# diegoroyo/mitransient

Measured on AMD Instinct MI355X. Metric: Mray/s (closest-hit + shadow rays), Cornell-box 512^2 x 1024 bins x 1024 spp per GPU, higher is better.
Workload: dtype f32; 1 GPU; cornell_box() diffuse, 512x512 px, 1024 time bins (start_opl 3.5, width 6/1024), 1024 spp per GPU (1024 spp total), max_depth 8, rr_depth 5, seed 0; parallelism=1 GPU, mode=auto (fused: scene + per-pixel time histograms in LDS)

## Files before the change

__graft_entry__.py:

```python
from __future__ import annotations

import os
import subprocess
import sys

ROOT = os.path.dirname(os.path.abspath(__file__))
if ROOT not in sys.path:
    sys.path.insert(0, ROOT)


def _run(cmd, cwd=None):
    r = subprocess.run(cmd, cwd=cwd, stdout=subprocess.PIPE, stderr=subprocess.STDOUT, text=True)
    if r.returncode != 0:
        raise RuntimeError(f"{' '.join(cmd)} failed:\n{r.stdout}")
    return r.stdout


def build_host_harness():
    out_dir = os.path.join(ROOT, "tests", "_build")
    os.makedirs(out_dir, exist_ok=True)
    out = os.path.join(out_dir, "libhost_harness.so")
    srcs = [os.path.join(ROOT, "tests", "host_harness.cpp"),
            os.path.join(ROOT, "mitransient_amd", "csrc", "mtr_scene_host.cpp"),
            os.path.join(ROOT, "mitransient_amd", "csrc", "mtr_bvh.cpp")]
    deps = srcs + [os.path.join(ROOT, "mitransient_amd", "csrc", h) for h in
                   ("mtr_core.h", "mtr_scene_host.h", "mtr_bvh.h", "mtr_knobs.h")]
    if os.path.exists(out) and all(os.path.getmtime(out) >= os.path.getmtime(d) for d in deps):
        return out
    _run(["g++", "-O2", "-std=c++17", "-fPIC", "-shared", "-ffp-contract=off", "-fno-fast-math", "-mfma", "-DMTR_EXPERIMENTS",
          "-o", out] + srcs)
    return out


def build() -> None:
    _run(["make", "-C", os.path.join(ROOT, "mitransient_amd", "csrc")])
    _run(["make", "-C", os.path.join(ROOT, "oracle")])
    build_host_harness()
    import mitransient_amd
    from mitransient_amd import _cabi
    lib = _cabi.load_library()
    for name in _cabi.EXPORTS:
        getattr(lib, name)


def smoke() -> None:
    import numpy as np
    import torch
    import mitransient_amd as mitr
    import mitransient_amd.mi as mi
    from oracle import oracle

    assert torch.cuda.is_available(), "smoke() needs a GPU"
    torch.cuda.set_device(0)
    mi.set_variant("llvm_ad_rgb")
    d = mitr.cornell_box()
    d["sensor"]["film"].update(width=64, height=64, temporal_bins=64, bin_width_opl=6.0 / 64)
    scene = mi.load_dict(d)
    integ = scene.integrator()
    integ.collect_stats = True
    steady, transient = mi.render(scene, spp=16, seed=0)
    torch.cuda.synchronize()
    t_gpu = np.array(transient)
    s_gpu = np.array(steady)
    sd = scene.data()
    params = integ.render_params(scene.sensors()[0].film(), 0, 16)
    t4, s4, cnt = oracle.render(sd, params, use_bvh=True)
    t_ref, s_ref = oracle.develop(sd.film, t4, s4)
    rel = float(np.linalg.norm(t_gpu - t_ref) / np.linalg.norm(t_ref))
    rel_s = float(np.linalg.norm(s_gpu - s_ref) / np.linalg.norm(s_ref))
    print(f"smoke: transient rel-L2 {rel:.3e}, steady rel-L2 {rel_s:.3e}, counters {integ.last_counters} vs oracle {cnt}")
    assert t_gpu.shape == (64, 64, 64, 3) and s_gpu.shape == (64, 64, 3)
    assert rel <= 1e-5, rel
    assert rel_s <= 1e-5, rel_s
    for k in ("paths", "rays_closest", "rays_shadow", "splats_issued", "bounces"):
        assert integ.last_counters[k] == cnt[k], (k, integ.last_counters[k], cnt[k])


if __name__ == "__main__":
    build()
# ... 3 lines not shown
```

include/mitransient_amd.h:

```cpp
#ifndef MITRANSIENT_AMD_H
#define MITRANSIENT_AMD_H

#include <stdint.h>
#include <stddef.h>

#ifdef __cplusplus
extern "C" {
#endif

#define MTR_ABI_VERSION 24

typedef enum mtr_status {
    MTR_OK = 0,
    MTR_ERR_INVALID = -1,
    MTR_ERR_NO_DEVICE = -2,
    MTR_ERR_HIP = -3,
    MTR_ERR_OOM = -4,
    MTR_ERR_UNSUPPORTED = -5
} mtr_status;

enum { MTR_BSDF_DIFFUSE = 0, MTR_BSDF_CONDUCTOR = 1, MTR_BSDF_DIELECTRIC = 2,
       MTR_BSDF_NULL = 3 ,
       MTR_BSDF_ROUGHCONDUCTOR = 4,
       MTR_BSDF_ROUGHPLASTIC = 5,
// ... 88 lines not shown
    uint32_t has_to_world;
    float    to_world[12];
    uint32_t kind;
    float    radius;
} mtr_shape;

#define MTR_NLOS_NO_RELAY 0xffffffffu
typedef struct mtr_nlos_desc {
    float    sensor_origin[3];
    uint32_t relay_shape;
    float    laser_to_world[16];
    float    laser_fov;
    float    laser_irradiance[3];
    float    laser_scale;
    uint32_t capture_type;
    uint32_t flags;
    int32_t  filter_depth;
    float    illumination_scan_fov;
    uint32_t n_shapes;
    const mtr_shape *shapes;
    uint32_t sensor_is_confocal;
    float    sensor_target[3];
} mtr_nlos_desc;

typedef struct mtr_scene_desc {
    uint32_t        n_tris;
    const float    *tri_verts;
    const uint32_t *tri_material;
    const int32_t  *tri_emitter;
    uint32_t        n_materials;
    const mtr_material *materials;
    uint32_t        n_emitters;
    const mtr_emitter  *emitters;
    mtr_camera      camera;
    mtr_film_desc   film;
    const mtr_nlos_desc *nlos;
    uint32_t        n_shapes;
    const mtr_shape *shapes;
    const float    *tri_uv;
    const float    *tri_normals;
    uint32_t        n_textures;
    const mtr_texture *textures;
} mtr_scene_desc;

enum { MTR_FLAG_CAMERA_UNWARP = 1u,
       MTR_FLAG_DISCARD_DIRECT_LIGHT = 2u,
       MTR_FLAG_FILM_ZERO = 4u,
       MTR_FLAG_KEEP_COUNTERS = 16u,
       MTR_FLAG_DETERMINISTIC = 32u,
       MTR_FLAG_DEVELOPED_ROWS = 64u,
       MTR_FLAG_PCG_INITSEQ_PLUS_LANE = 8u ,
       MTR_FLAG_POLARIZED = 256u,
       MTR_FLAG_PCG_TEA64 = 128u            };

enum { MTR_MODE_AUTO = 0,
       MTR_MODE_FUSED = 1,
       MTR_MODE_WAVEFRONT = 2,
       MTR_MODE_SAMPLES = 3      };

typedef struct mtr_render_params {
    uint32_t spp_total;
    uint32_t spp_begin;
    uint32_t spp_end;
    uint32_t pixel_begin;
    uint32_t pixel_end;
    uint32_t seed;
    int32_t  max_depth;
    int32_t  rr_depth;
    uint32_t flags;
    uint32_t mode;
    uint32_t spp_scale;
    uint32_t reserve_cus;
    uint32_t n_bands;
    uint32_t band_epoch;
    uint64_t band_done;
} mtr_render_params;

typedef struct mtr_counters {
    uint64_t paths;
    uint64_t rays_closest;
    uint64_t rays_shadow;
    uint64_t splats_issued;
    uint64_t bounces;
    uint64_t splats_overflow;
    uint64_t reserved[2];
} mtr_counters;

typedef struct mtr_splat_soa {
    const uint32_t *pixel;
    const float    *opl;
    const float    *r, *g, *b;
    uint64_t        n;
    const uint32_t *laser;
} mtr_splat_soa;

typedef struct mtr_kernel_times {
    float    total_ms;
    float    trace_ms;
    float    scatter_ms;
    uint32_t trace_launches;
    uint32_t scatter_launches;
    float    wf_trace_ms;
    uint32_t wf_trace_kernel_launches;
    float    wf_shade_ms;
} mtr_kernel_times;

typedef struct mtr_ctx   mtr_ctx;
typedef struct mtr_scene mtr_scene;

int  mtr_abi_version(void);

int  mtr_ctx_create(int device_ordinal, mtr_ctx **out);
void mtr_ctx_destroy(mtr_ctx *);
int  mtr_ctx_set_stream(mtr_ctx *, void *hip_stream);
const char *mtr_last_error(const mtr_ctx *);

int  mtr_scene_create(mtr_ctx *, const mtr_scene_desc *, mtr_scene **out);
void mtr_scene_destroy(mtr_scene *);
int  mtr_scene_set_film(mtr_scene *, const mtr_film_desc *);
int  mtr_scene_set_camera(mtr_scene *, const mtr_camera *);
int  mtr_scene_set_nlos(mtr_scene *, const mtr_nlos_desc *);
int  mtr_scene_bvh_info(const mtr_scene *, uint32_t *n_nodes, uint32_t *max_depth, uint32_t *n_leaves);
#define MTR_TRAIT_DIFFUSE          1u
#define MTR_TRAIT_ONE_RECT_EMITTER 2u
#define MTR_TRAIT_LEAF_PAIR        4u
#define MTR_TRAIT_FLAT_TOP         8u
#define MTR_TRAIT_FLAT_LEAVES     16u
#define MTR_TRAIT_NO_LOBES        32u
#define MTR_TRAIT_GREY            64u
int  mtr_scene_traits(const mtr_scene *, uint32_t *traits);
int  mtr_scene_set_colors(mtr_scene *, const float *material_a, const float *emitter_radiance);
int  mtr_scene_set_texture(mtr_scene *, uint32_t index, const float *rgb);
int  mtr_scene_texture_layout(const mtr_scene *, uint32_t index, uint32_t *first_texel, uint32_t *width, uint32_t *height);

int  mtr_scene_tint_layout(const mtr_scene *, uint32_t *n_slots, uint32_t *slot_material, uint32_t *slot_which);
int  mtr_scene_set_tints(mtr_scene *, const float *material_c, const float *material_c2);

int  mtr_film_clear(mtr_ctx *, const mtr_film_desc *, float *transient_hwt4 ,
                    float *steady_hw4 );

int  mtr_render(mtr_scene *, const mtr_render_params *,
                float *transient_hwt4, float *steady_hw4,
                mtr_counters *counters_out , mtr_kernel_times *times_out );

int  mtr_render_plan(mtr_scene *, const mtr_render_params *, uint32_t *mode_out,
                     uint32_t *developed_rows_ok );
int  mtr_render_samples_plan(mtr_scene *, const mtr_render_params *, uint32_t *slab_len, uint32_t *n_slabs,
                             uint32_t *scene_in_lds, uint32_t *extended);

int  mtr_render_grad(mtr_scene *, const mtr_render_params *params,
                     const float *grad_steady_hw3, const float *grad_transient_hwt3,
                     float *grad_materials, float *grad_emitters);

int  mtr_render_grad_tex(mtr_scene *, const mtr_render_params *params,
                         const float *grad_steady_hw3, const float *grad_transient_hwt3,
                         float *grad_materials, float *grad_emitters, float *grad_texels);
#define MTR_GRAD_TEX_NONE   0u
#define MTR_GRAD_TEX_SLAB   1u
#define MTR_GRAD_TEX_GLOBAL 2u
int  mtr_render_grad_tex_tier(const mtr_scene *, uint32_t *tier);

int  mtr_render_fwd(mtr_scene *, const mtr_render_params *params,
                    const float *tan_materials, const float *tan_emitters, const float *tan_texels ,
                    float *steady_hw3, float *transient_hwt3);
#define MTR_FWD_ROWS   1u
#define MTR_FWD_GLOBAL 2u
int  mtr_render_fwd_tier(const mtr_scene *, const mtr_render_params *params, uint32_t *tier);

int  mtr_render_grad_tint(mtr_scene *, const mtr_render_params *params,
                          const float *grad_steady_hw3, const float *grad_transient_hwt3,
                          float *grad_materials, float *grad_emitters, float *grad_texels , float *grad_tints );
int  mtr_render_fwd_tint(mtr_scene *, const mtr_render_params *params,
                         const float *tan_materials, const float *tan_emitters, const float *tan_texels ,
                         const float *tan_tints , float *steady_hw3, float *transient_hwt3);

int  mtr_counters_reset(mtr_ctx *);

int  mtr_counters_read(mtr_ctx *, mtr_counters *out );

int  mtr_film_develop(mtr_ctx *, const mtr_film_desc *,
                      const float *transient_hwt4, float *transient_hwt3 ,
                      const float *steady_hw4, float *steady_hw3 );

// ... 29 lines not shown
```

mitransient_amd/_cabi.py:

```python
from __future__ import annotations

import ctypes as C
import os

_HERE = os.path.dirname(os.path.abspath(__file__))
LIB_PATH = os.environ.get("MITRANSIENT_AMD_LIB") or os.path.join(_HERE, "csrc", "libmitransient_amd.so")

MTR_ABI_VERSION = 24
MTR_TRAIT_DIFFUSE, MTR_TRAIT_ONE_RECT_EMITTER, MTR_TRAIT_LEAF_PAIR, MTR_TRAIT_FLAT_TOP, MTR_TRAIT_FLAT_LEAVES, MTR_TRAIT_NO_LOBES, MTR_TRAIT_GREY = 1, 2, 4, 8, 16, 32, 64
MTR_SPLAT_FILM_ZERO = 0x100

MTR_BSDF_DIFFUSE, MTR_BSDF_CONDUCTOR, MTR_BSDF_DIELECTRIC, MTR_BSDF_NULL = 0, 1, 2, 3
MTR_BSDF_ROUGHCONDUCTOR, MTR_BSDF_ROUGHPLASTIC, MTR_BSDF_ROUGHDIELECTRIC, MTR_BSDF_THINDIELECTRIC, MTR_BSDF_PLASTIC = 4, 5, 6, 7, 8
MTR_MAT_TWOSIDED, MTR_MAT_NONLINEAR, MTR_MAT_BECKMANN, MTR_MAT_ANISOTROPIC = 1, 2, 4, 8
MTR_ROUGH_TRANSMITTANCE_RES = 64
MTR_FLAG_CAMERA_UNWARP = 1
MTR_FLAG_DISCARD_DIRECT_LIGHT = 2
MTR_FLAG_FILM_ZERO = 4
MTR_FLAG_PCG_INITSEQ_PLUS_LANE = 8
MTR_FLAG_PCG_TEA64 = 128
MTR_FLAG_KEEP_COUNTERS = 16
MTR_FLAG_DETERMINISTIC = 32
MTR_FLAG_DEVELOPED_ROWS = 64
MTR_FLAG_POLARIZED = 256
MTR_MODE_AUTO, MTR_MODE_FUSED, MTR_MODE_WAVEFRONT, MTR_MODE_SAMPLES = 0, 1, 2, 3
MTR_RECT_ANALYTIC, MTR_RECT_FLIP_NORMALS = 1, 2
MTR_EMITTER_AREA, MTR_EMITTER_POINT, MTR_EMITTER_SPOT, MTR_EMITTER_SPHERE = 0, 1, 2, 3
MTR_SHAPE_DEFAULT, MTR_SHAPE_SPHERE, MTR_SHAPE_FLIP_NORMALS = 0, 1, 0x100
MTR_GRAD_TEX_NONE, MTR_GRAD_TEX_SLAB, MTR_GRAD_TEX_GLOBAL = 0, 1, 2
MTR_FWD_ROWS, MTR_FWD_GLOBAL = 1, 2

_f3 = C.c_float * 3
_f16 = C.c_float * 16


class mtr_material(C.Structure):
    _fields_ = [("type", C.c_uint32), ("flags", C.c_uint32),
                ("a", _f3), ("b", _f3), ("c", _f3),
                ("int_ior", C.c_float), ("ext_ior", C.c_float), ("c2", _f3),
                ("alpha", C.c_float), ("internal_reflectance", C.c_float), ("specular_sampling_weight", C.c_float),
                ("albedo_texture", C.c_uint32), ("external_transmittance", C.c_float * MTR_ROUGH_TRANSMITTANCE_RES)]


class mtr_texture(C.Structure):
    _fields_ = [("width", C.c_uint32), ("height", C.c_uint32), ("rgb", C.POINTER(C.c_float))]


class mtr_emitter(C.Structure):
    _fields_ = [("center", _f3), ("du", _f3), ("dv", _f3), ("radiance", _f3),
                ("is_mesh", C.c_uint32), ("first_tri", C.c_uint32), ("n_tris", C.c_uint32),
                ("flip_normals", C.c_uint32),
                ("angular", C.c_uint32), ("cutoff", C.c_float), ("cos_cutoff", C.c_float), ("cos_beam", C.c_float),
                ("inv_transition", C.c_float),
                ("kind", C.c_uint32), ("axis", _f3),
                ("radius", C.c_float)]


class mtr_camera(C.Structure):
    _fields_ = [("sample_to_camera", _f16), ("to_world", _f16),
                ("near_clip", C.c_float), ("far_clip", C.c_float)]


class mtr_film_desc(C.Structure):
    _fields_ = [("width", C.c_uint32), ("height", C.c_uint32),
                ("crop_width", C.c_uint32), ("crop_height", C.c_uint32),
                ("crop_offset_x", C.c_uint32), ("crop_offset_y", C.c_uint32),
                ("temporal_bins", C.c_uint32),
                ("start_opl", C.c_float), ("bin_width_opl", C.c_float),
                ("laser_scan_width", C.c_uint32), ("laser_scan_height", C.c_uint32),
                ("n_frequencies", C.c_uint32), ("frequencies", C.POINTER(C.c_float))]


MTR_CAPTURE_SINGLE, MTR_CAPTURE_CONFOCAL, MTR_CAPTURE_EXHAUSTIVE = 1, 2, 3
# ... 41 lines not shown
                ("emitters", C.POINTER(mtr_emitter)),
                ("camera", mtr_camera),
                ("film", mtr_film_desc),
                ("nlos", C.POINTER(mtr_nlos_desc)),
                ("n_shapes", C.c_uint32),
                ("shapes", C.POINTER(mtr_shape)),
                ("tri_uv", C.POINTER(C.c_float)),
                ("tri_normals", C.POINTER(C.c_float)),
                ("n_textures", C.c_uint32),
                ("textures", C.POINTER(mtr_texture))]


class mtr_render_params(C.Structure):
    _fields_ = [("spp_total", C.c_uint32), ("spp_begin", C.c_uint32), ("spp_end", C.c_uint32),
                ("pixel_begin", C.c_uint32), ("pixel_end", C.c_uint32),
                ("seed", C.c_uint32), ("max_depth", C.c_int32), ("rr_depth", C.c_int32),
                ("flags", C.c_uint32), ("mode", C.c_uint32), ("spp_scale", C.c_uint32), ("reserve_cus", C.c_uint32),
                ("n_bands", C.c_uint32), ("band_epoch", C.c_uint32), ("band_done", C.c_uint64)]


class mtr_counters(C.Structure):
    _fields_ = [("paths", C.c_uint64), ("rays_closest", C.c_uint64), ("rays_shadow", C.c_uint64),
                ("splats_issued", C.c_uint64), ("bounces", C.c_uint64), ("splats_overflow", C.c_uint64),
                ("reserved", C.c_uint64 * 2)]

    def as_dict(self):
        d = {k: int(getattr(self, k)) for k in
             ("paths", "rays_closest", "rays_shadow", "splats_issued", "bounces", "splats_overflow")}
        d["reserved"] = [int(self.reserved[0]), int(self.reserved[1])]
        return d


class mtr_splat_soa(C.Structure):
    _fields_ = [("pixel", C.c_void_p), ("opl", C.c_void_p),
                ("r", C.c_void_p), ("g", C.c_void_p), ("b", C.c_void_p), ("n", C.c_uint64),
                ("laser", C.c_void_p)]


class mtr_kernel_times(C.Structure):
    _fields_ = [("total_ms", C.c_float), ("trace_ms", C.c_float), ("scatter_ms", C.c_float),
                ("trace_launches", C.c_uint32), ("scatter_launches", C.c_uint32),
                ("wf_trace_ms", C.c_float), ("wf_trace_kernel_launches", C.c_uint32),
                ("wf_shade_ms", C.c_float)]

    def as_dict(self):
        return {"total_ms": float(self.total_ms), "trace_ms": float(self.trace_ms),
                "scatter_ms": float(self.scatter_ms), "trace_launches": int(self.trace_launches),
                "scatter_launches": int(self.scatter_launches), "wf_trace_ms": float(self.wf_trace_ms),
                "wf_trace_kernel_launches": int(self.wf_trace_kernel_launches), "wf_shade_ms": float(self.wf_shade_ms)}


EXPORTS = [
    "mtr_abi_version", "mtr_ctx_create", "mtr_ctx_destroy", "mtr_ctx_set_stream", "mtr_last_error",
    "mtr_scene_create", "mtr_scene_destroy", "mtr_scene_set_film", "mtr_scene_set_nlos", "mtr_scene_bvh_info", "mtr_scene_traits",
    "mtr_ctx_trim", "mtr_film_clear", "mtr_render", "mtr_render_plan", "mtr_counters_reset", "mtr_counters_read", "mtr_film_develop", "mtr_splat_add", "mtr_debug_set_splat_log",
    "mtr_render_grad", "mtr_scene_set_colors",
    "mtr_render_grad_tex", "mtr_render_grad_tex_tier", "mtr_scene_set_texture", "mtr_scene_texture_layout",
    "mtr_render_fwd", "mtr_render_fwd_tier",
    "mtr_scene_tint_layout", "mtr_scene_set_tints", "mtr_render_grad_tint", "mtr_render_fwd_tint",
    "mtr_scene_set_camera", "mtr_render_samples_plan",
    "mtr_backproject",
]

_lib = None


class MitransientAMDError(RuntimeError):
    pass


def load_library() -> C.CDLL:
    global _lib
    if _lib is not None:
        return _lib
    if not os.path.exists(LIB_PATH):
        raise MitransientAMDError(
            f"{LIB_PATH} not found: build the gfx950 HIP library first "
            "(python -c 'import __graft_entry__ as g; g.build()'). There is no CPU fallback.")
    import torch
    lib = C.CDLL(LIB_PATH)
    vp = C.c_void_p
    lib.mtr_abi_version.restype = C.c_int
    lib.mtr_ctx_create.argtypes = [C.c_int, C.POINTER(vp)]
    lib.mtr_ctx_destroy.argtypes = [vp]
    lib.mtr_ctx_destroy.restype = None
    lib.mtr_ctx_set_stream.argtypes = [vp, vp]
    lib.mtr_last_error.argtypes = [vp]
    lib.mtr_last_error.restype = C.c_char_p
    lib.mtr_scene_create.argtypes = [vp, C.POINTER(mtr_scene_desc), C.POINTER(vp)]
    lib.mtr_scene_destroy.argtypes = [vp]
    lib.mtr_scene_destroy.restype = None
    lib.mtr_scene_set_film.argtypes = [vp, C.POINTER(mtr_film_desc)]
    lib.mtr_scene_set_nlos.argtypes = [vp, C.POINTER(mtr_nlos_desc)]
    lib.mtr_scene_bvh_info.argtypes = [vp, C.POINTER(C.c_uint32), C.POINTER(C.c_uint32), C.POINTER(C.c_uint32)]
    lib.mtr_scene_traits.argtypes = [vp, C.POINTER(C.c_uint32)]
    lib.mtr_counters_read.argtypes = [vp, C.POINTER(mtr_counters)]
    lib.mtr_counters_reset.argtypes = [vp]
    lib.mtr_ctx_trim.argtypes = [vp]
    lib.mtr_render_plan.argtypes = [vp, C.POINTER(mtr_render_params), C.POINTER(C.c_uint32), C.POINTER(C.c_uint32)]
    lib.mtr_film_clear.argtypes = [vp, C.POINTER(mtr_film_desc), vp, vp]
    lib.mtr_render.argtypes = [vp, C.POINTER(mtr_render_params), vp, vp,
                               C.POINTER(mtr_counters), C.POINTER(mtr_kernel_times)]
    lib.mtr_film_develop.argtypes = [vp, C.POINTER(mtr_film_desc), vp, vp, vp, vp]
    lib.mtr_splat_add.argtypes = [vp, C.POINTER(mtr_splat_soa), C.POINTER(mtr_film_desc), C.c_int, vp,
                                  C.POINTER(C.c_float)]
    lib.mtr_debug_set_splat_log.argtypes = [vp, vp, C.c_uint64, vp]
    lib.mtr_render_grad.argtypes = [vp, C.POINTER(mtr_render_params), vp, vp, vp, vp]
    lib.mtr_scene_set_colors.argtypes = [vp, vp, vp]
    lib.mtr_render_grad_tex.argtypes = [vp, C.POINTER(mtr_render_params), vp, vp, vp, vp, vp]
    lib.mtr_render_grad_tex_tier.argtypes = [vp, C.POINTER(C.c_uint32)]
    lib.mtr_scene_set_texture.argtypes = [vp, C.c_uint32, vp]
    lib.mtr_scene_texture_layout.argtypes = [vp, C.c_uint32, C.POINTER(C.c_uint32), C.POINTER(C.c_uint32), C.POINTER(C.c_uint32)]
    lib.mtr_render_fwd.argtypes = [vp, C.POINTER(mtr_render_params), vp, vp, vp, vp, vp]
    lib.mtr_render_fwd_tier.argtypes = [vp, C.POINTER(mtr_render_params), C.POINTER(C.c_uint32)]
    lib.mtr_scene_tint_layout.argtypes = [vp, C.POINTER(C.c_uint32), vp, vp]
    lib.mtr_scene_set_tints.argtypes = [vp, vp, vp]
    lib.mtr_render_grad_tint.argtypes = [vp, C.POINTER(mtr_render_params), vp, vp, vp, vp, vp, vp]
    lib.mtr_render_fwd_tint.argtypes = [vp, C.POINTER(mtr_render_params), vp, vp, vp, vp, vp, vp]
    lib.mtr_scene_set_camera.argtypes = [vp, C.POINTER(mtr_camera)]
    lib.mtr_render_samples_plan.argtypes = [vp, C.POINTER(mtr_render_params)] + [C.POINTER(C.c_uint32)] * 4
    lib.mtr_backproject.argtypes = [vp, C.POINTER(mtr_backproject_desc), vp, vp]
    if lib.mtr_abi_version() != MTR_ABI_VERSION:
        raise MitransientAMDError("libmitransient_amd.so ABI version mismatch; rebuild")
    _lib = lib
    return lib


def check(status: int, ctx=None, what: str = ""):
    if status == 0:
        return
    msg = ""
    try:
        msg = (load_library().mtr_last_error(ctx) or b"").decode()
    except Exception:
        pass
    raise MitransientAMDError(f"{what} failed (status {status}): {msg}")
```

mitransient_amd/csrc/mtr_api.hip:

```cpp
#include "../../include/mitransient_amd.h"
#include "mtr_knobs.h"
#include "mtr_scene_host.h"
#include "mtr_core.h"
#include "mtr_kernels.h"
#include "mtr_polar.h"
#include "mtr_grad.h"
#include "mtr_fwd_args.h"
#include "mtr_tint_args.h"
#include "mtr_samples_args.h"
#include "mtr_backproject.h"

#include <hip/hip_runtime.h>
#include <cassert>
#include <cmath>
#include <cstdio>
#include <cstring>
#include <cstdlib>
#include <initializer_list>
#include <string>
#include <vector>
#include <algorithm>
#include <utility>

using namespace mtr;
// ... 10 lines not shown
    hipEvent_t ev2 = nullptr, ev3 = nullptr;
    float *d_freq = nullptr; size_t freq_cap = 0;
    void *d_runs = nullptr; size_t runs_cap = 0;
    uint32_t *d_band_count = nullptr; size_t band_cap = 0;
    void *d_part = nullptr; size_t part_cap = 0;
    void *d_samples = nullptr; size_t samples_cap = 0;
    void *d_start = nullptr; size_t start_cap = 0;
    void *d_bp = nullptr; size_t bp_cap = 0;
};

struct WfWorkspace {
    void *planes = nullptr, *q_live = nullptr, *q_ray = nullptr, *q_mat = nullptr, *r_shadow = nullptr, *occ = nullptr, *counts = nullptr, *rec = nullptr, *rec_count = nullptr, *q_zombie = nullptr;
    uint32_t n_slots = 0, P = 0, rec_cap = 0, rows = 0;
    size_t bytes = 0;
    bool polar = false;
    uint32_t *host_count = nullptr;
    hipEvent_t poll_ev[2] = { nullptr, nullptr };
    void release()
    {
        n_slots = 0; P = 0; rec_cap = 0; rows = 0; bytes = 0; polar = false;
        for (void **p : { &planes, &q_live, &q_ray, &q_mat, &r_shadow, &occ, &counts, &rec, &rec_count, &q_zombie })
            if (*p) { (void)hipFree(*p); *p = nullptr; }
    }
};

struct NlosDev {
    bool on = false;
    NlosConst k{};
    void *shapes = nullptr, *tables = nullptr, *hg_tris = nullptr, *hg_vn = nullptr, *targets = nullptr;
    std::vector<mtr_shape> host_shapes;
};

struct mtr_scene {
    mtr_ctx *ctx = nullptr;
    WfWorkspace wf;
    NlosDev nlos;
    std::vector<float> tri_verts;
    std::vector<float> tri_normals;
    uint32_t n_emitters_area = 0;
    bool polar_ok = false;
    bool grey_scene = false;
    bool has_sphere = false;
    SceneDev dev{};
    Camera cam{};
    Film film{};
    mtr_film_desc film_desc{};
    float *d_freq = nullptr;
    std::vector<float> h_freq;
    uint32_t n_leaves = 0;
    std::vector<q4> tex_info;
    uint32_t n_texels = 0;
    std::vector<void *> allocs;
    SplatLog log{ nullptr, 0, nullptr };
};

static thread_local std::string g_err;

static int fail(mtr_ctx *c, int code, const std::string &msg)
{
    if (c) c->err = msg; else g_err = msg;
    return code;
}
static int usable_cus(const mtr_ctx *c, const mtr_render_params *p)
{
    const int keep = (int)std::min<uint32_t>(p->reserve_cus, (uint32_t)(c->n_cu > 1 ? c->n_cu - 1 : 0));
    return c->n_cu - keep;
}

#define HIP_TRY(c, expr)                                                                       \
    do {                                                                                        \
        hipError_t e_ = (expr);                                                                 \
        if (e_ != hipSuccess)                                                                   \
            return fail((c), e_ == hipErrorOutOfMemory ? MTR_ERR_OOM : MTR_ERR_HIP,             \
                        std::string(#expr) + ": " + hipGetErrorString(e_));                     \
    } while (0)

extern "C" {

int mtr_abi_version(void) { return MTR_ABI_VERSION; }

const char *mtr_last_error(const mtr_ctx *c) { return c ? c->err.c_str() : g_err.c_str(); }

int mtr_ctx_create(int device_ordinal, mtr_ctx **out)
{
    if (!out) return fail(nullptr, MTR_ERR_INVALID, "mtr_ctx_create: out is NULL");
    *out = nullptr;
    int n = 0;
    if (hipGetDeviceCount(&n) != hipSuccess || n == 0)
        return fail(nullptr, MTR_ERR_NO_DEVICE, "no HIP device visible; this library has no CPU path");
    if (device_ordinal < 0 || device_ordinal >= n)
        return fail(nullptr, MTR_ERR_INVALID, "mtr_ctx_create: device ordinal out of range");
    mtr_ctx *c = new mtr_ctx();
    c->device = device_ordinal;
    HIP_TRY(nullptr, hipSetDevice(device_ordinal));
    hipDeviceProp_t prop;
    HIP_TRY(nullptr, hipGetDeviceProperties(&prop, device_ordinal));
    c->n_cu = prop.multiProcessorCount > 0 ? prop.multiProcessorCount : 256;
    HIP_TRY(nullptr, hipMalloc((void **)&c->d_counters, sizeof(DevCounters)));
    HIP_TRY(nullptr, hipMalloc((void **)&c->d_ticket, 32 * sizeof(uint32_t)));
    for (hipEvent_t *e : { &c->ev0, &c->ev1, &c->ev2, &c->ev3 }) HIP_TRY(nullptr, hipEventCreate(e));
    *out = c;
    return MTR_OK;
}

void mtr_ctx_destroy(mtr_ctx *c)
{
// ... 32 lines not shown
    return MTR_OK;
}

template <class T>
static int upload(mtr_scene *s, const std::vector<T> &v, const T **out)
{
    size_t bytes = ((v.size() * sizeof(T) + 15) / 16) * 16;
    if (bytes == 0) bytes = 16;
    void *p = nullptr;
    HIP_TRY(s->ctx, hipMalloc(&p, bytes));
    s->allocs.push_back(p);
    HIP_TRY(s->ctx, hipMemset(p, 0, bytes));
    if (!v.empty()) HIP_TRY(s->ctx, hipMemcpy(p, v.data(), v.size() * sizeof(T), hipMemcpyHostToDevice));
    *out = (const T *)p;
    return MTR_OK;
}

extern "C" {

static int scene_take_film(mtr_scene *s, const mtr_film_desc &f);

int mtr_scene_create(mtr_ctx *c, const mtr_scene_desc *d, mtr_scene **out)
{
    if (!c || !d || !out) return fail(c, MTR_ERR_INVALID, "mtr_scene_create: NULL argument");
    *out = nullptr;
    int rc = check_film(c, d->film);
    if (rc) return rc;
    HostScene hs;
    if (const char *msg = derive_scene(*d, hs)) return fail(c, MTR_ERR_INVALID, std::string("mtr_scene_create: ") + msg);
    HIP_TRY(c, hipSetDevice(c->device));

    mtr_scene *s = new mtr_scene();
    s->ctx = c;
    s->cam = hs.cam;
    rc = scene_take_film(s, d->film);
    if (rc) { delete s; return rc; }

#define UP(vec, field)                                                       \
    do { rc = upload(s, vec, &s->dev.field); if (rc) { mtr_scene_destroy(s); return rc; } } while (0)
    UP(hs.nodes, nodes); UP(hs.tpairs, tpairs); UP(hs.tshade, tshade); UP(hs.mats, mats); UP(hs.ems, ems);
    s->dev.n_wnodes = (uint32_t)hs.wnodes.size(); s->dev.n_wnodes4 = (uint32_t)hs.wnodes4.size(); s->dev.n_wnodes8q = (uint32_t)hs.wnodes8q.size();
    if (hs.has_wide) UP(hs.wnodes, wnodes);
    UP(hs.wnodes4, wnodes4);
    if (!hs.wnodes8q.empty()) UP(hs.wnodes8q, wnodes8q);
    if (!hs.samp_tris.empty()) { UP(hs.samp_tris, samp_tris); UP(hs.face_pmf, face_pmf); UP(hs.face_cdf, face_cdf); }
    if (!hs.samp_vn.empty()) UP(hs.samp_vn, samp_vn);
    if (!hs.vnormals.empty()) UP(hs.vnormals, vnormals);
    if (!hs.texels.empty()) { UP(hs.texels, texels); UP(hs.tex_info, tex_info); UP(hs.uvs, uvs); }
#undef UP
    s->tex_info = hs.tex_info; s->n_texels = (uint32_t)hs.texels.size();
    s->dev.n_nodes = (uint32_t)hs.nodes.size(); s->dev.n_slots = (uint32_t)hs.tshade.size();
    s->dev.n_mats = d->n_materials; s->dev.n_ems = d->n_emitters;
    s->polar_ok = hs.polar_ok; s->grey_scene = hs.grey_scene; s->has_sphere = hs.has_sphere;
    s->dev.has_rough = hs.needs_ext ? 1u : 0u; s->dev.traits = hs.traits; s->dev.flat = hs.flat;
    s->dev.bvh_depth = hs.bvh_depth; s->n_leaves = hs.n_leaves;
    s->dev.wide_levels = hs.wide_levels; s->dev.wide4_levels = hs.wide4_levels; s->dev.wide8q_levels = hs.wide8q_levels;
    s->tri_verts.assign(d->tri_verts, d->tri_verts + 9 * (size_t)d->n_tris);
    if (d->tri_normals) s->tri_normals.assign(d->tri_normals, d->tri_normals + 9 * (size_t)d->n_tris);
    s->n_emitters_area = d->n_emitters;
    if (d->nlos) {
        rc = mtr_scene_set_nlos(s, d->nlos);
        if (rc) { mtr_scene_destroy(s); return rc; }
    }
    *out = s;
    return MTR_OK;
}

int mtr_scene_set_nlos(mtr_scene *s, const mtr_nlos_desc *n)
{
    if (!s || !n) return fail(s ? s->ctx : nullptr, MTR_ERR_INVALID, "mtr_scene_set_nlos: NULL argument");
    mtr_ctx *c = s->ctx;
    HIP_TRY(c, hipSetDevice(c->device));
    mtr_scene_desc d{};
    d.n_tris = (uint32_t)(s->tri_verts.size() / 9); d.tri_verts = s->tri_verts.data(); d.n_emitters = s->n_emitters_area;
    d.tri_normals = s->tri_normals.empty() ? nullptr : s->tri_normals.data();
    d.film = s->film_desc;
    memcpy(d.camera.sample_to_camera, s->cam.s2c, sizeof s->cam.s2c);
    memcpy(d.camera.to_world, s->cam.tw, sizeof s->cam.tw);
    d.camera.near_clip = s->cam.near_clip; d.camera.far_clip = s->cam.far_clip;
    d.nlos = n;
    if (d.film.n_frequencies && n->capture_type == MTR_CAPTURE_EXHAUSTIVE)
        return fail(c, MTR_ERR_UNSUPPORTED, "mtr_scene_set_nlos: an Exhaustive capture (MTR_CAPTURE_EXHAUSTIVE) is not available with a phasor_hdr_film");
    HostNlos hn;
    if (const char *msg = derive_nlos(d, hn)) return fail(c, MTR_ERR_INVALID, std::string("mtr_scene_set_nlos: ") + msg);
    NlosDev &D = s->nlos;
    void **old[] = { &D.shapes, &D.tables, &D.hg_tris, &D.hg_vn, &D.targets };
    for (void **p : old) if (*p) { (void)hipFree(*p); *p = nullptr; }
    const size_t ns = hn.shapes.size(), nt = hn.face_pmf.size();
    HIP_TRY(c, hipMalloc(&D.shapes, ns * sizeof(NlosShape)));
    HIP_TRY(c, hipMemcpy(D.shapes, hn.shapes.data(), ns * sizeof(NlosShape), hipMemcpyHostToDevice));
    std::vector<float> tab;
    tab.insert(tab.end(), hn.shape_pmf.begin(), hn.shape_pmf.end());
    tab.insert(tab.end(), hn.shape_cdf.begin(), hn.shape_cdf.end());
    tab.insert(tab.end(), hn.face_pmf.begin(), hn.face_pmf.end());
    tab.insert(tab.end(), hn.face_cdf.begin(), hn.face_cdf.end());
    HIP_TRY(c, hipMalloc(&D.tables, tab.size() * 4));
    HIP_TRY(c, hipMemcpy(D.tables, tab.data(), tab.size() * 4, hipMemcpyHostToDevice));
    HIP_TRY(c, hipMalloc(&D.hg_tris, hn.hg_tris.size() * sizeof(q4)));
    HIP_TRY(c, hipMemcpy(D.hg_tris, hn.hg_tris.data(), hn.hg_tris.size() * sizeof(q4), hipMemcpyHostToDevice));
    if (!hn.hg_vn.empty()) {
        HIP_TRY(c, hipMalloc(&D.hg_vn, hn.hg_vn.size() * sizeof(q4)));
        HIP_TRY(c, hipMemcpy(D.hg_vn, hn.hg_vn.data(), hn.hg_vn.size() * sizeof(q4), hipMemcpyHostToDevice));
    }
    const size_t n_targets = nlos_target_count(hn.k);
    HIP_TRY(c, hipMalloc(&D.targets, n_targets * sizeof(q4)));
    D.k = hn.k;
    D.k.shapes = (const NlosShape *)D.shapes;
// ... 119 lines not shown
                if (slot_material) slot_material[slots[i]] = (uint32_t)(i / 2u);
                if (slot_which) slot_which[slots[i]] = (uint32_t)(i & 1u);
            }
    return MTR_OK;
}

int mtr_scene_set_texture(mtr_scene *s, uint32_t index, const float *rgb)
{
    if (!s || !rgb) return fail(s ? s->ctx : nullptr, MTR_ERR_INVALID, "mtr_scene_set_texture: NULL argument");
    mtr_ctx *c = s->ctx;
    if (index >= s->tex_info.size()) return fail(c, MTR_ERR_INVALID, "mtr_scene_set_texture: unknown texture");
    if (s->nlos.on) return fail(c, MTR_ERR_UNSUPPORTED, "mtr_scene_set_texture: not for the NLOS tier");
    HIP_TRY(c, hipSetDevice(c->device));
    HIP_TRY(c, hipStreamSynchronize(c->stream));
    const q4 info = s->tex_info[index];
    const size_t first = fbits(info.x), n = (size_t)fbits(info.y) * fbits(info.z);
    std::vector<q4> tx(n);
    for (size_t k = 0; k < n; ++k) tx[k] = q4{ rgb[3 * k], rgb[3 * k + 1], rgb[3 * k + 2], 0.0f };
    HIP_TRY(c, hipMemcpy((void *)(s->dev.texels + first), tx.data(), n * sizeof(q4), hipMemcpyHostToDevice));
    double mean[3] = { 0.0, 0.0, 0.0 };
    for (size_t k = 0; k < n; ++k) for (int j = 0; j < 3; ++j) mean[j] += (double)rgb[3 * k + j];
    std::vector<mtr_material> mats(s->dev.n_mats);
    if (!mats.empty()) HIP_TRY(c, hipMemcpy(mats.data(), s->dev.mats, mats.size() * sizeof(mtr_material), hipMemcpyDeviceToHost));
    for (mtr_material &m : mats)
        if (m.albedo_texture == index + 1u) for (int j = 0; j < 3; ++j) m.a[j] = (float)(mean[j] / (double)n);
    if (!mats.empty()) HIP_TRY(c, hipMemcpy((void *)s->dev.mats, mats.data(), mats.size() * sizeof(mtr_material), hipMemcpyHostToDevice));
    return MTR_OK;
}

int mtr_scene_texture_layout(const mtr_scene *s, uint32_t index, uint32_t *first_texel, uint32_t *width, uint32_t *height)
{
    if (!s || index > s->tex_info.size()) return MTR_ERR_INVALID;
    const bool end = index == s->tex_info.size();
    if (first_texel) *first_texel = end ? s->n_texels : fbits(s->tex_info[index].x);
    if (width) *width = end ? 0u : fbits(s->tex_info[index].y);
    if (height) *height = end ? 0u : fbits(s->tex_info[index].z);
    return MTR_OK;
}

int mtr_render_grad_tex_tier(const mtr_scene *s, uint32_t *tier)
{
    if (!s || !tier) return MTR_ERR_INVALID;
    *tier = grad_tex_tier(s->dev, s->n_texels, s->nlos.on);
    return MTR_OK;
}

int mtr_scene_traits(const mtr_scene *s, uint32_t *traits)
{
    if (!s || !traits) return MTR_ERR_INVALID;
    static_assert(MTR_TRAIT_DIFFUSE == kTrDiffuse && MTR_TRAIT_ONE_RECT_EMITTER == kTrOneRectEmitter && MTR_TRAIT_LEAF_PAIR == kTrLeafPair &&
                  MTR_TRAIT_FLAT_TOP == kTrFlatTop && MTR_TRAIT_FLAT_LEAVES == kTrFlatLeaves && MTR_TRAIT_NO_LOBES == kTrNoLobes &&
                  MTR_TRAIT_GREY == kTrGrey, "public trait bits");
    *traits = s->dev.traits;
    return MTR_OK;
}

}

struct WfBytes {
    size_t planes, q_live, q_ray, q_mat, q_zombie, r_shadow, occ, counts, rec, rec_count;
    size_t total() const { return planes + q_live + q_ray + q_mat + q_zombie + r_shadow + occ + counts + rec + rec_count; }
};
static WfBytes wf_bytes(uint32_t n_slots, uint32_t P, uint32_t n_seg, uint32_t rec_cap, bool polar)
{
    WfBytes b;
    b.planes = wf_planes_bytes(n_slots) + (polar ? wf_polar_planes_bytes(n_slots) : 0);
    b.q_live = (size_t)2 * n_slots * 4;
    b.q_ray = (size_t)2 * n_slots * 32;
    b.q_mat = (size_t)kWfKeys * n_slots * 4;
    b.q_zombie = (size_t)2 * n_slots * 4;
    b.r_shadow = (size_t)n_slots * 32;
    b.occ = (size_t)n_slots + (size_t)n_seg * 16u + 16u;
    b.counts = ((size_t)n_seg * (7 + kWfKeys) + 16) * 4;
    b.rec = std::max<size_t>(16, (size_t)P * rec_cap * 16);
    b.rec_count = (size_t)P * 4;
    return b;
}
static int wf_alloc(mtr_scene *s, uint32_t n_slots, uint32_t P, uint32_t n_seg, uint32_t rec_cap, bool polar = false)
{
    mtr_ctx *c = s->ctx;
    WfWorkspace &w = s->wf;
    if (w.n_slots >= n_slots && w.P >= P && w.rec_cap == rec_cap && w.rows >= n_seg && w.planes && (w.polar || !polar)) return MTR_OK;
    w.release();
    const WfBytes b = wf_bytes(n_slots, P, n_seg, rec_cap, polar);
    HIP_TRY(c, hipMalloc(&w.planes, b.planes));
    HIP_TRY(c, hipMalloc(&w.q_live, b.q_live));
    HIP_TRY(c, hipMalloc(&w.q_ray, b.q_ray));
    HIP_TRY(c, hipMalloc(&w.q_mat, b.q_mat));
    HIP_TRY(c, hipMalloc(&w.q_zombie, b.q_zombie));
    HIP_TRY(c, hipMalloc(&w.r_shadow, b.r_shadow));
    HIP_TRY(c, hipMalloc(&w.occ, b.occ));
    HIP_TRY(c, hipMalloc(&w.counts, b.counts));
    HIP_TRY(c, hipMalloc(&w.rec, b.rec));
    HIP_TRY(c, hipMalloc(&w.rec_count, b.rec_count));
    if (!w.host_count) HIP_TRY(c, hipHostMalloc((void **)&w.host_count, 64));
    for (hipEvent_t &e : w.poll_ev) if (!e) HIP_TRY(c, hipEventCreateWithFlags(&e, hipEventDisableTiming));
    w.n_slots = n_slots; w.P = P; w.rec_cap = rec_cap; w.rows = n_seg; w.bytes = b.total(); w.polar = polar;
    return MTR_OK;
}

struct RenderStats {
    uint32_t launches = 0, scatter_launches = 0, trace_kernel_launches = 0;
    float trace_ms = 0.0f, shade_ms = 0.0f, scatter_ms = 0.0f;
};
struct EventPairs {
    std::vector<std::pair<hipEvent_t, hipEvent_t>> ev;
// ... 260 lines not shown
    HIP_TRY(c, hipMemcpy(&h, c->d_counters, sizeof h, hipMemcpyDeviceToHost));
    memset(out, 0, sizeof *out);
    out->paths = h.paths; out->rays_closest = h.rays_closest; out->rays_shadow = h.rays_shadow;
    out->splats_issued = h.splats_issued; out->bounces = h.bounces; out->splats_overflow = h.splats_overflow;
    out->reserved[0] = h.r0; out->reserved[1] = h.r1;
    return MTR_OK;
}
static int grow_device_buffer(mtr_ctx *c, void **ptr, size_t *cap, size_t need)
{
    if (*cap >= need) return MTR_OK;
    HIP_TRY(c, hipStreamSynchronize(c->stream));
    if (*ptr) (void)hipFree(*ptr);
    *ptr = nullptr; *cap = 0;
    HIP_TRY(c, hipMalloc(ptr, need));
    *cap = need;
    return MTR_OK;
}

extern "C" {

int mtr_film_clear(mtr_ctx *c, const mtr_film_desc *f, float *t4, float *s4)
{
    if (!c || !f) return fail(c, MTR_ERR_INVALID, "mtr_film_clear: NULL argument");
    HIP_TRY(c, hipSetDevice(c->device));
    size_t npix = (size_t)f->width * f->height;
    const Film fm = film_from_desc(*f);
    const size_t per_pixel = fm.n_freq ? (size_t)2 * fm.n_freq + 1 : (size_t)fm.bins * 4;
    if (t4) HIP_TRY(c, hipMemsetAsync(t4, 0, npix * per_pixel * sizeof(float), c->stream));
    if (s4) HIP_TRY(c, hipMemsetAsync(s4, 0, npix * 4 * sizeof(float), c->stream));
    return MTR_OK;
}

int mtr_render(mtr_scene *s, const mtr_render_params *p, float *t4, float *s4,
               mtr_counters *counters_out, mtr_kernel_times *times_out)
{
    if (!s || !p || !t4 || !s4) return fail(s ? s->ctx : nullptr, MTR_ERR_INVALID, "mtr_render: NULL argument");
    mtr_ctx *c = s->ctx;
    const Film &f = s->film;
    if (int r = check_render_ranges(c, f, p, "mtr_render", "shard the render")) return r;
    if (p->mode > MTR_MODE_SAMPLES) return fail(c, MTR_ERR_INVALID, "mtr_render: unknown mode");
    SamplesPlan spl{};
    if (p->mode == MTR_MODE_SAMPLES)
        if (int r = samples_check(s, p, p->pixel_end - p->pixel_begin, p->spp_end - p->spp_begin, &spl)) return r;
    HIP_TRY(c, hipSetDevice(c->device));

    FusedArgs a{};
    a.sc = s->dev; a.cam = s->cam; a.film = f;
    a.rc = make_render_const(*p, f, s->dev.n_ems);
    a.pixel_begin = p->pixel_begin; a.pixel_end = p->pixel_end;
    a.spp_begin = p->spp_begin; a.spp_chunk = p->spp_end - p->spp_begin;
    a.film_out = t4; a.steady_out = s4;
    a.counters = c->d_counters;
    a.log = s->log;
    a.nlos_on = s->nlos.on ? 1u : 0u;
    if (s->nlos.on) {
        a.nlos = s->nlos.k;
        if (s->nlos.k.film_w != f.width || s->nlos.k.film_h != f.height)
            return fail(c, MTR_ERR_INVALID, "mtr_render: film size changed after mtr_scene_set_nlos; call it again");
    }

    const uint32_t n_pixels = p->pixel_end - p->pixel_begin;
    const bool want_stats = counters_out || times_out;
    if (!(p->flags & MTR_FLAG_KEEP_COUNTERS)) HIP_TRY(c, hipMemsetAsync(c->d_counters, 0, sizeof(DevCounters), c->stream));
    if (s->log.count) HIP_TRY(c, hipMemsetAsync(s->log.count, 0, sizeof(unsigned long long), c->stream));
    if (times_out) HIP_TRY(c, hipEventRecord(c->ev0, c->stream));
    RenderStats st;
    if (n_pixels && a.spp_chunk && p->mode == MTR_MODE_SAMPLES) {
        constexpr size_t kSamplesRetain = (size_t)256 << 20;
        if (int r = grow_device_buffer(c, &c->d_samples, &c->samples_cap, spl.partial_bytes)) return r;
        SamplesArgs sa{};
        sa.sc = s->dev; sa.cam = s->cam; sa.film = f; sa.rc = a.rc;
        sa.pixel_begin = p->pixel_begin; sa.n_pixels = n_pixels; sa.spp_begin = p->spp_begin; sa.spp_chunk = a.spp_chunk;
        sa.film_zero = (p->flags & MTR_FLAG_FILM_ZERO) ? 1u : 0u;
        sa.partial = (float *)c->d_samples; sa.film_out = t4; sa.steady_out = s4; sa.counters = c->d_counters;
        HIP_TRY(c, launch_samples(sa, spl, c->stream));
        st.launches = 2;
        if (c->samples_cap > kSamplesRetain) {
            HIP_TRY(c, hipStreamSynchronize(c->stream));
            (void)hipFree(c->d_samples);
            c->d_samples = nullptr; c->samples_cap = 0;
        }
    } else if (n_pixels && a.spp_chunk) {
        uint32_t mode = p->mode, dev_ok = 0u;
        if (int r = resolve_mode(s, p, n_pixels, a.spp_chunk, &mode, &dev_ok)) return r;
        if ((p->flags & MTR_FLAG_DEVELOPED_ROWS) && !dev_ok)
            return fail(c, MTR_ERR_UNSUPPORTED, "mtr_render: MTR_FLAG_DEVELOPED_ROWS needs the fused organisation with time-bin rows in LDS (see mtr_render_plan)");
        if (p->n_bands && (mode == MTR_MODE_WAVEFRONT || !p->band_done || p->n_bands > n_pixels))
            return fail(c, MTR_ERR_UNSUPPORTED, "mtr_render: band completion words need the fused organisation, a band_done array and at most one band per pixel");
        if (mode == MTR_MODE_WAVEFRONT) {
            if (int r = wf_render(s, p, t4, s4, a.rc, times_out != nullptr, want_stats, &st)) return r;
        } else {
            FusedConfig cfg{};
            if (!fused_plan(s->dev, f, n_pixels, a.spp_chunk, usable_cus(c, p), a, cfg))
                return fail(c, MTR_ERR_UNSUPPORTED, "mtr_render: no kernel configuration fits (BVH depth / LDS)");
            const uint32_t launch_slot = c->fused_launches++ & 15u;
            a.ticket = c->d_ticket + launch_slot;
            static_assert(kStartSlots == 16u, "one path-start table per ticket counter of the rotation");
            if (const size_t tab_bytes = fused_start_table_bytes(a, cfg)) {
                if (start_slot_stride(c->start_cap) < tab_bytes)
                    if (int r = grow_device_buffer(c, &c->d_start, &c->start_cap, start_alloc_bytes(tab_bytes))) return r;
                a.start_tab = (unsigned char *)c->d_start + start_slot_off(start_slot_stride(c->start_cap), launch_slot);
            }
            a.n_bands = 0u;
            if (p->n_bands) {
                if (int r = grow_device_buffer(c, (void **)&c->d_band_count, &c->band_cap, (size_t)p->n_bands * sizeof(uint32_t))) return r;
                HIP_TRY(c, hipMemsetAsync(c->d_band_count, 0, (size_t)p->n_bands * sizeof(uint32_t), c->stream));
// ... 441 lines not shown
```

mitransient_amd/csrc/mtr_core.h:

```cpp
#pragma once
#ifndef MTR_WIDE
#define MTR_WIDE 8
#endif
#ifndef MTR_BATCH
#define MTR_BATCH 15
#endif
#ifndef MTR_PATH_STATE
#define MTR_PATH_STATE 3
#endif

#include <stdint.h>
#include <math.h>
#include "../../include/mitransient_amd.h"
#include "mtr_flat_prims.h"

#if defined(__HIPCC__)
#include <hip/hip_runtime.h>
#define MTR_HD __host__ __device__ __forceinline__
#else
#define MTR_HD inline __attribute__((always_inline))
#endif

namespace mtr {

struct f3 { float x, y, z; };

MTR_HD f3 mk(float x, float y, float z) { f3 r; r.x = x; r.y = y; r.z = z; return r; }
MTR_HD f3 operator-(f3 a, f3 b) { return mk(a.x - b.x, a.y - b.y, a.z - b.z); }
MTR_HD f3 operator-(f3 a) { return mk(-a.x, -a.y, -a.z); }
MTR_HD f3 operator*(f3 a, float s) { return mk(a.x * s, a.y * s, a.z * s); }
MTR_HD f3 operator/(f3 a, float s) { float r = 1.0f / s; return mk(a.x * r, a.y * r, a.z * r); }
MTR_HD float dot(f3 a, f3 b) { return fmaf(a.x, b.x, fmaf(a.y, b.y, a.z * b.z)); }
MTR_HD f3 cross(f3 a, f3 b)
{
    return mk(fmaf(a.y, b.z, -(a.z * b.y)), fmaf(a.z, b.x, -(a.x * b.z)), fmaf(a.x, b.y, -(a.y * b.x)));
}
MTR_HD f3 normalize(f3 a) { return a / sqrtf(dot(a, a)); }
MTR_HD f3 fma3(f3 a, float s, f3 b) { return mk(fmaf(a.x, s, b.x), fmaf(a.y, s, b.y), fmaf(a.z, s, b.z)); }
MTR_HD float max3(float a, float b, float c) { return fmaxf(a, fmaxf(b, c)); }
MTR_HD bool sign_neg(float s) { return s < 0.0f || (s == 0.0f && signbit(s)); }

constexpr float kPi = 3.14159265358979323846f;
constexpr float kInvPi = 0.31830988618379067154f;
constexpr float kRayEps = 1500.0f * 5.9604644775390625e-8f;
constexpr float kShadowEps = kRayEps * 10.0f;
constexpr float kInf = __builtin_huge_valf();
constexpr float kEdgeEps = 1.9073486328125e-06f;

struct Rng { uint64_t state, inc; };

MTR_HD uint32_t rng_u32(Rng &r)
{
    uint64_t old = r.state;
    r.state = old * 0x5851f42d4c957f2dULL + r.inc;
    uint32_t xs = (uint32_t)(((old >> 18u) ^ old) >> 27u);
    uint32_t rot = (uint32_t)(old >> 59u);
    return (xs >> rot) | (xs << ((0u - rot) & 31u));
}
MTR_HD float rng_f32(Rng &r)
{
    uint32_t u = (rng_u32(r) >> 9) | 0x3f800000u;
    float f;
    __builtin_memcpy(&f, &u, 4);
    return f - 1.0f;
}
MTR_HD void tea4(uint32_t &v0, uint32_t &v1)
{
// ... 221 lines not shown
    const uint32_t q = (uint32_t)(int32_t)k & 3u;
    s = (q == 0u) ? sq : (q == 1u) ? cq : (q == 2u) ? -sq : -cq;
    c = (q == 0u) ? cq : (q == 1u) ? -sq : (q == 2u) ? -cq : sq;
}
MTR_HD void sphere_dir_encode(f3 n, float &u, float &v)
{
    const float inv = 1.0f / ((fabsf(n.x) + fabsf(n.y)) + fabsf(n.z));
    const float px = n.x * inv, py = n.y * inv;
    const bool low = n.z < 0.0f;
    u = low ? copysignf(1.0f - fabsf(py), px) : px;
    v = low ? copysignf(1.0f - fabsf(px), py) : py;
}
MTR_HD f3 sphere_dir_decode(float u, float v)
{
    const float z = (1.0f - fabsf(u)) - fabsf(v);
    const bool low = z < 0.0f;
    return normalize(mk(low ? copysignf(1.0f - fabsf(v), u) : u, low ? copysignf(1.0f - fabsf(u), v) : v, z));
}

struct Camera {
    float s2c[16];
    float tw[16];
    float near_clip, far_clip;
};

struct Film {
    uint32_t width, height, crop_w, crop_h, crop_x, crop_y;
    uint32_t bins;
    float start_opl, bin_width;
    uint32_t tbins;
    uint32_t lasers;
    uint32_t n_freq;
    const float *freq;
};

struct SceneView {
    bool node_pairs;
    const Node *nodes;
    const WNode *wnodes;
    const QNode4 *wnodes4;
    const QNode8 *wnodes8q;
    const TriPair *tpairs;
    const TriShade *tshade;
    const mtr_material *mats;
    const Emitter *ems;
    uint32_t n_emitters;
    uint32_t n_slots;
    const q4 *samp_tris;
    const q4 *samp_vn;
    const float *face_pmf, *face_cdf;
    const q4 *vnormals;
    const q4 *texels; const q4 *tex_info; const q4 *uvs;
    uint32_t flat_off;
};

MTR_HD uint32_t distr_sample_reuse(const float *cdf, const float *pmf, uint32_t n, float value, float &reused, float &pmf_out)
{
    uint32_t i = 0;
    while (i + 1 < n && !(value < cdf[i])) ++i;
    while (i + 1 < n && pmf[i] == 0.0f) ++i;
    const float prev = i ? cdf[i - 1] : 0.0f;
    reused = (value - prev) / pmf[i];
    pmf_out = pmf[i];
    return i;
}

MTR_HD void mesh_sample_position(const q4 *samp_tris, const float *face_cdf, const float *face_pmf, uint32_t first_tri,
                                 uint32_t n_tris, float u1, float u2, f3 &p, f3 &n, const q4 *samp_vn = nullptr)
{
    float sy = u2;
    uint32_t fi = 0;
    if (n_tris > 1) { float r2, fp; fi = distr_sample_reuse(face_cdf + first_tri, face_pmf + first_tri, n_tris, u2, r2, fp); sy = r2; }
    const q4 *t = samp_tris + 3 * (size_t)(first_tri + fi);
    const q4 a = t[0], b = t[1], cc = t[2];
    const float tt = sqrtf(fmaxf(1.0f - u1, 0.0f));
    const float b0 = 1.0f - tt, b1 = tt * sy;
    p = mk(fmaf(a.w, b0, fmaf(b.z, b1, a.x)), fmaf(b.x, b0, fmaf(b.w, b1, a.y)), fmaf(b.y, b0, fmaf(cc.x, b1, a.z)));
    n = mk(cc.y, cc.z, cc.w);
    if (samp_vn) {
        const q4 *v = samp_vn + 3 * (size_t)(first_tri + fi);
        const q4 n0 = v[0];
        if (n0.w != 0.0f) {
            const q4 n1 = v[1], n2 = v[2];
            const float w0 = 1.0f - b0 - b1;
            n = normalize(mk(fmaf(n0.x, w0, fmaf(n1.x, b0, n2.x * b1)), fmaf(n0.y, w0, fmaf(n1.y, b0, n2.y * b1)),
                             fmaf(n0.z, w0, fmaf(n1.z, b0, n2.z * b1))));
        }
    }
}

struct FastDiv { uint32_t m, s1, s2, d; };
inline FastDiv fastdiv_make(uint32_t d)
{
    FastDiv f; f.d = d ? d : 1u;
    if (f.d == 1u) { f.m = 0u; f.s1 = 0u; f.s2 = 0u; return f; }
    uint32_t l = 0; while ((1ull << l) < f.d) ++l;
    f.m = (uint32_t)((((1ull << l) - f.d) << 32) / f.d + 1ull);
    f.s1 = 1u; f.s2 = l - 1u;
    return f;
}
MTR_HD uint32_t fastdiv(uint32_t n, const FastDiv &f)
{
#if defined(__HIP_DEVICE_COMPILE__)
    const uint32_t t = __umulhi(f.m, n);
#else
    const uint32_t t = (uint32_t)(((uint64_t)f.m * n) >> 32);
// ... 518 lines not shown
    while (tr.cur != kTravDone) {
        const bool at_prim = tr.cur < 0;
        if (__ballot(at_prim) != 0ull) {
            if (is_quad_leaf(tr.cur)) {
                const bool found = trav_quad_test(tr, sc, st, ANY_HIT);
                if (ANY_HIT & found) tr.cur = kTravDone;
                else wide_advance<kWide>(tr, sc.wnodes, st, tr.grp);
            } else if (at_prim) wide_leaf_step<kWide, ONE_PAIR, SPH>(tr, sc, sc.wnodes, st, ANY_HIT);
        } else {
            wide_node_step<kWide, true>(tr, sc.wnodes, st);
        }
    }
#endif
}
#endif

#if defined(__HIPCC__)
template <class T, bool ONE_BASE = false>
__device__ __forceinline__ T kernarg_copy(size_t offset)
{
    static_assert(sizeof(T) % 4 == 0, "dword-sized fields");
    typedef const uint32_t __attribute__((address_space(4))) *WordPtr;
    typedef const char __attribute__((address_space(4))) *BytePtr;
    BytePtr base = (BytePtr)__builtin_amdgcn_kernarg_segment_ptr();
    if (ONE_BASE) asm volatile("" : "+s"(base));
    WordPtr w = (WordPtr)(base + offset);
    if (!ONE_BASE) asm volatile("" : "+s"(w));
    T out;
    uint32_t *o = (uint32_t *)&out;
#pragma unroll
    for (size_t k = 0; k < sizeof(T) / 4; ++k) o[k] = w[k];
    return out;
}
constexpr bool flat_prim_table_on(bool lean, bool top_leaves) { return lean && !top_leaves && (MTR_BATCH & 4) != 0 && kWide <= kFlatPrimQuads; }
template <size_t N>
__device__ __forceinline__ void kernarg_pin_words(const uint32_t *o)
{
#define MTR_PIN_W(k) "s"(o[(k) < N ? (k) : N - 1])
    asm volatile("" :: MTR_PIN_W(0), MTR_PIN_W(1), MTR_PIN_W(2), MTR_PIN_W(3), MTR_PIN_W(4), MTR_PIN_W(5), MTR_PIN_W(6), MTR_PIN_W(7),
                       MTR_PIN_W(8), MTR_PIN_W(9), MTR_PIN_W(10), MTR_PIN_W(11), MTR_PIN_W(12), MTR_PIN_W(13), MTR_PIN_W(14), MTR_PIN_W(15));
#undef MTR_PIN_W
    if constexpr (N > 16) kernarg_pin_words<N - 16>(o + 16);
}
template <class T>
__device__ __forceinline__ void kernarg_pin(const T &v)
{
    static_assert(sizeof(T) % 4 == 0, "dword-sized fields");
    kernarg_pin_words<sizeof(T) / 4>((const uint32_t *)&v);
}
#endif

template <class S, class = void> struct stack_one_kernarg_base { static constexpr bool value = false; };
template <class S> struct stack_one_kernarg_base<S, decltype((void)S::kOneKernargBase)> { static constexpr bool value = S::kOneKernargBase; };

#if defined(__HIP_DEVICE_COMPILE__)
template <bool ANY_HIT, uint32_t J, bool BATCH = false>
__device__ __forceinline__ void flat_slab_pair(const f3 id, const f3 noid, const float tb, const uint32_t sel0, const uint32_t sel1, const uint32_t sel2,
                                               const char *root, const bool p0, const bool p1, uint32_t &qm, uint32_t &key1, uint32_t &key2)
{
    const char *pb = root + 48u * J;
    f2 nx, fx, ny, fy, nz, fz;
    if constexpr (BATCH) {
        const f2 pnx = *(const f2 *)(pb + sel0), pfx = *(const f2 *)(pb + (sel0 ^ 8u));
        const f2 pny = *(const f2 *)(pb + sel1), pfy = *(const f2 *)(pb + (sel1 ^ 8u));
        const f2 pnz = *(const f2 *)(pb + sel2), pfz = *(const f2 *)(pb + (sel2 ^ 8u));
        nx = fma2<kPkSlabs>(pnx, id.x, noid.x); fx = fma2<kPkSlabs>(pfx, id.x, noid.x);
        ny = fma2<kPkSlabs>(pny, id.y, noid.y); fy = fma2<kPkSlabs>(pfy, id.y, noid.y);
        nz = fma2<kPkSlabs>(pnz, id.z, noid.z); fz = fma2<kPkSlabs>(pfz, id.z, noid.z);
    } else {
        nx = fma2<kPkSlabs>(*(const f2 *)(pb + sel0), id.x, noid.x); fx = fma2<kPkSlabs>(*(const f2 *)(pb + (sel0 ^ 8u)), id.x, noid.x);
        ny = fma2<kPkSlabs>(*(const f2 *)(pb + sel1), id.y, noid.y); fy = fma2<kPkSlabs>(*(const f2 *)(pb + (sel1 ^ 8u)), id.y, noid.y);
        nz = fma2<kPkSlabs>(*(const f2 *)(pb + sel2), id.z, noid.z); fz = fma2<kPkSlabs>(*(const f2 *)(pb + (sel2 ^ 8u)), id.z, noid.z);
    }
    const float tn0 = fmaxf(fmaxf(nx.x, ny.x), fmaxf(nz.x, 0.0f));
    const float tf0 = fminf(fminf(fx.x, fy.x), fminf(fz.x, tb));
    const float tn1 = fmaxf(fmaxf(nx.y, ny.y), fmaxf(nz.y, 0.0f));
    const float tf1 = fminf(fminf(fx.y, fy.y), fminf(fz.y, tb));
    const bool h0 = (tn0 <= tf0) && p0;
    const bool h1 = (tn1 <= tf1) && p1;
    qm |= (h0 ? 1u : 0u) << (2u * J);
    qm |= (h1 ? 2u : 0u) << (2u * J);
    if (!ANY_HIT) {
        const uint32_t ka = h0 ? ((fbits(tn0) & ~7u) | (2u * J)) : 0xffffffffu, kb = h1 ? ((fbits(tn1) & ~7u) | (2u * J + 1u)) : 0xffffffffu;
        key2 = min(key2, max(key1, ka)); key1 = min(key1, ka);
        key2 = min(key2, max(key1, kb)); key1 = min(key1, kb);
    }
}
__device__ __forceinline__ RecByValue flat_prim_fetch(const char *root, const uint32_t n_boxes, const uint32_t entry)
{
    const char *tab = root - flat_prim_bytes(n_boxes);
    const TriPair *p = (const TriPair *)(tab + flat_prim_rec_off(entry));
    RecByValue r;
    r.tp.g[0] = p->g[0]; r.tp.g[1] = p->g[1]; r.tp.g[2] = p->g[2]; r.tp.g[3] = p->g[3]; r.tp.g[4] = p->g[4];
    r.first = *(const uint32_t *)(tab + flat_prim_first_off(n_boxes, entry));
    return r;
}
template <bool ANY_HIT, bool ONE_PAIR, bool TOP_LEAVES, class Stack>
__device__ __forceinline__ Hit flat_walk_device(const SceneView &sc, const f3 o, const f3 d, const float tmax, Stack &st)
{
    typedef WNode N;
    Trav tr;
    const RayByValue ray{ o, d, tmax };
    tr.h.t = kInf; tr.h.u = 0.0f; tr.h.v = 0.0f; tr.h.prim = -1;
    tr.best_orig = 0xffffffffu;
    st.reset();
    if (!sc.n_slots) return tr.h;
    const char *root = (const char *)sc.wnodes;
    constexpr bool kOneBase = stack_one_kernarg_base<Stack>::value;
    constexpr bool kTable = flat_prim_table_on(kOneBase, TOP_LEAVES);
    const FlatHdr fh =kernarg_copy<FlatHdr, kOneBase>(sc.flat_off);
    bool live = true;
    uint32_t fm = 0u;
    const float omax = fmaxf(fmaxf(fabsf(o.x), fabsf(o.y)), fabsf(o.z));
    for (uint32_t b = 0; b < fh.n_boxes; ++b) {
        const FlatXf X = kernarg_copy<FlatXf, kOneBase>(sc.flat_off + sizeof(FlatHdr) + sizeof(FlatXf) * b);
        const q4 A = X.A, B = X.B, C = X.C, S = X.S;
        const f3 ol = mk(fmaf(A.z, o.z, fmaf(A.y, o.y, fmaf(A.x, o.x, A.w))), fmaf(B.z, o.z, fmaf(B.y, o.y, fmaf(B.x, o.x, B.w))),
                         fmaf(C.z, o.z, fmaf(C.y, o.y, fmaf(C.x, o.x, C.w))));
        const f3 dl = mk(fmaf(A.z, d.z, fmaf(A.y, d.y, A.x * d.x)), fmaf(B.z, d.z, fmaf(B.y, d.y, B.x * d.x)),
                         fmaf(C.z, d.z, fmaf(C.y, d.y, C.x * d.x)));
        const f3 id = mk(safe_rcp(dl.x), safe_rcp(dl.y), safe_rcp(dl.z));
        fm |= box_select(box_mag_bound(A, B, C, S, omax), ol, dl, id, tmax) << (6u * b);
    }
    st.prof_flat(0);
    while (__ballot(live && fm != 0u) != 0ull) {
        if (live && fm != 0u) {
            const uint32_t k = (uint32_t)__builtin_ctz(fm);
            fm &= fm - 1u;
            if constexpr (kTable) {
                const RecByValue rec = flat_prim_fetch(root, fh.n_boxes, kFlatPrimQuads + k);
                const bool found = trav_leaf_test<true, false>(tr, sc, st, ANY_HIT, ray, rec);
                if (ANY_HIT && found) live = false;
            } else {
                const uint32_t box = (k * 43u) >> 8, face = k - 6u * box;
                tr.cur = *(const int32_t *)(root + (size_t)(fh.node0 + box) * N::kBytes + N::kRefOff + 4u * face);
                const bool found = trav_leaf_test<true>(tr, sc, st, ANY_HIT, ray);
                if (ANY_HIT && found) live = false;
            }
        }
    }
    st.prof_flat(5);
    if (__ballot(live) != 0ull) {
        const f3 id = mk(safe_rcp(d.x), safe_rcp(d.y), safe_rcp(d.z));
        const f3 noid = mk(-(o.x * id.x), -(o.y * id.y), -(o.z * id.z));
        const uint32_t sel0 = id.x < 0.0f ? 8u : 0u, sel1 = 16u + (id.y < 0.0f ? 8u : 0u), sel2 = 32u + (id.z < 0.0f ? 8u : 0u);
        const float tb = fminf(tmax, tr.h.t);
        uint32_t qm = 0u;
        uint32_t key1 = 0xffffffffu, key2 = 0xffffffffu;
#define MTR_FLAT_SLAB_PAIR(J) flat_slab_pair<ANY_HIT, J, kOneBase && (MTR_BATCH & 1) != 0>(id, noid, tb, sel0, sel1, sel2, root, \
            TOP_LEAVES ? ((fh.prim_mask >> (2u * J)) & 1u) != 0u : 2u * J < fh.n_quads, \
            TOP_LEAVES ? ((fh.prim_mask >> (2u * J + 1u)) & 1u) != 0u : 2u * J + 1u < fh.n_quads, qm, key1, key2)
        if (TOP_LEAVES) {
            MTR_FLAT_SLAB_PAIR(0u);
            if (fh.prim_mask > 3u) MTR_FLAT_SLAB_PAIR(1u);
            if (fh.prim_mask > 15u) MTR_FLAT_SLAB_PAIR(2u);
            if (kWide > 6u && fh.prim_mask > 63u) MTR_FLAT_SLAB_PAIR(3u);
        } else {
            MTR_FLAT_SLAB_PAIR(0u); MTR_FLAT_SLAB_PAIR(1u); MTR_FLAT_SLAB_PAIR(2u);
            if (kWide > 6u && fh.n_quads > 6u) MTR_FLAT_SLAB_PAIR(3u);
        }
#undef MTR_FLAT_SLAB_PAIR
        if (!live) qm = 0u;
        st.prof_flat(2);
        for (uint32_t it = 0; __ballot(qm != 0u) != 0ull; ++it) {
            if (qm != 0u) {
                const uint32_t k = (!ANY_HIT && it == 0u) ? (key1 & 7u) : (uint32_t)__builtin_ctz(qm);
                qm &= ~(1u << k);
                if constexpr (kTable) {
                    const RecByValue rec = flat_prim_fetch(root, fh.n_boxes, flat_prim_quad_entry(k));
                    const bool found = trav_quad_test(tr, sc, st, ANY_HIT, ray, rec);
                    if (ANY_HIT ? found : (it == 0u && tr.h.t < bitsf(key2 & ~7u))) qm = 0u;
                } else {
                    tr.cur = *(const int32_t *)(root + N::kRefOff + 4u * k);
                    const bool found = (!TOP_LEAVES || is_quad_leaf(tr.cur)) ? trav_quad_test(tr, sc, st, ANY_HIT, ray)
                                                                             : trav_leaf_test<ONE_PAIR, false>(tr, sc, st, ANY_HIT, ray);
                    if (ANY_HIT ? found : (it == 0u && tr.h.t < bitsf(key2 & ~7u))) qm = 0u;
                }
            }
        }
    }
    st.prof_flat(4);
    return tr.h;
}
#endif

template <bool ANY_HIT, bool ONE_PAIR = false, int FLAT = 0, bool SPH = !ONE_PAIR && FLAT == 0, class Stack>
MTR_HD Hit traverse(const SceneView &sc, f3 o, f3 d, float tmax, Stack &st)
{
#if defined(__HIP_DEVICE_COMPILE__)
    if (FLAT) return flat_walk_device<ANY_HIT, ONE_PAIR, FLAT == 2>(sc, o, d, tmax, st);
#endif
    Trav tr;
    trav_init(tr, sc, o, d, tmax, st);
#ifdef MTR_PROFILE_SIMT
    uint32_t my_nodes = 0;
#endif
    if (sc.wnodes) {
#if defined(__HIP_DEVICE_COMPILE__) && !defined(MTR_NODES_FIRST)
        wide_walk_device<ANY_HIT, ONE_PAIR, SPH>(tr, sc, st);
#else
        while (tr.cur != kTravDone) {
            while (tr.cur >= 0) {
                wide_node_step<kWide, true>(tr, sc.wnodes, st);
#ifdef MTR_PROFILE_SIMT
                ++my_nodes;
#endif
            }
            if (is_quad_leaf(tr.cur)) {
                const bool found = trav_quad_test(tr, sc, st, ANY_HIT);
                if (ANY_HIT & found) tr.cur = kTravDone;
                else wide_advance<kWide>(tr, sc.wnodes, st, tr.grp);
            } else if (tr.cur != kTravDone) wide_leaf_step<kWide, ONE_PAIR, SPH>(tr, sc, sc.wnodes, st, ANY_HIT);
        }
#endif
    } else if (sc.wnodes8q) {
        while (tr.cur != kTravDone) {
            while (tr.cur >= 0) q8_node_step(tr, sc.wnodes8q, st);
            if (tr.cur != kTravDone) q8_leaf_step<SPH>(tr, sc, st, ANY_HIT);
        }
    } else if (sc.wnodes4) {
        while (tr.cur != kTravDone) {
            while (tr.cur >= 0) qwide_node_step(tr, sc.wnodes4, st);
            if (tr.cur != kTravDone) qwide_leaf_step<SPH>(tr, sc, st, ANY_HIT);
        }
    } else
    while (tr.cur != kTravDone) {
        while (tr.cur >= 0) {
            trav_node_step(tr, sc, st);
#ifdef MTR_PROFILE_SIMT
            ++my_nodes;
#endif
        }
        if (tr.cur != kTravDone) trav_leaf_step<SPH>(tr, sc, st, ANY_HIT);
    }
#ifdef MTR_PROFILE_SIMT
    st.tail(my_nodes);
#endif
    return tr.h;
}

MTR_HD Ray camera_ray(const Camera &c, const RenderConst &rc, uint32_t px, uint32_t py, float j1, float j2)
{
    float sx = fmaf((float)px + j1, rc.inv_crop_w, rc.off_x);
// ... 650 lines not shown
    if (!EXT || m.albedo_texture == 0u || !sc.texels) return mk(m.a[0], m.a[1], m.a[2]);
    float u, v;
    if (fbits(sc.tshade[h.prim].h[4].w) & kShadeQuadBit) { u = fmaf(h.u, 0.5f, 0.5f); v = fmaf(h.v, 0.5f, 0.5f); }
    else {
        const q4 a = sc.uvs[2u * (uint32_t)h.prim], b = sc.uvs[2u * (uint32_t)h.prim + 1u];
        const float b1 = h.u, b2 = h.v, b0 = 1.0f - b1 - b2;
        u = fmaf(b.x, b2, fmaf(a.z, b1, a.x * b0)); v = fmaf(b.y, b2, fmaf(a.w, b1, a.y * b0));
    }
    return texture_eval(sc.texels, sc.tex_info[m.albedo_texture - 1u], u, v);
}

struct TexTaps { size_t i00, i10, i01, i11; uint32_t first; float w0x, w1x, w0y, w1y; };
MTR_HD TexTaps texture_taps(q4 info, float u, float v)
{
    TexTaps t;
    const int32_t W = (int32_t)fbits(info.y), H = (int32_t)fbits(info.z);
    const float fu = fmaf(u, (float)W, -0.5f), fv = fmaf(v, (float)H, -0.5f);
    const float flu = floorf(fu), flv = floorf(fv);
    t.w1x = fu - flu; t.w1y = fv - flv; t.w0x = 1.0f - t.w1x; t.w0y = 1.0f - t.w1y;
    const int32_t ix = (int32_t)flu, iy = (int32_t)flv;
    int32_t x0 = ix % W, x1 = (ix + 1) % W, y0 = iy % H, y1 = (iy + 1) % H;
    x0 += x0 < 0 ? W : 0; x1 += x1 < 0 ? W : 0; y0 += y0 < 0 ? H : 0; y1 += y1 < 0 ? H : 0;
    t.first = fbits(info.x);
    t.i00 = (size_t)y0 * W + x0; t.i10 = (size_t)y0 * W + x1; t.i01 = (size_t)y1 * W + x0; t.i11 = (size_t)y1 * W + x1;
    return t;
}
MTR_HD f3 texture_eval(const q4 *texels, const TexTaps &k)
{
    const float w0x = k.w0x, w1x = k.w1x, w0y = k.w0y, w1y = k.w1y;
    const q4 *t = texels + k.first;
    const q4 v00 = t[k.i00], v10 = t[k.i10], v01 = t[k.i01], v11 = t[k.i11];
    const float r0 = fmaf(w0x, v00.x, w1x * v10.x), r1 = fmaf(w0x, v01.x, w1x * v11.x);
    const float g0 = fmaf(w0x, v00.y, w1x * v10.y), g1 = fmaf(w0x, v01.y, w1x * v11.y);
    const float b0 = fmaf(w0x, v00.z, w1x * v10.z), b1 = fmaf(w0x, v01.z, w1x * v11.z);
    return mk(fmaf(w0y, r0, w1y * r1), fmaf(w0y, g0, w1y * g1), fmaf(w0y, b0, w1y * b1));
}
MTR_HD void hit_uv(const SceneView &sc, const Hit &h, float &u, float &v)
{
    if (fbits(sc.tshade[h.prim].h[4].w) & kShadeQuadBit) { u = fmaf(h.u, 0.5f, 0.5f); v = fmaf(h.v, 0.5f, 0.5f); }
    else {
        const q4 a = sc.uvs[2u * (uint32_t)h.prim], b = sc.uvs[2u * (uint32_t)h.prim + 1u];
        const float b1 = h.u, b2 = h.v, b0 = 1.0f - b1 - b2;
        u = fmaf(b.x, b2, fmaf(a.z, b1, a.x * b0)); v = fmaf(b.y, b2, fmaf(a.w, b1, a.y * b0));
    }
}

MTR_HD f3 offset_point(f3 sp, f3 sn, f3 dir)
{
    float m = max3(fabsf(sp.x), fabsf(sp.y), fabsf(sp.z));
    float mag = (1.0f + m) * kRayEps;
    if (sign_neg(dot(sn, dir))) mag = -mag;
    return fma3(sn, mag, sp);
}

MTR_HD bool sphere_ref_outside(const Emitter &E, float dc2)
{
    const float radj = E.du[0] * (E.n[0] < 0.0f ? 1.0f + kRayEps : 1.0f - kRayEps);
    return dc2 > radj * radj;
}
MTR_HD float sphere_cone_one_minus_cos(const Emitter &E, float dc2, float &sin2_max, float &cos_max)
{
    sin2_max = (E.du[0] * E.du[0]) / dc2;
    const float c2 = 1.0f - sin2_max;
    cos_max = sqrtf(c2 > 0.0f ? c2 : 0.0f);
    return sin2_max / (1.0f + cos_max);
}
MTR_HD float sphere_pdf_direction(const Emitter &E, f3 ref, float dist2, float adp)
{
    const f3 dc = ld3(E.center) - ref;
    const float dc2 = dot(dc, dc);
    if (sphere_ref_outside(E, dc2)) {
        float s2, cm;
        const float omc = sphere_cone_one_minus_cos(E, dc2, s2, cm);
        const float pdf = 1.0f / ((2.0f * kPi) * omc);
        return (fabsf(pdf) <= 3.402823466e+38f) ? pdf : 0.0f;
    }
    const float x = dist2 / adp;
    return E.inv_area * ((fabsf(x) <= 3.402823466e+38f) ? x : 0.0f);
}
MTR_HD void sphere_sample_direction(const Emitter &E, f3 ref, float u1, float u2, f3 &ep, f3 &en)
{
    const f3 c = ld3(E.center);
    const f3 dc = c - ref;
    const float dc2 = dot(dc, dc), r = E.du[0];
    f3 d;
    if (sphere_ref_outside(E, dc2)) {
        float sin2_max, cos_max;
        const float omc = sphere_cone_one_minus_cos(E, dc2, sin2_max, cos_max);
        const float sin_max = sqrtf(sin2_max);
        const float ct = fmaf(-omc, u1, 1.0f);
        const float sin2 = sin2_max > 0.00068523f ? fmaf(-ct, ct, 1.0f) : sin2_max * u1;
        const float c2 = 1.0f - sin2, cos_t = sqrtf(c2 > 0.0f ? c2 : 0.0f);
        const float w = 1.0f - sin2 / sin2_max;
        const float cos_a = fmaf(cos_t, sqrtf(w > 0.0f ? w : 0.0f), sin2 / sin_max);
        const float sa2 = fmaf(-cos_a, cos_a, 1.0f), sin_a = sqrtf(sa2 > 0.0f ? sa2 : 0.0f);
        float sp, cp;
        sincos_2pi(u2, sp, cp);
        const f3 axis = -(dc / sqrtf(dc2));
        f3 fs, ft;
        coordinate_system(axis, fs, ft);
        const float lx = cp * sin_a, ly = sp * sin_a;
        d = mk(fmaf(axis.x, cos_a, fmaf(ft.x, ly, fs.x * lx)), fmaf(axis.y, cos_a, fmaf(ft.y, ly, fs.y * lx)), fmaf(axis.z, cos_a, fmaf(ft.z, ly, fs.z * lx)));
    } else {
        const float z = fmaf(-2.0f, u2, 1.0f), rho2 = fmaf(-z, z, 1.0f), rho = sqrtf(rho2 > 0.0f ? rho2 : 0.0f);
        float sp, cp;
        sincos_2pi(u1, sp, cp);
// ... 36 lines not shown
    const mtr_material &mat = sc.mats[c.mat];

    if (c.em_plus1 != 0u && !(rc.flags & MTR_FLAG_DISCARD_DIRECT_LIGHT)) {
        const Emitter &E = sc.ems[kOneRect ? 0u : c.em_plus1 - 1u];
        f3 rel = c.sp - p.prev_p;
        float dist = sqrtf(dot(rel, rel));
        f3 dd = rel / dist;
        float em_pdf = 0.0f;
        const bool ang = !kOneRect && E.angular != 0u;
        if (!prev_delta) {
            float dp = dot(dd, c.sn);
            if (dp < 0.0f && (!ang || angular_falloff(E, unit_z(to_local_about(c.sn, -dd))) > 0.0f)) {
                float adp = fabsf(dp);
                em_pdf = E.inv_area * (adp != 0.0f ? (dist * dist) / adp : 0.0f);
                if constexpr (kSph) { if (E.kind == kEmSphere) em_pdf = sphere_pdf_direction(E, p.prev_p, dist * dist, adp); }
                if (n_emitters > 1) em_pdf *= rc.inv_n_emitters;
            }
        }
        float mis = mis_weight(p.prev_pdf, em_pdf);
        if (ang) {
            const float fall = angular_falloff(E, unit_z(c.wi));
            if (c.wi.z > 0.0f && fall > 0.0f)
                pd.Le = mk((p.beta.x * mis) * (E.radiance[0] * fall), (p.beta.y * mis) * (E.radiance[1] * fall),
                           (p.beta.z * mis) * (E.radiance[2] * fall));
        } else
        if (c.wi.z > 0.0f)
            pd.Le = mk((p.beta.x * mis) * E.radiance[0], (p.beta.y * mis) * E.radiance[1],
                       (p.beta.z * mis) * E.radiance[2]);
        float vr = pd.Le.x * rc.sample_scale, vg = pd.Le.y * rc.sample_scale, vb = pd.Le.z * rc.sample_scale;
        if (in_film && (vr != 0.0f || vg != 0.0f || vb != 0.0f)) {
            int32_t bin = film_bin(film, p.dist);
            if (bin >= 0) sink.splat(fx, fy, (uint32_t)bin, vr, vg, vb, p.dist, p.depth, 0u);
        }
    }

    if (pd.active_next && (kDiff || mat.type == MTR_BSDF_DIFFUSE || (lobes_on<ROUGH, TR>() && bsdf_is_rough(mat.type))) && n_emitters > 0 ) {
        uint32_t ei = 0;
        if (n_emitters > 1) {
            float su = u1 * rc.n_emitters_f;
            uint32_t i = (uint32_t)su;
            if (i > n_emitters - 1) i = n_emitters - 1;
            ei = i; u1 = su - (float)i;
        }
        pick(ei);
        const Emitter &E = sc.ems[ei];
        const bool delta = !kOneRect && (kSph ? (E.kind == kEmPoint || E.kind == kEmSpot) : E.kind >= kEmPoint);
        const bool sphere = kSph && E.kind == kEmSphere;
        f3 ep, en;
        if (delta) { ep = ld3(E.center); en = ld3(E.n); }
        else if (sphere) sphere_sample_direction(E, c.sp, u1, u2, ep, en);
        else if (!kOneRect && E.kind == kEmMesh) {
            mesh_sample_position(sc.samp_tris, sc.face_cdf, sc.face_pmf, E.first_tri, E.n_tris, u1, u2, ep, en, ROUGH ? sc.samp_vn : nullptr);
        } else {
            float a = fmaf(u1, 2.0f, -1.0f), b = fmaf(u2, 2.0f, -1.0f);
            ep = mk(fmaf(E.du[0], a, fmaf(E.dv[0], b, E.center[0])),
                    fmaf(E.du[1], a, fmaf(E.dv[1], b, E.center[1])),
                    fmaf(E.du[2], a, fmaf(E.dv[2], b, E.center[2])));
            en = ld3(E.n);
        }
        f3 dd = ep - c.sp;
        float dist2 = dot(dd, dd), dist = sqrtf(dist2);
        dd = dd / dist;
        float dp = dot(dd, en), adp = fabsf(dp);
        float x = dist2 / adp;
        float pdf_dir = E.inv_area * ((fabsf(x) <= 3.402823466e+38f) ? x : 0.0f);
        if (delta) pdf_dir = dist2 > 0.0f ? 1.0f : 0.0f;
        if (sphere) pdf_dir = dist2 > 0.0f ? sphere_pdf_direction(E, c.sp, dist2, adp) : 0.0f;
        const bool ang = !kOneRect && (E.angular != 0u || E.kind == kEmSpot);
        const float fall = ang ? angular_falloff(E, unit_z(to_local_about(en, -dd))) : 1.0f;
        if (((dp < 0.0f) | delta) & (pdf_dir != 0.0f) & (fall > 0.0f)) {
            f3 emw;
            if (ang || delta) { const float inv_dist = 1.0f / dist; emw = (ld3(E.radiance) * (fall * (inv_dist * inv_dist))) / pdf_dir; }
            else emw = ld3(E.radiance) / pdf_dir;
            float pdf = pdf_dir;
            if (n_emitters > 1) { pdf = pdf_dir * rc.inv_n_emitters; emw = emw * rc.n_emitters_f; }
            if (pdf != 0.0f) {
                f3 wo = mk(dot(dd, c.ss), dot(dd, c.stt), dot(dd, c.sn));
                f3 wi_e = c.wi;
                if (!kDiff && (mat.flags & MTR_MAT_TWOSIDED) && wi_e.z < 0.0f) { wi_e.z = -wi_e.z; wo.z = -wo.z; }
                f3 so = offset_point(c.sp, c.gn, ep - c.sp);
                f3 sd = ep - so;
                float sdist = sqrtf(dot(sd, sd));
                shadow.o = so; shadow.d = sd / sdist; shadow.tmax = sdist * (1.0f - kShadowEps);
                pd.has_shadow = 1u;
                if constexpr (LEAN && (MTR_PATH_STATE & 2) != 0) { pd.Lr = mk(0, 0, 0); pd.opl = 0.0f; }
                if (lobes_on<ROUGH, TR>() && bsdf_is_rough(mat.type)) {
                    f3 bval; float bpdf;
                    pd.alb = material_albedo<ROUGH>(sc, mat, h); pd.has_alb = 1u;
                    rough_eval_pdf(mat, pd.alb, wi_e, wo, bval, bpdf);
                    float mis_em = delta ? 1.0f : mis_weight(pdf, bpdf);
                    pd.Lr = mk(((p.beta.x * mis_em) * bval.x) * emw.x, ((p.beta.y * mis_em) * bval.y) * emw.y,
                               ((p.beta.z * mis_em) * bval.z) * emw.z);
                    pd.opl = p.dist + dist * eta;
                } else
                if (wi_e.z > 0.0f && wo.z > 0.0f) {
                    float bpdf = kInvPi * wo.z;
                    float mis_em = delta ? 1.0f : mis_weight(pdf, bpdf);
                    const f3 alb = material_albedo<ROUGH>(sc, mat, h);
                    if (ROUGH) { pd.alb = alb; pd.has_alb = 1u; }
                    pd.Lr = mk(((p.beta.x * mis_em) * ((alb.x * kInvPi) * wo.z)) * emw.x,
                               ((p.beta.y * mis_em) * ((alb.y * kInvPi) * wo.z)) * emw.y,
                               ((p.beta.z * mis_em) * ((alb.z * kInvPi) * wo.z)) * emw.z);
                    pd.opl = p.dist + (kDiff ? dist : dist * eta);
                }
            }
        }
    }
}

template <bool ROUGH = true, uint32_t TR = 0u, bool LEAN = false, class Sink>
MTR_HD bool shade_finish(Path &p, const Hit &h, bool occluded, const Pending &pd, const SceneView &sc,
                         const Film &film, const RenderConst &rc, Sink &sink, const HitCtx *kept = nullptr)
{
    constexpr bool kDiff = (TR & kTrDiffuse) != 0u;
    const bool valid = h.prim >= 0;
    bool active_next = pd.active_next != 0u;
    f3 Lr = mk(0, 0, 0);
    if (pd.has_shadow && !occluded) {
        Lr = pd.Lr;
        const uint32_t fx = p.px - film.crop_x, fy = p.py - film.crop_y;
        float vr = Lr.x * rc.sample_scale, vg = Lr.y * rc.sample_scale, vb = Lr.z * rc.sample_scale;
        if ((fx < film.width) & (fy < film.height) && (vr != 0.0f || vg != 0.0f || vb != 0.0f)) {
            int32_t bin = film_bin(film, pd.opl);
            if (bin >= 0) sink.splat(fx, fy, (uint32_t)bin, vr, vg, vb, pd.opl, p.depth, 1u);
        }
    }
    float s1 = rng_f32(p.rng), s2a = rng_f32(p.rng), s2b = rng_f32(p.rng);
    float rr_u = rng_f32(p.rng);

    BsdfSample bs;
    bs.wo = mk(0, 0, 0); bs.pdf = 0.0f; bs.eta = 1.0f; bs.delta = false; bs.w = mk(0, 0, 0);
    f3 sp = mk(0, 0, 0);
    if constexpr (LEAN && (MTR_PATH_STATE & 2) != 0) {
        MTR_FORGET(bs.w.x); MTR_FORGET(bs.w.y); MTR_FORGET(bs.w.z); MTR_FORGET(bs.pdf); MTR_FORGET(sp.x); MTR_FORGET(sp.y); MTR_FORGET(sp.z);
    }
    p.L = mk((p.L.x + pd.Le.x) + Lr.x, (p.L.y + pd.Le.y) + Lr.y, (p.L.z + pd.Le.z) + Lr.z);
// ... 5 lines not shown
        if (active_next) {
            const f3 albedo = (ROUGH && pd.has_alb) ? pd.alb : material_albedo<ROUGH>(sc, sc.mats[c.mat], h);
            bs = bsdf_sample<ROUGH, TR>(sc.mats[c.mat], c.wi, s1, s2a, s2b, albedo);
            f3 wo_w = mk(fmaf(c.sn.x, bs.wo.z, fmaf(c.stt.x, bs.wo.y, c.ss.x * bs.wo.x)),
                         fmaf(c.sn.y, bs.wo.z, fmaf(c.stt.y, bs.wo.y, c.ss.y * bs.wo.x)),
                         fmaf(c.sn.z, bs.wo.z, fmaf(c.stt.z, bs.wo.y, c.ss.z * bs.wo.x)));
            p.ray.o = offset_point(c.sp, c.gn, wo_w);
            p.ray.d = wo_w;
            p.ray.tmax = kInf;
        }
    }
    if (!kDiff) p.eta *= bs.eta;
    p.beta = mk(p.beta.x * bs.w.x, p.beta.y * bs.w.y, p.beta.z * bs.w.z);
    p.prev_p = sp; p.prev_pdf = bs.pdf;
    if (!kDiff) p.prev_delta = bs.delta ? 1u : 0u;

    float bmax = max3(p.beta.x, p.beta.y, p.beta.z);
    active_next &= (bmax != 0.0f);
    float rr_prob = fminf(kDiff ? bmax : bmax * (p.eta * p.eta), 0.95f);
    active_next &= rr_prob > 0.0f;
    bool rr_active = p.depth >= rc.rr_depth;
    if (rr_active) {
        float inv = rr_prob > 0.0f ? 1.0f / rr_prob : 0.0f;
        p.beta = p.beta * inv;
    }
    active_next &= (!rr_active) | (rr_u < rr_prob);
    if (valid) p.depth += 1;
    return active_next;
}

struct NoRefresh { template <class Sink> MTR_HD void operator()(Path &, Sink &) const {} };
template <bool ROUGH = true, uint32_t TR = 0u, class Stack, class Sink, class Refresh = NoRefresh>
MTR_HD bool path_bounce(Path &p, const SceneView &sc, const Film &film, const RenderConst &rc,
                        Stack &st, Sink &sink, BounceStats &stats, const Refresh &refresh = Refresh(), bool unwarp_here = false)
{
    st.prof_mark(2);
    Hit h = traverse<false, (TR & kTrLeafPair) != 0u, flat_kind(TR), tr_spheres(TR)>(sc, p.ray.o, p.ray.d, p.ray.tmax, st);
    st.prof_mark(0);
    stats.closest++;
    Pending pd; Ray shadow;
    shadow.o = mk(0, 0, 0); shadow.d = mk(0, 0, 1); shadow.tmax = 0.0f;
    constexpr bool kLeanState = stack_one_kernarg_base<Stack>::value && flat_kind(TR) == 1;
    if constexpr (kLeanState && (MTR_PATH_STATE & 2) != 0) forget_ray(shadow);
    if (Stack::kPark) { p.prev_p = st.unpark_prev_p(); p.prev_pdf = st.unpark_prev_pdf(); p.rng.inc = st.unpark_inc(); }
    refresh(p, sink);
    if (unwarp_here && p.depth == 0u && h.prim >= 0) p.dist = -h.t;
    constexpr bool kHandOver = stack_one_kernarg_base<Stack>::value && flat_kind(TR) == 1 && (TR & kTrCornell) == kTrCornell && (MTR_BATCH & 8) != 0;
    HitCtx kept;
    shade_hit<ROUGH, TR, kLeanState>(p, h, sc, film, rc, sink, pd, shadow, kHandOver ? &kept : nullptr);
    st.prof_mark(1);
    bool occluded = false;
    if (pd.has_shadow) {
        stats.shadow++;
        Hit sh = traverse<true, (TR & kTrLeafPair) != 0u, flat_kind(TR), tr_spheres(TR)>(sc, shadow.o, shadow.d, shadow.tmax, st);
        occluded = sh.prim >= 0;
    }
    st.prof_mark(0);
    if (Stack::kPark) p.rng.inc = st.unpark_inc();
    refresh(p, sink);
    const bool an = shade_finish<ROUGH, TR, kLeanState>(p, h, occluded, pd, sc, film, rc, sink, kHandOver ? &kept : nullptr);
    if (Stack::kPark) { st.park_prev_p(p.prev_p); st.park_prev_pdf(p.prev_pdf); }
    st.prof_mark(1);
    return an;
}

template <class Sink>
MTR_HD void commit_pending(f3 &L, f3 Lr, float opl, uint32_t depth_log, uint32_t px, uint32_t py,
                           const Film &film, const RenderConst &rc, Sink &sink)
{
    const uint32_t fx = px - film.crop_x, fy = py - film.crop_y;
    const float vr = Lr.x * rc.sample_scale, vg = Lr.y * rc.sample_scale, vb = Lr.z * rc.sample_scale;
    if ((fx < film.width) & (fy < film.height) && (vr != 0.0f || vg != 0.0f || vb != 0.0f)) {
        const int32_t bin = film_bin(film, opl);
        if (bin >= 0) sink.splat(fx, fy, (uint32_t)bin, vr, vg, vb, opl, depth_log, 1u);
    }
    L = mk(L.x + Lr.x, L.y + Lr.y, L.z + Lr.z);
}

}
```

mitransient_amd/csrc/mtr_kernels.h:

```cpp
#pragma once
#include <hip/hip_runtime.h>
#include "mtr_core.h"
#include "mtr_nlos.h"
#include "mtr_start_blocks.h"

namespace mtr {

#ifndef MTR_BLOCK
#define MTR_BLOCK 256
#endif
constexpr int kBlock = MTR_BLOCK;

struct DevCounters {
    unsigned long long paths, rays_closest, rays_shadow, splats_issued, bounces, splats_overflow, r0, r1;
};

struct SceneDev {
    const Node *nodes; uint32_t n_nodes;
    const WNode *wnodes; uint32_t n_wnodes;
    const QNode4 *wnodes4; uint32_t n_wnodes4;
    const QNode8 *wnodes8q; uint32_t n_wnodes8q;
    const TriPair *tpairs; const TriShade *tshade; uint32_t n_slots;
    const mtr_material *mats; uint32_t n_mats;
    const Emitter *ems; uint32_t n_ems;
// ... 72 lines not shown
        WNode *n = (WNode *)(smem + off); off += al16(sc.n_wnodes * sizeof(WNode));
        TriPair *tg = (TriPair *)(smem + off); off += al16(sc.n_slots / 2 * sizeof(TriPair));
        TriShade *ts = (TriShade *)(smem + off); off += al16(sc.n_slots * sizeof(TriShade));
        mtr_material *mm = (mtr_material *)(smem + off); off += al16(sc.n_mats * sizeof(mtr_material));
        Emitter *ee = (Emitter *)(smem + off);
        cp16(n, sc.wnodes, al16(sc.n_wnodes * sizeof(WNode)), tid);
        cp16(tg, sc.tpairs, al16(sc.n_slots / 2 * sizeof(TriPair)), tid);
        cp16(ts, sc.tshade, al16(sc.n_slots * sizeof(TriShade)), tid);
        cp16(mm, sc.mats, al16(sc.n_mats * sizeof(mtr_material)), tid);
        cp16(ee, ems, al16(sc.n_ems * sizeof(Emitter)), tid);
        sv.nodes = nullptr; sv.wnodes = n; sv.wnodes4 = nullptr; sv.wnodes8q = nullptr; sv.tpairs = tg; sv.tshade = ts; sv.mats = mm; sv.ems = ee;
        sv.node_pairs = true;
    } else {
        sv.nodes = sc.nodes; sv.tpairs = sc.tpairs; sv.tshade = sc.tshade; sv.mats = sc.mats; sv.ems = ems;
        sv.wnodes = nullptr; sv.wnodes4 = sc.wnodes4; sv.wnodes8q = sc.wnodes8q;
        sv.node_pairs = false;
    }
    return sv;
}

template <class K, class A>
hipError_t launch_with_lds(K kernel, const A &args, int grid, size_t lds, hipStream_t stream)
{
    hipError_t e = hipFuncSetAttribute((const void *)kernel, hipFuncAttributeMaxDynamicSharedMemorySize, (int)lds);
    if (e != hipSuccess) return e;
    hipLaunchKernelGGL(kernel, dim3(grid), dim3(kBlock), lds, stream, args);
    return hipGetLastError();
}

struct SplatLog { uint32_t *rec; unsigned long long cap; unsigned long long *count; };

struct FusedArgs {
    SceneDev sc;
    Camera cam;
    Film film;
    RenderConst rc;
    uint32_t pixel_begin, pixel_end;
    uint32_t spp_begin, spp_chunk;
    uint32_t G;
    FastDiv div_spp, div_G;
    uint32_t stack_rows;
    uint32_t chunk, n_chunks;
    uint32_t *ticket;
    float *film_out;
    float *steady_out;
    DevCounters *counters;
    SplatLog log;
    uint32_t nlos_on;
    float fixed_lim; uint32_t fixed_dcap;
    uint32_t n_bands, band_px, band_epoch;
    uint32_t *band_count, *band_done;
    NlosConst nlos;
    unsigned char *start_tab;
};

struct FusedConfig { int stack; bool scene_lds; bool hist_lds; bool fixed; bool rough; size_t lds_bytes; int grid; int per_cu; uint32_t traits; };

constexpr uint64_t kChunkContribs = 16u;
inline uint32_t fused_chunk_cap(uint32_t chunk, uint32_t spp_chunk)
{
    const uint64_t per_px = (uint64_t)(spp_chunk ? spp_chunk : 1u) * kChunkContribs;
    const uint64_t cap = ((1ull << 32) - 1ull) / per_px;
    if ((uint64_t)chunk > cap) chunk = (uint32_t)cap;
    return chunk < 1u ? 1u : chunk;
}

uint32_t fused_chunk(uint32_t n_pixels, uint32_t spp_chunk, uint32_t grid);
bool fused_plan(const SceneDev &sc, const Film &film, uint32_t n_pixels, uint32_t spp_chunk, int n_cu,
                FusedArgs &args, FusedConfig &cfg);
size_t fused_start_table_bytes(const FusedArgs &args, const FusedConfig &cfg);
hipError_t launch_fused(const FusedArgs &args, const FusedConfig &cfg, hipStream_t stream);
hipError_t launch_nlos_prepare(const SceneDev &sc, const NlosConst &nc, q4 *targets, hipStream_t stream);

constexpr uint32_t kWfKeys = 5;

struct WfArgs {
    SceneDev sc;
    Camera cam;
    Film film;
    RenderConst rc;
    uint32_t pix0, P;
    uint32_t spp_begin, S;
    uint32_t n_slots;
    uint32_t G, seg, n_seg;
    uint32_t parity;
    uint32_t *ticket; uint32_t ticket_cur;
    float *planes;
    uint32_t *q_live;
    float4 *q_ray;
    uint32_t *seg_live;
    uint32_t *seg_list;
    uint32_t *seg_list_n;
    uint32_t *q_mat;
    float4 *r_shadow;
    uint32_t *seg_shadow;
    uint32_t *q_zombie;
    uint32_t *seg_zombie;
    uint8_t *occ;
    uint32_t occ_stride;
    uint32_t trace_any;
    uint32_t first_bounce;
    uint32_t *seg_mat;
    uint32_t *live_total;
    uint4 *rec;
    uint32_t *rec_count;
    uint32_t rec_cap;
// ... 43 lines not shown
```

mitransient_amd/csrc/mtr_kernels.hip:

```cpp
#include "mtr_kernels.h"
#include "mtr_knobs.h"

#include <hip/hip_runtime.h>
#include <algorithm>
#include <type_traits>
#include <hip/amd_detail/amd_hip_unsafe_atomics.h>

namespace mtr {

template <bool ONE_BASE = false>
struct LdsStackT {
    static constexpr bool kOneKernargBase = ONE_BASE;
    int32_t *base;
    int sp;
    __device__ __forceinline__ void reset() { sp = 0; }
    __device__ __forceinline__ void push_if(bool c, int32_t v) { base[sp * kBlock] = v; sp += c ? 1 : 0; }
    __device__ __forceinline__ int32_t pop() { --sp; return base[sp * kBlock]; }
    __device__ __forceinline__ bool empty() const { return sp == 0; }
#ifndef MTR_NO_PARK
    static constexpr bool kPark = true;
    static constexpr uint32_t kParkRows = 6;
    int park_row;
    __device__ __forceinline__ void park_prev_p(f3 v) { base[(park_row + 0) * kBlock] = (int32_t)fbits(v.x); base[(park_row + 1) * kBlock] = (int32_t)fbits(v.y); base[(park_row + 2) * kBlock] = (int32_t)fbits(v.z); }
    __device__ __forceinline__ f3 unpark_prev_p() const { return mk(bitsf((uint32_t)base[(park_row + 0) * kBlock]), bitsf((uint32_t)base[(park_row + 1) * kBlock]), bitsf((uint32_t)base[(park_row + 2) * kBlock])); }
    __device__ __forceinline__ void park_inc(uint64_t v) { base[(park_row + 3) * kBlock] = (int32_t)(uint32_t)v; base[(park_row + 4) * kBlock] = (int32_t)(uint32_t)(v >> 32); }
    __device__ __forceinline__ uint64_t unpark_inc() const { return (uint64_t)(uint32_t)base[(park_row + 3) * kBlock] | ((uint64_t)(uint32_t)base[(park_row + 4) * kBlock] << 32); }
    __device__ __forceinline__ void park_prev_pdf(float v) { base[(park_row + 5) * kBlock] = (int32_t)fbits(v); }
    __device__ __forceinline__ float unpark_prev_pdf() const { return bitsf((uint32_t)base[(park_row + 5) * kBlock]); }
#else
    static constexpr bool kPark = false;
    static constexpr uint32_t kParkRows = 0;
    __device__ __forceinline__ void park_prev_p(f3) {}
    __device__ __forceinline__ f3 unpark_prev_p() const { return mk(0, 0, 0); }
    __device__ __forceinline__ void park_inc(uint64_t) {}
    __device__ __forceinline__ uint64_t unpark_inc() const { return 0; }
    __device__ __forceinline__ void park_prev_pdf(float) {}
    __device__ __forceinline__ float unpark_prev_pdf() const { return 0.0f; }
#endif
#ifdef MTR_PROFILE_CYCLES
    unsigned long long t0, cyc[6];
#if MTR_PROFILE_CYCLES == 3
    __device__ __forceinline__ void prof_mark(int) {}
    __device__ __forceinline__ void prof_flat(int) {}
#elif MTR_PROFILE_CYCLES == 2
    __device__ __forceinline__ void prof_mark(int sec) { unsigned long long t = __builtin_readcyclecounter(); cyc[sec == 1 ? 1 : 3] += t - t0; t0 = t; }
    __device__ __forceinline__ void prof_flat(int sec) { unsigned long long t = __builtin_readcyclecounter(); cyc[sec] += t - t0; t0 = t; }
#else
    __device__ __forceinline__ void prof_mark(int sec) { unsigned long long t = __builtin_readcyclecounter(); cyc[sec] += t - t0; t0 = t; }
    __device__ __forceinline__ void prof_flat(int) {}
#endif
#else
    __device__ __forceinline__ void prof_mark(int) {}
    __device__ __forceinline__ void prof_flat(int) {}
#endif
#ifdef MTR_PROFILE_SIMT
    unsigned int ls[2], ws[2], wmax, wcalls;
    __device__ __forceinline__ void tail(unsigned int mine) {
        unsigned int mx = 0;
        for (int bit = 11; bit >= 0; --bit) { const unsigned int c = mx | (1u << bit); if (__ballot(mine >= c) != 0ull) mx = c; }
        unsigned long long m = __ballot(1);
        if ((int)(threadIdx.x & 63) == __ffsll((long long)m) - 1) { wmax += mx; wcalls += 1; }
    }
    __device__ __forceinline__ void count(int k) {
        ls[k]++;
        unsigned long long m = __ballot(1);
        if ((int)(threadIdx.x & 63) == __ffsll((long long)m) - 1) ws[k]++;
    }
#else
    __device__ __forceinline__ void count(int) {}
#endif
};
typedef LdsStackT<> LdsStack;

__device__ __forceinline__ void lds_add(float *p, float v)
{
    __hip_atomic_fetch_add(p, v, __ATOMIC_RELAXED, __HIP_MEMORY_SCOPE_WORKGROUP);
}

__device__ __forceinline__ void log_splat(const SplatLog &lg, uint32_t lane, uint32_t depth, uint32_t kind,
                                          uint32_t pixel, uint32_t bin, float r, float g, float b, float opl)
{
    unsigned long long i = atomicAdd(lg.count, 1ull);
    if (i < lg.cap) {
        uint32_t *R = lg.rec + 8 * i;
        R[0] = lane; R[1] = depth | (kind << 16); R[2] = pixel; R[3] = bin;
        R[4] = __float_as_uint(r); R[5] = __float_as_uint(g); R[6] = __float_as_uint(b); R[7] = __float_as_uint(opl);
    }
}

__device__ __forceinline__ void log_splat_fused(uint32_t lane, uint32_t depth, uint32_t kind,
                                                uint32_t pixel, uint32_t bin, float r, float g, float b, float opl)
{
    const SplatLog lg = kernarg_copy<SplatLog, true>(offsetof(FusedArgs, log));
    log_splat(lg, lane, depth, kind, pixel, bin, r, g, b, opl);
}

__device__ __forceinline__ unsigned long long splat_to_fixed(float v)
{
    long long q = __float2ll_rn(v * 4398046511104.0f);
    if (q == 0 && v != 0.0f) q = v > 0.0f ? 1 : -1;
    return (unsigned long long)q;
}
__device__ __forceinline__ float splat_from_fixed(unsigned long long q) { return __ll2float_rn((long long)q) * 2.2737367544323206e-13f; }
__device__ __forceinline__ float splat_fixed_limit(uint64_t n) { return 1048576.0f / (float)(n ? n : 1ull); }
__device__ __forceinline__ bool splat_fixed_unsafe(float r, float g, float b, float lim)
{
// ... 111 lines not shown
__device__ __forceinline__ void forget_dead(Path &p)
{
    forget_ray(p.ray); MTR_FORGET(p.beta.x); MTR_FORGET(p.beta.y); MTR_FORGET(p.beta.z);
    MTR_FORGET(p.prev_p.x); MTR_FORGET(p.prev_p.y); MTR_FORGET(p.prev_p.z); MTR_FORGET(p.prev_pdf); MTR_FORGET(p.dist); MTR_FORGET(p.depth);
    MTR_FORGET(p.rng.state);
}
#ifndef MTR_START_BLOCKS
#define MTR_START_BLOCKS 1
#endif
#ifndef MTR_START_CARRY
#define MTR_START_CARRY 0
#endif
typedef uint32_t StartRecWord __attribute__((ext_vector_type(4)));
typedef StartRecWord __attribute__((address_space(1))) *StartRecPtr;
struct StartTabArg { uint32_t lo, hi; };
template <class T, bool ON>
__device__ __forceinline__ T *kernarg_ptr(size_t offset, T *by_value)
{
    if constexpr (ON) { const StartTabArg w = kernarg_copy<StartTabArg, true>(offset); return (T *)(((uint64_t)w.hi << 32) | w.lo); }
    else return by_value;
}
__device__ __forceinline__ void path_resume(Path &p, const Film &f, const RenderConst &rc, uint32_t pixel, uint32_t s)
{
    const uint32_t py = fastdiv(pixel, rc.div_crop_w), px = pixel - f.crop_w * py;
    p.px = px + f.crop_x; p.py = py + f.crop_y; p.lane = pixel * rc.spp_total + s;
    p.beta = mk(1, 1, 1); p.L = mk(0, 0, 0); p.prev_p = mk(0, 0, 0);
    p.eta = 1.0f; p.dist = 0.0f; p.prev_pdf = 1.0f; p.depth = 0; p.prev_delta = 1;
}
#ifndef MTR_FUSED_MIN_WAVES
#define MTR_FUSED_MIN_WAVES 4
#endif
template <bool SCENE_LDS, bool HIST_LDS, bool NLOS, int MINW = MTR_FUSED_MIN_WAVES, bool PHASOR = false, bool FIXED = false, bool ROUGH = false, uint32_t TR = 0u>
__global__ void __launch_bounds__(kBlock, MINW) k_fused(const FusedArgs a)
{
    extern __shared__ __attribute__((aligned(16))) unsigned char smem[];
    const int tid = threadIdx.x;
    constexpr bool kLean = SCENE_LDS && HIST_LDS && !NLOS && !PHASOR && !FIXED && !ROUGH && flat_kind(TR) != 0;
    constexpr bool kPrimTable = flat_prim_table_on(kLean, flat_kind(TR) == 2);
    constexpr bool kStartBlocks = kLean && MTR_START_BLOCKS != 0;
    constexpr bool kCarryStart = kStartBlocks && (MTR_START_CARRY & 1) != 0;
#ifdef MTR_PROFILE_TAIL
    const unsigned long long t0_wall = wall_clock64();
#endif

    uint32_t off = 0;
    int32_t *s_stack = (int32_t *)(smem + off); off += (a.stack_rows + (NLOS ? 0u : LdsStack::kParkRows)) * kBlock * 4;
    unsigned long long *s_cnt = (unsigned long long *)(smem + off); off += 64;
    uint32_t *s_next = (uint32_t *)(s_cnt + 6);
    SceneView sv;
    sv.n_emitters = a.sc.n_ems; sv.n_slots = a.sc.n_slots;
    sv.samp_tris = a.sc.samp_tris; sv.samp_vn = a.sc.samp_vn; sv.face_pmf = a.sc.face_pmf; sv.face_cdf = a.sc.face_cdf; sv.vnormals = a.sc.vnormals;
    sv.texels = a.sc.texels; sv.tex_info = a.sc.tex_info; sv.uvs = a.sc.uvs;
    sv.flat_off = (uint32_t)(offsetof(FusedArgs, sc) + offsetof(SceneDev, flat));
    if (SCENE_LDS) {
        const uint32_t tree_bytes = a.sc.n_wnodes * (uint32_t)sizeof(WNode);
        if constexpr (kPrimTable) {
            static_assert(sizeof(TriPair) == kFlatPrimRecBytes && kFlatMaxBoxes * kFlatPrimFaces + kFlatPrimQuads <= 32u, "mtr_flat_prims.h");
            const uint32_t nb = a.sc.flat.n_boxes, n_ent = flat_prim_entries(nb);
            unsigned char *tab = smem + off; off += flat_prim_bytes(nb);
            constexpr uint32_t kWords = kFlatPrimEntryBytes / 4u;
            for (uint32_t w = tid; w < n_ent * kWords; w += kBlock) {
                const uint32_t e = w / kWords, j = w - kWords * e;
                const bool quad = e < kFlatPrimQuads;
                const uint32_t b = quad ? 0u : (e - kFlatPrimQuads) / kFlatPrimFaces, f = quad ? e : (e - kFlatPrimQuads) - kFlatPrimFaces * b;
                const uint32_t node = quad ? 0u : a.sc.flat.node0 + b;
                uint32_t v = 0u;
                if ((!quad || e < a.sc.flat.n_quads) && node < a.sc.n_wnodes) {
                    const uint32_t code = ~(uint32_t)a.sc.wnodes[node].ref[f];
                    const uint32_t first = (quad ? code & ~kLeafQuadBit : code) >> 2;
                    if (first < a.sc.n_slots) v = j < kWords - 1u ? ((const uint32_t *)(a.sc.tpairs + (first >> 1)))[j] : first;
                }
                *(uint32_t *)(tab + (j < kWords - 1u ? flat_prim_rec_off(e) + 4u * j : flat_prim_first_off(nb, e))) = v;
            }
        }
        WNode *n = (WNode *)(smem + off); off += align16(tree_bytes);
        TriPair *tg = (TriPair *)(smem + off); off += align16(a.sc.n_slots / 2 * sizeof(TriPair));
        TriShade *ts = (TriShade *)(smem + off); off += align16(a.sc.n_slots * sizeof(TriShade));
        mtr_material *mm = (mtr_material *)(smem + off); off += align16(a.sc.n_mats * sizeof(mtr_material));
        Emitter *ee = (Emitter *)(smem + off); off += align16(a.sc.n_ems * sizeof(Emitter));
        copy16(n, a.sc.wnodes, align16(tree_bytes), tid);
        copy16(tg, a.sc.tpairs, align16(a.sc.n_slots / 2 * sizeof(TriPair)), tid);
        copy16(ts, a.sc.tshade, align16(a.sc.n_slots * sizeof(TriShade)), tid);
        copy16(mm, a.sc.mats, align16(a.sc.n_mats * sizeof(mtr_material)), tid);
        copy16(ee, a.sc.ems, align16(a.sc.n_ems * sizeof(Emitter)), tid);
        sv.nodes = nullptr; sv.wnodes = n; sv.wnodes4 = nullptr; sv.wnodes8q = nullptr; sv.tpairs = tg; sv.tshade = ts; sv.mats = mm; sv.ems = ee;
        sv.node_pairs = true;
        __builtin_assume(sv.wnodes != nullptr);
    } else {
        sv.nodes = a.sc.nodes; sv.tpairs = a.sc.tpairs; sv.tshade = a.sc.tshade; sv.mats = a.sc.mats; sv.ems = a.sc.ems;
        sv.wnodes = nullptr; sv.wnodes4 = a.sc.wnodes4; sv.wnodes8q = a.sc.wnodes8q;
        sv.node_pairs = false;
    }
    const uint32_t K = a.G;
    float *s_steady = (float *)(smem + off); off += align16(K * 32);
    unsigned long long *s_steady64 = (unsigned long long *)s_steady;
    float *s_steady_ovf = (float *)(smem + off); if (FIXED) off += align16(K * 16);
    uint32_t *s_owner = (uint32_t *)(smem + off); off += align16(K * 4);
    uint32_t *s_done = (uint32_t *)(smem + off); off += align16(K * 4);
    float *s_hist = (float *)(smem + off);
    const uint32_t T = PHASOR ? 2u * a.film.n_freq : a.film.bins;
    constexpr bool kGrey = (TR & kTrGrey) != 0u;
    const uint32_t plane = kGrey ? 0u : K * T;

    if (tid < 6) s_cnt[tid] = 0ull;
    for (uint32_t k = tid; k < K; k += kBlock) s_done[k] = 0u;
    for (uint32_t k = tid; k < K * 8; k += kBlock) s_steady[k] = 0.0f;
    unsigned long long *s_hist64 = (unsigned long long *)s_hist;
    float *s_ovf = s_hist + 6u * plane;
    if (HIST_LDS) for (uint32_t k = tid; k < (kGrey ? K * T : (PHASOR ? 1u : (FIXED ? 9u : 3u)) * plane); k += kBlock) s_hist[k] = 0.0f;
    if (FIXED) for (uint32_t k = tid; k < K * 4; k += kBlock) s_steady_ovf[k] = 0.0f;

    LdsStackT<kLean> st; st.base = s_stack + tid; st.sp = 0;
#ifndef MTR_NO_PARK
    st.park_row = (int)a.stack_rows;
#endif
#ifdef MTR_PROFILE_SIMT
    st.ls[0] = st.ls[1] = st.ws[0] = st.ws[1] = 0; st.wmax = 0; st.wcalls = 0;
#endif
#ifdef MTR_PROFILE_CYCLES
    for (int k = 0; k < 6; ++k) st.cyc[k] = 0;
    st.t0 = __builtin_readcyclecounter();
#endif
    typedef typename std::conditional<kLean, uint32_t, unsigned long long>::type WaveCount;
    WaveCount w_closest = 0, w_shadow = 0, w_bounce = 0, w_paths = 0, w_splats = 0;
    auto drain_counters = [&]() {
        if ((tid & 63) == 0) {
            atomicAdd(&s_cnt[0], (unsigned long long)w_paths);
            atomicAdd(&s_cnt[2], (unsigned long long)w_shadow);
            atomicAdd(&s_cnt[3], (unsigned long long)w_splats);
            atomicAdd(&s_cnt[4], (unsigned long long)w_bounce);
        }
        w_paths = 0; w_shadow = 0; w_splats = 0; w_bounce = 0;
    };
#ifdef MTR_PROFILE_OCC
    unsigned long long occ_iter = 0, occ_alive = 0, occ_wait = 0;
    [[maybe_unused]] bool occ_ran = false, occ_need = false;
#endif
    uint32_t n_closest = 0, n_shadow = 0, n_splats = 0;

    uint32_t *s_chunk = s_next + 1;
    const uint32_t n_px_all = a.pixel_end - a.pixel_begin;
    if (tid == 0) { s_chunk[0] = 0u; s_chunk[1] = 0u; }
    for (;;) {
    __syncthreads();
    if (tid == 0 && a.n_bands && s_chunk[1] != 0u && s_chunk[0] < n_px_all) {
        __builtin_amdgcn_fence(__ATOMIC_RELEASE, "agent");
        uint32_t f = s_chunk[0];
        const uint32_t end = f + min(s_chunk[1], n_px_all - f);
        while (f < end) {
            const uint32_t bnd = min(f / a.band_px, a.n_bands - 1u);
            const bool last = bnd == a.n_bands - 1u;
            const uint32_t lim = last ? end : min(end, (bnd + 1u) * a.band_px), cnt = lim - f;
            const uint32_t in_band = last ? n_px_all - bnd * a.band_px : a.band_px;
            const uint32_t old = __hip_atomic_fetch_add(a.band_count + bnd, cnt, __ATOMIC_ACQ_REL, __HIP_MEMORY_SCOPE_AGENT);
            if (old + cnt == in_band) __hip_atomic_store(a.band_done + bnd, a.band_epoch, __ATOMIC_RELEASE, __HIP_MEMORY_SCOPE_SYSTEM);
            f = lim;
        }
    }
    if (tid == 0) {
        uint32_t *const ticket = kernarg_ptr<uint32_t, kStartBlocks>(offsetof(FusedArgs, ticket), a.ticket);
        const uint32_t seen = __hip_atomic_load(ticket, __ATOMIC_RELAXED, __HIP_MEMORY_SCOPE_AGENT);
        const uint32_t left = seen < n_px_all ? n_px_all - seen : 0u;
        uint32_t want = left / (2u * gridDim.x);
        want = want < 1u ? 1u : (want > a.chunk ? a.chunk : want);
        s_chunk[0] = atomicAdd(ticket, want); s_chunk[1] = want;
        *s_next = kBlock;
    }
    for (uint32_t k = tid; k < K; k += kBlock) s_owner[k] = k;
    __syncthreads();
    const uint32_t first = s_chunk[0];
// ... 74 lines not shown
        }
        if constexpr (kStartBlocks) {
            if (__ballot(want) == 0ull || __ballot(waiting) != 0ull) break;
            {
                const uint32_t wl = (uint32_t)tid & (kStartBlock - 1u);
                const bool fresh = blk_used == kStartFresh;
                if (fresh || blk_base < n_lanes) {
                    if (!fresh) {
                        uint32_t b = 0u;
                        if (wl == 0u) b = atomicAdd(s_next, kStartBlock);
                        blk_base = __builtin_amdgcn_readfirstlane(b);
                    }
                    blk_used = 0u;
                    const uint32_t fi = blk_base + wl;
                    {
                        const LoopArgs la = kernarg_copy<LoopArgs, kLean>(offsetof(FusedArgs, spp_begin));
                        const Camera cam_l = kernarg_copy<Camera, kLean>(offsetof(FusedArgs, cam));
                        const Film film_s = kernarg_copy<Film, kLean>(offsetof(FusedArgs, film));
                        const RenderConst rc_s = kernarg_copy<RenderConst, kLean>(offsetof(FusedArgs, rc));
                        const uint32_t fq = fastdiv(fi, la.div_spp);
                        Path t;
                        path_begin(t, cam_l, film_s, rc_s, pixel_of(fq), la.spp_begin + (fi - fq * la.spp_chunk));
                        const StartTabArg ta = kernarg_copy<StartTabArg, kLean>(offsetof(FusedArgs, start_tab));
                        const uint32_t wv = (uint32_t)tid / kStartBlock;
                        const StartRecPtr rec = (StartRecPtr)((((uint64_t)ta.hi << 32) | ta.lo) + start_rec_off(blockIdx.x, kBlock / kStartBlock, wv, wl));
                        rec[0] = StartRecWord{ fbits(t.ray.o.x), fbits(t.ray.o.y), fbits(t.ray.o.z), fbits(t.ray.d.x) };
                        rec[1] = StartRecWord{ fbits(t.ray.d.y), fbits(t.ray.d.z), fbits(t.ray.tmax), (uint32_t)t.rng.state };
                        rec[2] = StartRecWord{ (uint32_t)(t.rng.state >> 32), (uint32_t)t.rng.inc, (uint32_t)(t.rng.inc >> 32), 0u };
                    }
                    __builtin_amdgcn_fence(__ATOMIC_RELEASE, "wavefront");
                }
                const unsigned long long sm = __ballot(want);
                const uint32_t e = blk_used + __builtin_amdgcn_mbcnt_hi((uint32_t)(sm >> 32), __builtin_amdgcn_mbcnt_lo((uint32_t)sm, 0u));
                if (want) { i = blk_base + e; waiting = i < n_lanes; want = false; }
                blk_used = min(blk_used + (uint32_t)__popcll(sm), kStartBlock);
            }
        } else break;
        }
        st.prof_mark(2);
        if (__ballot(alive) == 0ull) {
            if (__ballot(waiting) == 0ull) break;
            __builtin_amdgcn_s_sleep(8);
            st.prof_mark(5);
            if constexpr (kLean && (MTR_PATH_STATE & 1) != 0) forget_dead(p);
            continue;
        }
        bool closes = false;
        bool ended = false;
#ifdef MTR_PROFILE_OCC
        occ_iter += 1;
#if MTR_PROFILE_OCC == 2
        occ_alive += occ_ran ? 1u : 0u; occ_wait += occ_need ? 1u : 0u; occ_ran = false; occ_need = false;
#elif MTR_PROFILE_OCC == 3
#else
        occ_alive += (uint32_t)__popcll(__ballot(alive)); occ_wait += (uint32_t)__popcll(__ballot(waiting));
#endif
#endif
        w_bounce += (uint32_t)__popcll(__ballot(alive));
        uint32_t did_shadow = 0u, did_splats = 0u;
        if (alive) {
            BounceStats bstat; bstat.closest = 0; bstat.shadow = 0;
            const bool unwarp = !NLOS && (a.rc.flags & MTR_FLAG_CAMERA_UNWARP) != 0u;
            Film film_l = a.film; RenderConst rc_l = a.rc;
            NlosConst nc_l = a.nlos;
            auto reload_nlos = [&]() {
                nc_l = kernarg_copy<NlosConst>(offsetof(FusedArgs, nlos));
                film_l = kernarg_copy<Film>(offsetof(FusedArgs, film)); rc_l = kernarg_copy<RenderConst>(offsetof(FusedArgs, rc));
            };
            auto refresh = [&](Path &pp, auto &) {
                uint32_t w = xy; asm volatile("" : "+v"(w));
                pp.px = w & 0xffffu; pp.py = w >> 16;
                if (!NLOS) { film_l = kernarg_copy<Film, kLean>(offsetof(FusedArgs, film)); rc_l = kernarg_copy<RenderConst, kLean>(offsetof(FusedArgs, rc)); }
                if constexpr (kLean && (MTR_BATCH & 2) != 0) { kernarg_pin(film_l); kernarg_pin(rc_l); }
#if defined(MTR_PROFILE_CYCLES) && MTR_PROFILE_CYCLES == 3
                if constexpr (kLean) {
                    typedef const volatile unsigned long long __attribute__((address_space(3))) *LdsWord;
                    const unsigned long long c0 = __builtin_readcyclecounter();
                    asm volatile("" :: "s"(c0));
                    const unsigned long long c1 = __builtin_readcyclecounter();
                    asm volatile("" :: "s"(c1));
                    const Film fr = kernarg_copy<Film, true>(offsetof(FusedArgs, film)); kernarg_pin(fr);
                    const unsigned long long c2 = __builtin_readcyclecounter();
                    asm volatile("" :: "s"(c2));
                    const unsigned long long c3 = __builtin_readcyclecounter();
                    asm volatile("" :: "s"(c3));
                    const unsigned long long w = *((LdsWord)(const char *)sv.wnodes + (tid & 1));
                    asm volatile("" :: "v"(w));
                    const unsigned long long c4 = __builtin_readcyclecounter();
                    st.cyc[0] += c2 - c1; st.cyc[1] += c4 - c3; st.cyc[2] += c1 - c0; st.cyc[3] += 1ull;
                }
#endif
            };
            if (PHASOR && NLOS) {
                LdsPhasorSinkNlos sink; sink.row = s_hist + slot * T;
                sink.film_w = a.film.width; sink.lane = p.lane; sink.n_splats = 0; sink.log = a.log;
                alive = nlos_bounce<ROUGH, TR>(p, sv, nc_l, film_l, rc_l, st, sink, bstat, reload_nlos);
                n_splats += sink.n_splats;
            } else if (PHASOR) {
                LdsPhasorSink sink; sink.row = s_hist + slot * T; sink.freq = a.film.freq; sink.n_freq = a.film.n_freq;
                sink.start_opl = a.film.start_opl; sink.film_w = a.film.width; sink.lane = p.lane; sink.n_splats = 0; sink.log = a.log;
                alive = path_bounce<ROUGH, TR>(p, sv, film_l, rc_l, st, sink, bstat, refresh, unwarp);
                did_splats = sink.n_splats;
            } else if (FIXED) {
                LdsFixedSink sink; sink.hist = s_hist64; sink.ovf = s_ovf; sink.plane = plane; sink.row = slot * T;
                sink.lim = a.fixed_lim; sink.dcap = a.fixed_dcap;
                sink.film_w = a.film.width; sink.lane = p.lane; sink.n_splats = 0; sink.log = a.log;
// ... 138 lines not shown
                        }
                        if (any) {
                            const float4 z = make_float4(0.0f, 0.0f, 0.0f, 0.0f);
                            *(float4 *)(h + t) = z; *(float4 *)(h + t + plane) = z; *(float4 *)(h + t + 2 * plane) = z;
                        }
                    }
                    for (uint32_t t = T4 + wl; t < T; t += 64u) {
                        float r = h[t], gc = h[t + plane], b = h[t + 2 * plane];
                        if (r != 0.0f || gc != 0.0f || b != 0.0f) {
                            float4 v = make_float4(0.0f, 0.0f, 0.0f, 0.0f);
                            if (!(a.rc.flags & MTR_FLAG_FILM_ZERO)) v = row[t];
                            v.x += r; v.y += gc; v.z += b;
                            row[t] = v;
                            h[t] = 0; h[t + plane] = 0; h[t + 2 * plane] = 0;
                        }
                    }
                }
                if (wl < 4) {
                    float v;
                    if (FIXED) { v = splat_from_fixed(s_steady64[4 * fs + wl]) + s_steady_ovf[4 * fs + wl]; s_steady64[4 * fs + wl] = 0ull; s_steady_ovf[4 * fs + wl] = 0.0f; }
                    else { v = s_steady[4 * fs + wl]; s_steady[4 * fs + wl] = 0.0f; }
                    if (wl == 3) v = (float)a.spp_chunk;
                    if (v != 0.0f) steady_out[fpix * 4u + wl] += v;
                }
            }
            if (wl == 0) {
                s_done[fs] = 0u;
                __hip_atomic_store(s_owner + fs, fq + K, __ATOMIC_RELEASE, __HIP_MEMORY_SCOPE_WORKGROUP);
            }
        }
        if (kLean && __builtin_expect(w_bounce >= 0x40000000u, 0)) drain_counters();
    }
    if (kLean) drain_counters();
    }
    __syncthreads();

    if (NLOS) {
        atomicAdd(&s_cnt[1], (unsigned long long)n_closest);
        atomicAdd(&s_cnt[2], (unsigned long long)n_shadow);
        atomicAdd(&s_cnt[3], (unsigned long long)n_splats);
    } else if (!kLean) w_closest += w_bounce;
    if (!kLean && (tid & 63) == 0) {
        atomicAdd(&s_cnt[0], w_paths);
        atomicAdd(&s_cnt[1], w_closest);
        atomicAdd(&s_cnt[2], w_shadow);
        atomicAdd(&s_cnt[3], w_splats);
        atomicAdd(&s_cnt[4], w_bounce);
    }
    __syncthreads();
    if (kLean && tid == 0) s_cnt[1] = s_cnt[4] + ((a.rc.flags & MTR_FLAG_CAMERA_UNWARP) ? s_cnt[0] : 0ull);
    if (kLean) __syncthreads();
    if (tid < 5 && a.counters) atomicAdd(&a.counters->paths + tid, s_cnt[tid]);
#ifdef MTR_PROFILE_OCC
    if ((tid & 63) == 0 && a.counters) {
        atomicAdd(&a.counters->splats_overflow, occ_iter); atomicAdd(&a.counters->r0, occ_alive); atomicAdd(&a.counters->r1, occ_wait);
    }
#endif
#ifdef MTR_PROFILE_TAIL
    if (tid == 0 && a.counters) {
        const unsigned long long t = wall_clock64();
        atomicMax(&a.counters->r0, ~(t - t0_wall));
        atomicMax(&a.counters->r1, t - t0_wall);
        atomicAdd(&a.counters->splats_overflow, t - t0_wall);
    }
#endif
#ifdef MTR_PROFILE_SIMT
    if (a.counters) {
        unsigned long long *c = &a.counters->splats_overflow;
        atomicAdd(c + 0, ((unsigned long long)st.ls[0] << 32) | st.ws[0]);
        atomicAdd(c + 1, ((unsigned long long)st.ls[1] << 32) | st.ws[1]);
        atomicAdd(c + 2, ((unsigned long long)st.wcalls << 32) | (unsigned long long)st.wmax);
    }
#endif
#ifdef MTR_PROFILE_CYCLES
    if ((tid & 63) == 0 && a.counters) {
        st.prof_mark(5);
        unsigned long long *c = &a.counters->splats_overflow;
#if MTR_PROFILE_CYCLES == 3
        atomicAdd(c + 0, st.cyc[0]); atomicAdd(c + 1, st.cyc[1]); atomicAdd(c + 2, (st.cyc[3] << 32) | ((st.cyc[2] >> 6) & 0xffffffffull));
#else
        atomicAdd(c + 0, ((st.cyc[0] >> 10) << 32) | (st.cyc[1] >> 10));
        atomicAdd(c + 1, ((st.cyc[2] >> 10) << 32) | (st.cyc[3] >> 10));
        atomicAdd(c + 2, ((st.cyc[4] >> 10) << 32) | (st.cyc[5] >> 10));
#endif
    }
#endif
}

static uint32_t scene_lds_bytes(const SceneDev &sc)
{
    return align16(sc.n_wnodes * sizeof(WNode)) + align16(sc.n_slots / 2 * sizeof(TriPair)) +
           align16(sc.n_slots * sizeof(TriShade)) + align16(sc.n_mats * sizeof(mtr_material)) +
           align16(sc.n_ems * sizeof(Emitter));
}

uint32_t fused_chunk(uint32_t n_pixels, uint32_t spp_chunk, uint32_t grid)
{
    uint32_t chunk = (32768u + spp_chunk - 1u) / (spp_chunk ? spp_chunk : 1u);
    const uint32_t c_bal = (uint32_t)((unsigned long long)n_pixels / (2ull * (unsigned long long)(grid ? grid : 1u)));
    if (chunk > c_bal) chunk = c_bal;
    if (chunk < 1u) chunk = 1u;
    return fused_chunk_cap(chunk, spp_chunk);
}

static bool fused_lean_flat_quads(bool nlos_on, uint32_t n_freq, const FusedConfig &cfg)
{
    return !nlos_on && !n_freq && !cfg.rough && !cfg.fixed && cfg.scene_lds && cfg.hist_lds && (cfg.traits & kTrFlatGeneral) == kTrFlatFlags;
}
static uint32_t fused_prim_table_bytes(const SceneDev &sc, bool nlos_on, uint32_t n_freq, const FusedConfig &cfg)
// ... 482 lines not shown
```

mitransient_amd/csrc/mtr_scene_host.cpp:

```cpp
#include "mtr_scene_host.h"
#include "mtr_polar.h"
#include <chrono>
#include <cstdio>
#include "mtr_knobs.h"
#include <cstring>
#include <cmath>

namespace mtr {

Film film_from_desc(const mtr_film_desc &d)
{
    Film f;
    f.width = d.width; f.height = d.height; f.crop_w = d.crop_width; f.crop_h = d.crop_height;
    f.crop_x = d.crop_offset_x; f.crop_y = d.crop_offset_y;
    f.tbins = d.temporal_bins;
    f.lasers = (d.laser_scan_width && d.laser_scan_height) ? d.laser_scan_width * d.laser_scan_height : 1u;
    f.bins = f.tbins * f.lasers;
    f.start_opl = d.start_opl; f.bin_width = d.bin_width_opl;
    f.n_freq = d.n_frequencies; f.freq = d.frequencies;
    if (f.n_freq) { f.tbins = 1; f.lasers = 1; f.bins = 1; }
    return f;
}

static double tri_area_d(const float *v)
{
    double e1[3] = { (double)v[3] - v[0], (double)v[4] - v[1], (double)v[5] - v[2] };
    double e2[3] = { (double)v[6] - v[0], (double)v[7] - v[1], (double)v[8] - v[2] };
    double c[3] = { e1[1] * e2[2] - e1[2] * e2[1], e1[2] * e2[0] - e1[0] * e2[2], e1[0] * e2[1] - e1[1] * e2[0] };
    return 0.5 * sqrt(c[0] * c[0] + c[1] * c[1] + c[2] * c[2]);
}

static double fill_mesh_tables(const float *tri_verts, uint32_t first, uint32_t n, float *pmf, float *cdf, q4 *quads)
{
    double a = 0.0, acc = 0.0;
    for (uint32_t t = 0; t < n; ++t) a += tri_area_d(tri_verts + 9 * (size_t)(first + t));
    for (uint32_t t = 0; t < n; ++t) {
        const float *v = tri_verts + 9 * (size_t)(first + t);
        const double at = tri_area_d(v);
        acc += at;
        pmf[first + t] = (float)(at / a);
        cdf[first + t] = (float)(acc / a);
        const f3 p0 = mk(v[0], v[1], v[2]), e1 = mk(v[3], v[4], v[5]) - p0, e2 = mk(v[6], v[7], v[8]) - p0;
        const f3 nn = normalize(cross(e1, e2));
        q4 *q = &quads[3 * (size_t)(first + t)];
        q[0] = q4{ p0.x, p0.y, p0.z, e1.x }; q[1] = q4{ e1.y, e1.z, e2.x, e2.y }; q[2] = q4{ e2.z, nn.x, nn.y, nn.z };
    }
    return a;
}

static void fill_mesh_normals(const float *tri_normals, uint32_t first, uint32_t n, uint32_t n_total, std::vector<q4> &quads)
{
    if (!tri_normals) return;
    for (uint32_t t = 0; t < n; ++t) {
        const float *vn = tri_normals + 9 * (size_t)(first + t);
        bool smooth = false;
        for (int k = 0; k < 9; ++k) smooth = smooth || vn[k] != 0.0f;
        if (!smooth) continue;
        if (quads.empty()) quads.assign(3 * (size_t)n_total, q4{ 0, 0, 0, 0 });
        for (int k = 0; k < 3; ++k) quads[3 * (size_t)(first + t) + k] = q4{ vn[3 * k], vn[3 * k + 1], vn[3 * k + 2], k == 0 ? 1.0f : 0.0f };
    }
}

static f3 coordinate_system_s(f3 n)
{
    const float sign = copysignf(1.0f, n.z);
    const float a = -(1.0f / (sign + n.z));
    const float b = (n.x * n.y) * a;
    const bool neg = sign_neg(n.z);
    const float x = (n.x * n.x) * a, nx = -n.x;
    return mk((neg ? -x : x) + 1.0f, neg ? -b : b, neg ? -nx : nx);
}
static void sh_frame_from(f3 n, f3 dp_du, f3 &s, f3 &t) { sh_frame_of(n, dp_du, s, t); }
static void rect_to_object(const float c[3], const float du[3], const float dv[3], float rx[4], float ry[4], float rz[4])
{
    const double a[3] = { du[0], du[1], du[2] }, b[3] = { dv[0], dv[1], dv[2] }, o[3] = { c[0], c[1], c[2] };
    double n[3] = { a[1] * b[2] - a[2] * b[1], a[2] * b[0] - a[0] * b[2], a[0] * b[1] - a[1] * b[0] };
    const double ln = sqrt(n[0] * n[0] + n[1] * n[1] + n[2] * n[2]);
    n[0] /= ln; n[1] /= ln; n[2] /= ln;
    const double bn[3] = { b[1] * n[2] - b[2] * n[1], b[2] * n[0] - b[0] * n[2], b[0] * n[1] - b[1] * n[0] };
    const double na[3] = { n[1] * a[2] - n[2] * a[1], n[2] * a[0] - n[0] * a[2], n[0] * a[1] - n[1] * a[0] };
    const double da = a[0] * bn[0] + a[1] * bn[1] + a[2] * bn[2], db = b[0] * na[0] + b[1] * na[1] + b[2] * na[2];
    const double X[3] = { bn[0] / da, bn[1] / da, bn[2] / da }, Y[3] = { na[0] / db, na[1] / db, na[2] / db };
    for (int k = 0; k < 3; ++k) { rx[k] = (float)X[k]; ry[k] = (float)Y[k]; rz[k] = (float)n[k]; }
    rx[3] = (float)(-(X[0] * o[0] + X[1] * o[1] + X[2] * o[2]));
    ry[3] = (float)(-(Y[0] * o[0] + Y[1] * o[1] + Y[2] * o[2]));
    rz[3] = (float)(-(n[0] * o[0] + n[1] * o[1] + n[2] * o[2]));
}
static bool object_space_of(const float tw[12], float inv[12], bool *axis_aligned = nullptr)
{
    const double m[9] = { tw[0], tw[1], tw[2], tw[4], tw[5], tw[6], tw[8], tw[9], tw[10] }, t[3] = { tw[3], tw[7], tw[11] };
    double big = 0.0;
    for (double x : m) big = fmax(big, fabs(x));
    bool aligned = true;
    for (int r = 0; r < 3; ++r) {
        int nz = 0;
        for (int c = 0; c < 3; ++c) nz += fabs(m[3 * r + c]) > 1e-6 * big ? 1 : 0;
        aligned = aligned && nz <= 1;
    }
    const double det = m[0] * (m[4] * m[8] - m[5] * m[7]) - m[1] * (m[3] * m[8] - m[5] * m[6]) + m[2] * (m[3] * m[7] - m[4] * m[6]);
    if (axis_aligned) *axis_aligned = aligned;
    if ((aligned && !axis_aligned) || !(fabs(det) > 1e-30)) return false;
    const double c[9] = { m[4] * m[8] - m[5] * m[7], m[2] * m[7] - m[1] * m[8], m[1] * m[5] - m[2] * m[4],
                          m[5] * m[6] - m[3] * m[8], m[0] * m[8] - m[2] * m[6], m[2] * m[3] - m[0] * m[5],
                          m[3] * m[7] - m[4] * m[6], m[1] * m[6] - m[0] * m[7], m[0] * m[4] - m[1] * m[3] };
    for (int r = 0; r < 3; ++r) {
        double row[3] = { c[3 * r] / det, c[3 * r + 1] / det, c[3 * r + 2] / det };
        for (int k = 0; k < 3; ++k) inv[4 * r + k] = (float)row[k];
        inv[4 * r + 3] = (float)(-(row[0] * t[0] + row[1] * t[1] + row[2] * t[2]));
    }
    return true;
}

const char *derive_scene(const mtr_scene_desc &d, HostScene &s)
{
    if (d.n_tris && (!d.tri_verts || !d.tri_material || !d.tri_emitter)) return "triangle arrays missing";
    if (d.n_materials > 0xffffu || d.n_emitters > 0x7fffu) return "too many materials/emitters";
    for (uint32_t i = 0; i < d.n_tris; ++i) {
        if (d.tri_material[i] >= d.n_materials) return "triangle references an unknown material";
        if (d.tri_emitter[i] >= (int32_t)d.n_emitters) return "triangle references an unknown emitter";
    }
    for (uint32_t i = 0; i < d.n_materials; ++i)
        if (d.materials[i].type > MTR_BSDF_PLASTIC) return "unknown BSDF type";
    for (uint32_t i = 0; i < d.n_materials; ++i) {
        if (bsdf_is_rough(d.materials[i].type) && d.materials[i].type != MTR_BSDF_PLASTIC && !(d.materials[i].alpha > 0.0f)) return "rough BSDF: alpha must be positive";
        if (bsdf_is_rough(d.materials[i].type) && d.materials[i].type != MTR_BSDF_PLASTIC && (d.materials[i].flags & MTR_MAT_ANISOTROPIC) &&
            !(rough_alpha_v(d.materials[i]) > 0.0f)) return "rough BSDF: alpha_v of an anisotropic lobe must be positive";
// ... 300 lines not shown
    hs.polar_ok = hs.texels.empty();
    bool lobes = false;
    for (uint32_t i = 0; i < d.n_materials; ++i) {
        if (!polar_bsdf_supported(d.materials[i].type)) hs.polar_ok = false;
        if (bsdf_is_lobe(d.materials[i].type)) lobes = true;
    }
    for (const Emitter &e : hs.ems) if (e.angular || e.kind >= kEmPoint) hs.polar_ok = false;
    hs.needs_ext = lobes || !hs.vnormals.empty() || !hs.texels.empty();
    hs.traits = 0u;
    if (!hs.needs_ext) {
        bool diffuse_only = d.n_materials > 0;
        for (uint32_t i = 0; i < d.n_materials; ++i)
            if (d.materials[i].type != MTR_BSDF_DIFFUSE || (d.materials[i].flags & MTR_MAT_TWOSIDED)) diffuse_only = false;
        if (diffuse_only) hs.traits |= kTrDiffuse;
        if (d.n_emitters == 1 && hs.ems[0].kind == kEmRect && !hs.ems[0].angular && !hs.has_sphere) hs.traits |= kTrOneRectEmitter;
        bool leaf_pairs = hs.has_wide;
        for (const WNode &n : hs.wnodes)
            for (uint32_t k = 0; k < n.count; ++k) {
                const uint32_t code = ~(uint32_t)n.ref[k];
                if (n.ref[k] < 0 && !(code & kLeafQuadBit) && (code & 3u) + 1u > 2u) leaf_pairs = false;
            }
        if (leaf_pairs && !hs.has_sphere) hs.traits |= kTrLeafPair;
    } else if (!lobes) hs.traits |= kTrNoLobes;
    hs.grey_scene = scene_is_grey(hs.has_sphere, d.materials, d.n_materials, hs.ems.data(), d.n_emitters, !hs.texels.empty());
    if (hs.grey_scene) hs.traits |= kTrGrey;
    memset(&hs.flat, 0, sizeof hs.flat);
    if (hs.has_wide && !hs.wnodes.empty() && hs.wide_levels <= 2 && !hs.has_sphere && !mtr::knob("MTR_NO_FLAT")) {
        const WNode &root = hs.wnodes[0];
        bool flat = root.flags == 0u && root.count >= 1u;
        uint32_t n_inner = 0u, prim_mask = 0u;
        for (uint32_t k = 0; flat && k < root.count; ++k) {
            const int32_t ref = root.ref[k];
            if (k < root.n_quads) { flat = ref < 0 && ((~(uint32_t)ref) & kLeafQuadBit) != 0u; prim_mask |= 1u << k; }
            else if (ref < 0) { flat = ((~(uint32_t)ref) & kLeafQuadBit) == 0u; prim_mask |= 1u << k; }
            else {
                flat = ref == (int32_t)(1u + n_inner) && (size_t)ref < hs.wnodes.size() && hs.wnodes[ref].flags == 3u && hs.wnodes[ref].count == 6u;
                ++n_inner;
            }
        }
        flat = flat && n_inner <= kFlatMaxBoxes;
        if (flat) {
            FlatTop &ft = hs.flat;
            ft.n_quads = root.n_quads; ft.n_boxes = n_inner; ft.node0 = 1u; ft.prim_mask = prim_mask;
            for (uint32_t b = 0; b < ft.n_boxes; ++b) {
                const float *x = hs.wnodes[1u + b].xf;
                memcpy(ft.xf[b], x, 12 * sizeof(float));
                for (int k = 0; k < 3; ++k) ft.xf[b][12 + k] = (fabsf(x[4 * k]) + fabsf(x[4 * k + 1]) + fabsf(x[4 * k + 2])) * 1.000001f;
                ft.xf[b][15] = 0.0f;
            }
            hs.traits |= kTrFlatTop;
            if (prim_mask >> root.n_quads) hs.traits |= kTrFlatLeaves;
        }
    }
}

const char *derive_nlos(const mtr_scene_desc &d, HostNlos &o)
{
    const mtr_nlos_desc *n = d.nlos;
    if (!n) return "no NLOS description";
    if (n->capture_type != MTR_CAPTURE_SINGLE && n->capture_type != MTR_CAPTURE_CONFOCAL &&
        n->capture_type != MTR_CAPTURE_EXHAUSTIVE)
        return "capture_type must be Single, Confocal or Exhaustive";
    const bool exhaustive = n->capture_type == MTR_CAPTURE_EXHAUSTIVE;
    if (exhaustive && !(d.film.laser_scan_width && d.film.laser_scan_height))
        return "Exhaustive capture needs an exhaustive_scan film (laser_scan_width / laser_scan_height > 0)";
    if (exhaustive && (n->flags & MTR_NLOS_FORCE_EQUAL_GRIDS) &&
        (d.film.laser_scan_width != d.film.width || d.film.laser_scan_height != d.film.height))
        return "Sensor and laser scan resolution must be equal if force_equal_illumination_scanning is set to True";
    const bool camera_sensor = n->relay_shape == MTR_NLOS_NO_RELAY;
    if (camera_sensor && (d.film.crop_width != d.film.width || d.film.crop_height != d.film.height))
        return "NLOS with a perspective sensor: crop windows are not supported";
    if (!n->shapes || n->n_shapes == 0 || (!camera_sensor && n->relay_shape >= n->n_shapes)) return "NLOS: bad shape table";
    if (!camera_sensor && !n->shapes[n->relay_shape].is_rectangle) return "NLOS: the relay wall must be a rectangle";
    if (d.n_emitters != 0) return "NLOS: area emitters are not supported next to the projector";
    uint32_t covered = 0;
    for (uint32_t s = 0; s < n->n_shapes; ++s) {
        if (n->shapes[s].first_tri != covered) return "NLOS: shapes must tile the triangle array in order";
        covered += n->shapes[s].n_tris;
    }
    if (covered != d.n_tris) return "NLOS: shapes must cover every triangle";
    NlosConst &k = o.k;
    k.sensor_origin = mk(n->sensor_origin[0], n->sensor_origin[1], n->sensor_origin[2]);
    k.camera_sensor = camera_sensor ? 1u : 0u;
    memcpy(k.cam.s2c, d.camera.sample_to_camera, sizeof k.cam.s2c);
    memcpy(k.cam.tw, d.camera.to_world, sizeof k.cam.tw);
    k.cam.near_clip = d.camera.near_clip; k.cam.far_clip = d.camera.far_clip;
    k.inv_w = 1.0f / (float)d.film.width; k.inv_h = 1.0f / (float)d.film.height;
    k.sensor_confocal = n->sensor_is_confocal ? 1u : 0u;
    k.sensor_target = ld3(n->sensor_target);
    if (n->sensor_is_confocal && (camera_sensor || d.film.width != 1 || d.film.height != 1))
        return "Confocal configuration requires a nlos_capture_meter with a film of size [1,1]";
    if (!camera_sensor) {
        const mtr_shape &rw = n->shapes[n->relay_shape];
        k.w_center = ld3(rw.center); k.w_du = ld3(rw.du); k.w_dv = ld3(rw.dv);
    } else { k.w_center = mk(0, 0, 0); k.w_du = mk(1, 0, 0); k.w_dv = mk(0, 1, 0); }
    const float *T = n->laser_to_world;
    k.l_origin = mk(T[3], T[7], T[11]);
    k.l_forward = mk(T[2], T[6], T[10]);
    const float inv[9] = { T[0], T[4], T[8], T[1], T[5], T[9], T[2], T[6], T[10] };
    memcpy(k.l_inv, inv, sizeof inv);
    k.l_cot = (float)(1.0 / tan(0.5 * (double)n->laser_fov * 3.14159265358979323846 / 180.0));
    k.l_scale = n->laser_scale;
    k.l_irr = ld3(n->laser_irradiance);
    k.capture_type = n->capture_type; k.flags = n->flags; k.filter_depth = n->filter_depth; k.n_shapes = n->n_shapes;
    k.film_w = d.film.width; k.film_h = d.film.height;
    k.laser_w = exhaustive ? d.film.laser_scan_width : 0u; k.laser_h = exhaustive ? d.film.laser_scan_height : 0u;
// ... 69 lines not shown
```

mitransient_amd/csrc/mtr_scene_host.h:

```cpp
#pragma once
#include <vector>
#include "mtr_core.h"
#include "mtr_bvh.h"
#include "mtr_nlos.h"

namespace mtr {

struct HostScene {
    std::vector<Node> nodes;
    std::vector<WNode> wnodes;
    std::vector<QNode8> wnodes8q;
    std::vector<QNode4> wnodes4;
    bool has_wide = false;
    std::vector<TriPair> tpairs;
    std::vector<TriShade> tshade;
    std::vector<uint32_t> slot_orig;
    std::vector<mtr_material> mats;
    std::vector<Emitter> ems;
    std::vector<q4> samp_tris;
    std::vector<q4> samp_vn;
    std::vector<q4> vnormals;
    std::vector<q4> texels; std::vector<q4> tex_info; std::vector<q4> uvs;
    std::vector<float> face_pmf, face_cdf;
    uint32_t bvh_depth = 0, n_leaves = 0;
    uint32_t wide_levels = 0, wide4_levels = 0, wide8q_levels = 0;
    Camera cam{};
    Film film{};
    uint32_t traits = 0;
    bool needs_ext = false;
    bool polar_ok = false;
    bool grey_scene = false;
    bool has_sphere = false;
    FlatTop flat{};
};

inline bool bsdf_is_lobe(uint32_t type) { return bsdf_is_rough(type) || type == MTR_BSDF_THINDIELECTRIC; }
bool colours_are_grey(const mtr_material *mats, uint32_t n_mats, const Emitter *ems, uint32_t n_ems, bool textured);
inline bool scene_is_grey(bool has_sphere, const mtr_material *mats, uint32_t n_mats, const Emitter *ems, uint32_t n_ems, bool textured)
{
    return !has_sphere && colours_are_grey(mats, n_mats, ems, n_ems, textured);
}
void classify_scene(const mtr_scene_desc &d, HostScene &s);
uint32_t traits_with_laser(uint32_t traits, bool grey_scene, const float laser_irradiance[3]);

uint32_t tint_slot_table(const mtr_material *mats, uint32_t n_mats, int32_t *slots);

struct HostNlos {
    std::vector<NlosShape> shapes;
    std::vector<float> shape_pmf, shape_cdf, face_pmf, face_cdf;
    std::vector<q4> hg_tris;
    std::vector<q4> hg_vn;
    NlosConst k{};
};
const char *derive_nlos(const mtr_scene_desc &d, HostNlos &out);

Film film_from_desc(const mtr_film_desc &d);
const char *derive_scene(const mtr_scene_desc &d, HostScene &out);
RenderConst make_render_const(const mtr_render_params &p, const Film &f, uint32_t n_emitters);

}
```

mitransient_amd/integrators/common.py:

```python
from __future__ import annotations

import ctypes as C
from typing import Tuple

from .. import _cabi, variant
from ..films.transient_hdr_film import TransientHDRFilm
from ..runtime import get_context
from ..scene import Properties
from ..tensor import TensorXf


def _dual_tangent(v):
    try:
        import torch
        if not isinstance(v, torch.Tensor):
            return None
        return torch.autograd.forward_ad.unpack_dual(v).tangent
    except Exception:
        return None


def _wants_grad(v):
    return bool(getattr(v, "requires_grad", False)) or _dual_tangent(v) is not None


class _Seed:
    requires_grad = True

    def __init__(self, shape):
        self.shape = tuple(shape)


_MODES = {"auto": _cabi.MTR_MODE_AUTO, "fused": _cabi.MTR_MODE_FUSED, "wavefront": _cabi.MTR_MODE_WAVEFRONT,
          "samples": _cabi.MTR_MODE_SAMPLES}

RADIANCEMETER_DEFAULTS_TO_SAMPLES = True


class TransientADIntegrator:
    def __init__(self, props: Properties):
        max_depth = int(props.get("max_depth", 6))
        if max_depth < 0 and max_depth != -1:
            raise Exception("\"max_depth\" must be set to -1 (infinite) or a value >= 0")
        self.max_depth = max_depth if max_depth != -1 else 0xFFFFFFFF
        self.rr_depth = int(props.get("rr_depth", 5))
        if self.rr_depth <= 0:
            raise Exception("\"rr_depth\" must be set to a value greater than zero!")
        self.hide_emitters = bool(props.get("hide_emitters", False))
        self.camera_unwarp = bool(props.get("camera_unwarp", False))
        self.discard_direct_light = bool(props.get("discard_direct_light", False))
        _ = props.get("gaussian_stddev", 0.5)
        _ = props.get("temporal_filter", "")
        _ = props.get("block_size", 0)
        self.pcg_initseq_plus_lane = bool(props.get("amd_pcg_initseq_plus_lane", False))
        self.pcg_tea64 = bool(props.get("amd_pcg_tea64", False))
        self.deterministic = bool(props.get("amd_deterministic", False))
        self.direct_develop = bool(props.get("amd_direct_develop", True))
        self.reserve_cus = int(props.get("amd_reserve_cus", 0))
        self.mode = _cabi.MTR_MODE_AUTO
        m = props.get("amd_mode", None)
        if m is not None:
            self.mode = _MODES[m]
        self.max_wavefront_size = 2 ** 32
        self.pass_wavefront_size = 2 ** 26 - 1
        self.last_counters = None
        self.last_times = None
        self.total_counters = None
        self.total_times = None
        self.collect_stats = False

    @property
    def amd_mode(self):
        return {v: k for k, v in _MODES.items()}[int(self.mode)]

    @amd_mode.setter
    def amd_mode(self, m):
        self.mode = _MODES[m]

    def aov_names(self):
        return []

    def prepare(self, scene, sensor, seed, spp, aovs, _direct_develop=False):
        film = sensor.film()
        if hasattr(film, "direct_develop"):
            film.direct_develop = bool(_direct_develop)
        sampler = sensor.sampler().clone()
        if spp != 0:
            sampler.set_sample_count(spp)
        spp = sampler.sample_count()
        sampler.set_samples_per_wavefront(spp)
        film_size = film.crop_size()
        self.total_counters, self.total_times = None, None
        n_pixels = film_size[0] * film_size[1]
        wavefront_size = n_pixels * spp
        if wavefront_size > self.max_wavefront_size and int(self.pass_wavefront_size / n_pixels) == 0:
            raise Exception("Your film is too big. Please make it smaller.")
        film.prepare(aovs)
        return self._pass_samplers(sensor, sampler, seed, spp, n_pixels)

    def _pass_samplers(self, sensor, sampler, seed, spp, n_pixels):
        wavefront_size = n_pixels * spp
        if wavefront_size <= self.max_wavefront_size:
            sampler.seed(seed, wavefront_size)
            return [(sampler, spp)]
        spp_per_pass = int(self.pass_wavefront_size / n_pixels)
        if spp_per_pass == 0:
            raise Exception("Your film is too big. Please make it smaller.")
        needs_remainder = spp % spp_per_pass != 0
        num_passes = spp // spp_per_pass + 1 * needs_remainder
        sampler.set_sample_count(num_passes)
        sampler.set_samples_per_wavefront(num_passes)
        sampler.seed(seed, num_passes)
        import numpy as np
        seeds = (sampler.next_1d_first() * np.float32(2 ** 32)).astype(np.uint32)

        def sampler_per_pass(i):
            spp_i = spp % spp_per_pass if (needs_remainder and i == num_passes - 1) else spp_per_pass
            clone = sensor.sampler().clone()
            clone.set_sample_count(spp_i)
            clone.set_samples_per_wavefront(spp_i)
            clone.seed(int(seeds[i]), n_pixels * spp_i)
            return clone, spp_i

        return [sampler_per_pass(i) for i in range(num_passes)]

    def check_transient_(self, scene, sensor):
        if isinstance(sensor, int):
            sensor = scene.sensors()[sensor]
        if not isinstance(sensor.film(), TransientHDRFilm):
            raise AssertionError("The film of the sensor must be of type transient_hdr_film or phasor_hdr_film")
        from ..sensors import RadianceMeter
        if isinstance(sensor, RadianceMeter) and variant.is_polarized():
            raise ValueError(f"{variant.get()}: a radiancemeter renders with the unpolarized variants only")

    def _samples_by_default(self, sensor):
        from ..sensors import RadianceMeter
        return RADIANCEMETER_DEFAULTS_TO_SAMPLES and int(self.mode) == _cabi.MTR_MODE_AUTO and isinstance(sensor, RadianceMeter)

    def add_transient_f(self, film, pos, ray_weight, sample_scale):
        return (lambda spec, distance, wavelengths=None, active=None, laser_x=None, laser_y=None:
                film.add_transient_data(pos, distance, wavelengths, spec * sample_scale, ray_weight, active))

    def _flags(self):
        f = 0
        if self.camera_unwarp:
            f |= _cabi.MTR_FLAG_CAMERA_UNWARP
        if self.discard_direct_light:
            f |= _cabi.MTR_FLAG_DISCARD_DIRECT_LIGHT
        if self.pcg_initseq_plus_lane:
            f |= _cabi.MTR_FLAG_PCG_INITSEQ_PLUS_LANE
        if self.pcg_tea64:
            f |= _cabi.MTR_FLAG_PCG_TEA64
        if self.deterministic:
            if variant.is_polarized():
                raise ValueError(f"{variant.get()}: amd_deterministic is not available with polarization "
                                 "(the Stokes film is summed with f32 atomics; render without amd_deterministic)")
            f |= _cabi.MTR_FLAG_DETERMINISTIC
        if variant.is_polarized():
            f |= _cabi.MTR_FLAG_POLARIZED
        return f

    def render_params(self, film, seed_value, spp_total, spp_begin=0, spp_end=None,
                      pixel_begin=0, pixel_end=None, spp_scale=0) -> _cabi.mtr_render_params:
        p = _cabi.mtr_render_params()
        p.spp_total = spp_total
        p.spp_scale = spp_scale
        p.spp_begin = spp_begin
        p.spp_end = spp_total if spp_end is None else spp_end
        cw, ch = film.crop_size()
        p.pixel_begin = pixel_begin
        p.pixel_end = cw * ch if pixel_end is None else pixel_end
        p.seed = seed_value & 0xFFFFFFFF
        p.max_depth = -1 if self.max_depth >= 0x7FFFFFFF else int(self.max_depth)
        p.rr_depth = int(self.rr_depth)
        p.flags = self._flags()
        p.mode = int(self.mode)
        p.reserve_cus = max(0, int(self.reserve_cus))
        return p

    def render(self, scene, sensor=0, seed=0, spp=0, develop=True, evaluate=True,
               progress_callback=None, spp_range=None, pixel_range=None) -> Tuple[TensorXf, TensorXf]:
        if not develop:
            raise Exception("develop=True must be specified when invoking AD integrators")
        if isinstance(sensor, int):
            sensor = scene.sensors()[sensor]
        film = sensor.film()
        self.check_transient_(scene, sensor)
        direct = spp_range is None and pixel_range is None and self._direct_develop_ok(scene, sensor, spp)
        samplers_spps = self.prepare(scene=scene, sensor=sensor, seed=seed, spp=spp, aovs=self.aov_names(), _direct_develop=direct)
        total_spp = sum(s for _, s in samplers_spps)
        self.accumulate(scene, sensor, samplers_spps, total_spp, spp_range, pixel_range, progress_callback)
        return film.develop()

    def _direct_develop_ok(self, scene, sensor, spp):
        film = sensor.film()
        if not self.direct_develop or type(film) is not TransientHDRFilm:
            return False
        if int(self.mode) == _cabi.MTR_MODE_SAMPLES or self._samples_by_default(sensor):
            return False
        if tuple(film.crop_size()) != tuple(film.size()) or tuple(film.crop_offset()) != (0, 0):
            return False
        spp = spp if spp != 0 else sensor.sampler().sample_count()
        W, H = film.size()
        if W * H * spp > self.max_wavefront_size:
            return False
        ctx = get_context()
        handle = scene.gpu_handle(ctx, sensor)
        params = self.render_params(film, 0, spp)
        mode, ok = C.c_uint32(0), C.c_uint32(0)
        ctx.check(ctx.lib.mtr_render_plan(handle, C.byref(params), C.byref(mode), C.byref(ok)), "mtr_render_plan")
        return bool(ok.value)

# ... 321 lines not shown
```

mitransient_amd/mi.py:

```python
from __future__ import annotations

import ctypes as C
import os
from typing import Any, Dict

from . import _cabi, plugins
from . import variant as _variant_mod
from .scene import Properties, flatten_scene, film_desc_from
from .sensors import IndependentSampler, PerspectiveSensor, RadianceMeter
from .transform import ScalarTransform4f
from .tensor import TensorXf

Transform4f = ScalarTransform4f


def variant():
    return _variant_mod.get()


POLARIZED_VARIANTS = ("llvm_ad_mono_polarized", "cuda_ad_mono_polarized")


def set_variant(*names):
    for n in names:
# ... 377 lines not shown
            return
        self.ensure_own_records([key])
        self.param_values_[key] = [float(np.float32(x)) for x in v]
        if key.endswith(".intensity.value") and key[:-len(".intensity.value")] in self.lights_:
            self.lights_[key[:-len(".intensity.value")]].intensity = np.asarray(self.param_values_[key], np.float64)
        lib = _cabi.load_library()
        for skey, sd in self._data.items():
            self._apply_params(sd)
            a = np.array([[sd.materials[i].a[c] for c in range(3)] for i in range(max(1, sd.n_materials))], np.float32)
            r = np.array([[sd.emitters[i].radiance[c] for c in range(3)] for i in range(max(1, sd.n_emitters))], np.float32)
            for hkey in [h for h in self._handles if h[0] == skey]:
                ok = lib.mtr_scene_set_colors(self._handles[hkey], C.c_void_p(a.ctypes.data), C.c_void_p(r.ctypes.data)) == 0
                if ok and sd.tint_params and sd.nlos is None:
                    t = np.array([[[m.c[c] for c in range(3)], [m.c2[c] for c in range(3)]]
                                  for m in sd.materials[:max(1, sd.n_materials)]], np.float32)
                    t0, t1 = np.ascontiguousarray(t[:, 0]), np.ascontiguousarray(t[:, 1])
                    ok = lib.mtr_scene_set_tints(self._handles[hkey], C.c_void_p(t0.ctypes.data), C.c_void_p(t1.ctypes.data)) == 0
                if not ok:
                    lib.mtr_scene_destroy(self._handles.pop(hkey))
                    self._nlos_fp.pop(hkey, None)

    def gpu_handle(self, ctx, sensor=0):
        if isinstance(sensor, int):
            sensor = self.sensors_[sensor]
        key = (id(sensor), ctx.device_index)
        sd = self.data(sensor)
        if key not in self._handles:
            h = C.c_void_p()
            d = sd.desc()
            ctx.check(ctx.lib.mtr_scene_create(ctx.handle, C.byref(d), C.byref(h)), "mtr_scene_create")
            self._handles[key] = h
        h = self._handles[key]
        fd = sd.film
        ctx.check(ctx.lib.mtr_scene_set_film(h, C.byref(fd)), "mtr_scene_set_film")
        if sd.nlos is not None:
            d = sd.desc()
            n = sd.nlos
            n_val = type(n).from_buffer_copy(n)
            n_val.shapes = None
            fp = (bytes(n_val), bytes(memoryview(sd.shapes)),
                  int(fd.width), int(fd.height), int(fd.laser_scan_width), int(fd.laser_scan_height))
            if self._nlos_fp.get(key) != fp:
                ctx.check(ctx.lib.mtr_scene_set_nlos(h, d.nlos), "mtr_scene_set_nlos")
                self._nlos_fp[key] = fp
        return h

    def gpu_traits(self, sensor=0):
        from .runtime import get_context
        ctx = get_context()
        t = C.c_uint32(0)
        ctx.check(ctx.lib.mtr_scene_traits(self.gpu_handle(ctx, sensor), C.byref(t)), "mtr_scene_traits")
        return int(t.value)

    def __del__(self):
        try:
            lib = _cabi.load_library()
            for h in self._handles.values():
                lib.mtr_scene_destroy(h)
        except Exception:
            pass


def load_dict(d: Dict[str, Any], base_dir: str = ".", approximate_materials: bool = False):
    t = d.get("type")
    if t == "scene":
        return Scene(d, base_dir, approximate_materials)
    if t in _SHAPE_TYPES:
        return _load_shape(d)
    if t == "projector":
        from .emitters import Projector
        e = Projector(Properties("projector", d))
        e.dict_ = d
        return e
    if t in ("point", "spot"):
        from .emitters import make_delta_emitter
        return make_delta_emitter(d)
    from . import integrators as _i, films as _f
    if str(t).endswith("_film"):
        return plugins.create_film(t, Properties(t, d))
    if t in ("nlos_capture_meter", "perspective", "radiancemeter"):
        return _make_sensor(d)
    if str(t).startswith("transient"):
        return plugins.create_integrator(t, Properties(t, d))
    raise ValueError(f"load_dict(): unsupported top-level plugin type \"{t}\"")


def _tea32(v0, v1, rounds=4):
    M = 0xFFFFFFFF
    v0, v1, s = v0 & M, v1 & M, 0
    for _ in range(rounds):
        s = (s + 0x9E3779B9) & M
        v0 = (v0 + ((((v1 << 4) & M) + 0xA341316C) ^ ((v1 + s) & M) ^ ((v1 >> 5) + 0xC8013EA4))) & M
        v1 = (v1 + ((((v0 << 4) & M) + 0xAD90777D) ^ ((v0 + s) & M) ^ ((v0 >> 5) + 0x7E95761E))) & M
    return v0


def _grad_values(params):
    if not params:
        return []
    from .integrators.common import _wants_grad
    return [(k, v) for k, v in params.items() if _wants_grad(v)]


def render(scene: Scene, params=None, sensor=0, integrator=None, seed=0, seed_grad=0, spp=0, spp_grad=0):
    integ = integrator or scene.integrator()
    grads = _grad_values(params)
# ... 106 lines not shown
```

Baseline: 44810 Mray/s.

## Skip shadow-ray leaf tests using a conservative convex-hull classification of the scene

Adds a host-side classification of the flat top-level rectangles into a convex hull of bounding planes plus an emitter plane, with conservative float error margins. Shadow rays whose origin lies strictly inside the hull (wave-uniform) skip all rectangle slab tests, and rays near only the emitter's side test just the emitter child. This targets the leaf intersection cost of shadow rays in the Cornell box. It adds per-ray plane evaluations and kernarg reads, plus a risk of missed occlusion if the error bounds are wrong.

New measurement: 46160 Mray/s, median of 6. +3.0%, better.

```diff
diff --git a/__graft_entry__.py b/__graft_entry__.py
--- a/__graft_entry__.py
+++ b/__graft_entry__.py
@@ -24,7 +24,7 @@
             os.path.join(ROOT, "mitransient_amd", "csrc", "mtr_scene_host.cpp"),
             os.path.join(ROOT, "mitransient_amd", "csrc", "mtr_bvh.cpp")]
     deps = srcs + [os.path.join(ROOT, "mitransient_amd", "csrc", h) for h in
-                   ("mtr_core.h", "mtr_scene_host.h", "mtr_bvh.h", "mtr_knobs.h")]
+                   ("mtr_core.h", "mtr_shadow_hull.h", "mtr_scene_host.h", "mtr_bvh.h", "mtr_knobs.h")]
     if os.path.exists(out) and all(os.path.getmtime(out) >= os.path.getmtime(d) for d in deps):
         return out
     _run(["g++", "-O2", "-std=c++17", "-fPIC", "-shared", "-ffp-contract=off", "-fno-fast-math", "-mfma", "-DMTR_EXPERIMENTS",
diff --git a/include/mitransient_amd.h b/include/mitransient_amd.h
--- a/include/mitransient_amd.h
+++ b/include/mitransient_amd.h
@@ -164,6 +164,8 @@
        MTR_FLAG_PCG_INITSEQ_PLUS_LANE = 8u ,
        MTR_FLAG_POLARIZED = 256u,
        MTR_FLAG_PCG_TEA64 = 128u            };
+#define MTR_SHADOW_HULL_SHIFT 16u
+#define MTR_SHADOW_HULL_OFF   0xffffu
 
 enum { MTR_MODE_AUTO = 0,
        MTR_MODE_FUSED = 1,
@@ -241,6 +243,7 @@
 #define MTR_TRAIT_NO_LOBES        32u
 #define MTR_TRAIT_GREY            64u
 int  mtr_scene_traits(const mtr_scene *, uint32_t *traits);
+int  mtr_scene_shadow_hull(const mtr_scene *, uint32_t *n_hull_rectangles);
 int  mtr_scene_set_colors(mtr_scene *, const float *material_a, const float *emitter_radiance);
 int  mtr_scene_set_texture(mtr_scene *, uint32_t index, const float *rgb);
 int  mtr_scene_texture_layout(const mtr_scene *, uint32_t index, uint32_t *first_texel, uint32_t *width, uint32_t *height);
diff --git a/mitransient_amd/_cabi.py b/mitransient_amd/_cabi.py
--- a/mitransient_amd/_cabi.py
+++ b/mitransient_amd/_cabi.py
@@ -19,6 +19,7 @@
 MTR_FLAG_FILM_ZERO = 4
 MTR_FLAG_PCG_INITSEQ_PLUS_LANE = 8
 MTR_FLAG_PCG_TEA64 = 128
+MTR_SHADOW_HULL_SHIFT, MTR_SHADOW_HULL_OFF = 16, 0xFFFF
 MTR_FLAG_KEEP_COUNTERS = 16
 MTR_FLAG_DETERMINISTIC = 32
 MTR_FLAG_DEVELOPED_ROWS = 64
@@ -166,7 +167,7 @@
 
 EXPORTS = [
     "mtr_abi_version", "mtr_ctx_create", "mtr_ctx_destroy", "mtr_ctx_set_stream", "mtr_last_error",
-    "mtr_scene_create", "mtr_scene_destroy", "mtr_scene_set_film", "mtr_scene_set_nlos", "mtr_scene_bvh_info", "mtr_scene_traits",
+    "mtr_scene_create", "mtr_scene_destroy", "mtr_scene_set_film", "mtr_scene_set_nlos", "mtr_scene_bvh_info", "mtr_scene_traits", "mtr_scene_shadow_hull",
     "mtr_ctx_trim", "mtr_film_clear", "mtr_render", "mtr_render_plan", "mtr_counters_reset", "mtr_counters_read", "mtr_film_develop", "mtr_splat_add", "mtr_debug_set_splat_log",
     "mtr_render_grad", "mtr_scene_set_colors",
     "mtr_render_grad_tex", "mtr_render_grad_tex_tier", "mtr_scene_set_texture", "mtr_scene_texture_layout",
@@ -208,6 +209,7 @@
     lib.mtr_scene_set_nlos.argtypes = [vp, C.POINTER(mtr_nlos_desc)]
     lib.mtr_scene_bvh_info.argtypes = [vp, C.POINTER(C.c_uint32), C.POINTER(C.c_uint32), C.POINTER(C.c_uint32)]
     lib.mtr_scene_traits.argtypes = [vp, C.POINTER(C.c_uint32)]
+    lib.mtr_scene_shadow_hull.argtypes = [vp, C.POINTER(C.c_uint32)]
     lib.mtr_counters_read.argtypes = [vp, C.POINTER(mtr_counters)]
     lib.mtr_counters_reset.argtypes = [vp]
     lib.mtr_ctx_trim.argtypes = [vp]
diff --git a/mitransient_amd/csrc/mtr_api.hip b/mitransient_amd/csrc/mtr_api.hip
--- a/mitransient_amd/csrc/mtr_api.hip
+++ b/mitransient_amd/csrc/mtr_api.hip
@@ -86,6 +86,7 @@
     uint32_t n_texels = 0;
     std::vector<void *> allocs;
     SplatLog log{ nullptr, 0, nullptr };
+    ShadowHull hull{};
 };
 
 static thread_local std::string g_err;
@@ -224,7 +225,7 @@
     s->dev.n_nodes = (uint32_t)hs.nodes.size(); s->dev.n_slots = (uint32_t)hs.tshade.size();
     s->dev.n_mats = d->n_materials; s->dev.n_ems = d->n_emitters;
     s->polar_ok = hs.polar_ok; s->grey_scene = hs.grey_scene; s->has_sphere = hs.has_sphere;
-    s->dev.has_rough = hs.needs_ext ? 1u : 0u; s->dev.traits = hs.traits; s->dev.flat = hs.flat;
+    s->dev.has_rough = hs.needs_ext ? 1u : 0u; s->dev.traits = hs.traits; s->dev.flat = hs.flat; s->hull = hs.hull;
     s->dev.bvh_depth = hs.bvh_depth; s->n_leaves = hs.n_leaves;
     s->dev.wide_levels = hs.wide_levels; s->dev.wide4_levels = hs.wide4_levels; s->dev.wide8q_levels = hs.wide8q_levels;
     s->tri_verts.assign(d->tri_verts, d->tri_verts + 9 * (size_t)d->n_tris);
@@ -450,6 +451,13 @@
                   MTR_TRAIT_FLAT_TOP == kTrFlatTop && MTR_TRAIT_FLAT_LEAVES == kTrFlatLeaves && MTR_TRAIT_NO_LOBES == kTrNoLobes &&
                   MTR_TRAIT_GREY == kTrGrey, "public trait bits");
     *traits = s->dev.traits;
+    return MTR_OK;
+}
+
+int mtr_scene_shadow_hull(const mtr_scene *s, uint32_t *n_hull_rectangles)
+{
+    if (!s || !n_hull_rectangles) return MTR_ERR_INVALID;
+    *n_hull_rectangles = s->hull.count;
     return MTR_OK;
 }
 
@@ -816,6 +824,10 @@
     a.film_out = t4; a.steady_out = s4;
     a.counters = c->d_counters;
     a.log = s->log;
+    {
+        const uint32_t v = p->flags >> MTR_SHADOW_HULL_SHIFT;
+        a.hull = shadow_hull_with_margin(s->hull, v == MTR_SHADOW_HULL_OFF ? 0.0f : (float)(v + 1u));
+    }
     a.nlos_on = s->nlos.on ? 1u : 0u;
     if (s->nlos.on) {
         a.nlos = s->nlos.k;
diff --git a/mitransient_amd/csrc/mtr_core.h b/mitransient_amd/csrc/mtr_core.h
--- a/mitransient_amd/csrc/mtr_core.h
+++ b/mitransient_amd/csrc/mtr_core.h
@@ -13,6 +13,7 @@
 #include <math.h>
 #include "../../include/mitransient_amd.h"
 #include "mtr_flat_prims.h"
+#include "mtr_shadow_hull.h"
 
 #if defined(__HIPCC__)
 #include <hip/hip_runtime.h>
@@ -340,6 +341,7 @@
     const q4 *vnormals;
     const q4 *texels; const q4 *tex_info; const q4 *uvs;
     uint32_t flat_off;
+    uint32_t hull_off;
 };
 
 MTR_HD uint32_t distr_sample_reuse(const float *cdf, const float *pmf, uint32_t n, float value, float &reused, float &pmf_out)
@@ -964,13 +966,14 @@
 
 template <class S, class = void> struct stack_one_kernarg_base { static constexpr bool value = false; };
 template <class S> struct stack_one_kernarg_base<S, decltype((void)S::kOneKernargBase)> { static constexpr bool value = S::kOneKernargBase; };
+template <class S, class = void> struct stack_shadow_hull { static constexpr bool value = false; };
+template <class S> struct stack_shadow_hull<S, decltype((void)S::kShadowHull)> { static constexpr bool value = S::kShadowHull; };
 
 #if defined(__HIP_DEVICE_COMPILE__)
-template <bool ANY_HIT, uint32_t J, bool BATCH = false>
-__device__ __forceinline__ void flat_slab_pair(const f3 id, const f3 noid, const float tb, const uint32_t sel0, const uint32_t sel1, const uint32_t sel2,
-                                               const char *root, const bool p0, const bool p1, uint32_t &qm, uint32_t &key1, uint32_t &key2)
-{
-    const char *pb = root + 48u * J;
+template <bool ANY_HIT, bool BATCH = false>
+__device__ __forceinline__ void flat_slab_pair_at(const f3 id, const f3 noid, const float tb, const uint32_t sel0, const uint32_t sel1, const uint32_t sel2,
+                                                  const char *pb, const uint32_t j2, const bool p0, const bool p1, uint32_t &qm, uint32_t &key1, uint32_t &key2)
+{
     f2 nx, fx, ny, fy, nz, fz;
     if constexpr (BATCH) {
         const f2 pnx = *(const f2 *)(pb + sel0), pfx = *(const f2 *)(pb + (sel0 ^ 8u));
@@ -990,13 +993,19 @@
     const float tf1 = fminf(fminf(fx.y, fy.y), fminf(fz.y, tb));
     const bool h0 = (tn0 <= tf0) && p0;
     const bool h1 = (tn1 <= tf1) && p1;
-    qm |= (h0 ? 1u : 0u) << (2u * J);
-    qm |= (h1 ? 2u : 0u) << (2u * J);
+    qm |= (h0 ? 1u : 0u) << j2;
+    qm |= (h1 ? 2u : 0u) << j2;
     if (!ANY_HIT) {
-        const uint32_t ka = h0 ? ((fbits(tn0) & ~7u) | (2u * J)) : 0xffffffffu, kb = h1 ? ((fbits(tn1) & ~7u) | (2u * J + 1u)) : 0xffffffffu;
+        const uint32_t ka = h0 ? ((fbits(tn0) & ~7u) | j2) : 0xffffffffu, kb = h1 ? ((fbits(tn1) & ~7u) | (j2 + 1u)) : 0xffffffffu;
         key2 = min(key2, max(key1, ka)); key1 = min(key1, ka);
         key2 = min(key2, max(key1, kb)); key1 = min(key1, kb);
     }
+}
+template <bool ANY_HIT, uint32_t J, bool BATCH = false>
+__device__ __forceinline__ void flat_slab_pair(const f3 id, const f3 noid, const float tb, const uint32_t sel0, const uint32_t sel1, const uint32_t sel2,
+                                               const char *root, const bool p0, const bool p1, uint32_t &qm, uint32_t &key1, uint32_t &key2)
+{
+    flat_slab_pair_at<ANY_HIT, BATCH>(id, noid, tb, sel0, sel1, sel2, root + 48u * J, 2u * J, p0, p1, qm, key1, key2);
 }
 __device__ __forceinline__ RecByValue flat_prim_fetch(const char *root, const uint32_t n_boxes, const uint32_t entry)
 {
@@ -1007,9 +1016,10 @@
     r.first = *(const uint32_t *)(tab + flat_prim_first_off(n_boxes, entry));
     return r;
 }
-template <bool ANY_HIT, bool ONE_PAIR, bool TOP_LEAVES, class Stack>
+template <bool ANY_HIT, bool ONE_PAIR, bool TOP_LEAVES, bool HULL = false, class Stack>
 __device__ __forceinline__ Hit flat_walk_device(const SceneView &sc, const f3 o, const f3 d, const float tmax, Stack &st)
 {
+    static_assert(!HULL || (ANY_HIT && !TOP_LEAVES), "SHADOW HULL: shadow rays over a top level of rectangles and boxes");
     typedef WNode N;
     Trav tr;
     const RayByValue ray{ o, d, tmax };
@@ -1021,6 +1031,7 @@
     constexpr bool kOneBase = stack_one_kernarg_base<Stack>::value;
     constexpr bool kTable = flat_prim_table_on(kOneBase, TOP_LEAVES);
     const FlatHdr fh =kernarg_copy<FlatHdr, kOneBase>(sc.flat_off);
+    constexpr int kProfKind = ANY_HIT ? 8 : 0;
     bool live = true;
     uint32_t fm = 0u;
     const float omax = fmaxf(fmaxf(fabsf(o.x), fabsf(o.y)), fabsf(o.z));
@@ -1034,7 +1045,7 @@
         const f3 id = mk(safe_rcp(dl.x), safe_rcp(dl.y), safe_rcp(dl.z));
         fm |= box_select(box_mag_bound(A, B, C, S, omax), ol, dl, id, tmax) << (6u * b);
     }
-    st.prof_flat(0);
+    st.prof_flat(kProfKind + 0);
     while (__ballot(live && fm != 0u) != 0ull) {
         if (live && fm != 0u) {
             const uint32_t k = (uint32_t)__builtin_ctz(fm);
@@ -1051,8 +1062,44 @@
             }
         }
     }
-    st.prof_flat(5);
-    if (__ballot(live) != 0ull) {
+    st.prof_flat(kProfKind + 5);
+    uint32_t tier = 0u, e_child = 0u;
+    bool risky_e = false;
+    if constexpr (HULL) {
+        if (__ballot(live) != 0ull) {
+            struct Head { uint32_t count, e_child; float e_delta, pad; float e_row[4]; float delta[kHullRows]; };
+            struct Rows4 { float row[4][4]; };
+            struct Rows2 { float row[2][4]; };
+            static_assert(sizeof(Head) == offsetof(ShadowHull, row) && kHullRows == 8u, "the block in four reads");
+            const Head hh = kernarg_copy<Head, kOneBase>(sc.hull_off);
+            if (hh.count != 0u) {
+                const Rows4 ra = kernarg_copy<Rows4, kOneBase>(sc.hull_off + sizeof(Head));
+                bool risky_h = false;
+                for (uint32_t k = 0; k < 4u; ++k) risky_h |= !(hull_side(ra.row[k], o.x, o.y, o.z) >= hh.delta[k]);
+                if (hh.count > 4u) {
+                    const Rows2 rb = kernarg_copy<Rows2, kOneBase>(sc.hull_off + sizeof(Head) + sizeof(Rows4));
+                    for (uint32_t k = 0; k < 2u; ++k) risky_h |= !(hull_side(rb.row[k], o.x, o.y, o.z) >= hh.delta[4u + k]);
+                }
+                if (hh.count > 6u) {
+                    const Rows2 rc = kernarg_copy<Rows2, kOneBase>(sc.hull_off + sizeof(Head) + sizeof(Rows4) + sizeof(Rows2));
+                    for (uint32_t k = 0; k < 2u; ++k) risky_h |= !(hull_side(rc.row[k], o.x, o.y, o.z) >= hh.delta[6u + k]);
+                }
+                risky_e = !(hull_side(hh.e_row, o.x, o.y, o.z) >= hh.e_delta);
+                e_child = hh.e_child;
+                const bool any_h = __ballot(live && risky_h) != 0ull, any_e = __ballot(live && risky_e) != 0ull;
+                tier = any_h ? 0u : (any_e ? 1u : 2u);
+#if defined(MTR_PROFILE_OCC) && MTR_PROFILE_OCC == 4
+                if (any_h) st.occ_hull(3);
+                if (any_e) st.occ_hull(4);
+#endif
+            }
+        }
+#if defined(MTR_PROFILE_OCC) && MTR_PROFILE_OCC == 4
+        st.occ_hull(0);
+        if (tier != 2u && __ballot(live) != 0ull) st.occ_hull(1);
+#endif
+    }
+    if ((!HULL || tier != 2u) && __ballot(live) != 0ull) {
         const f3 id = mk(safe_rcp(d.x), safe_rcp(d.y), safe_rcp(d.z));
         const f3 noid = mk(-(o.x * id.x), -(o.y * id.y), -(o.z * id.z));
         const uint32_t sel0 = id.x < 0.0f ? 8u : 0u, sel1 = 16u + (id.y < 0.0f ? 8u : 0u), sel2 = 32u + (id.z < 0.0f ? 8u : 0u);
@@ -1062,7 +1109,11 @@
 #define MTR_FLAT_SLAB_PAIR(J) flat_slab_pair<ANY_HIT, J, kOneBase && (MTR_BATCH & 1) != 0>(id, noid, tb, sel0, sel1, sel2, root, \
             TOP_LEAVES ? ((fh.prim_mask >> (2u * J)) & 1u) != 0u : 2u * J < fh.n_quads, \
             TOP_LEAVES ? ((fh.prim_mask >> (2u * J + 1u)) & 1u) != 0u : 2u * J + 1u < fh.n_quads, qm, key1, key2)
-        if (TOP_LEAVES) {
+        if (HULL && tier == 1u) {
+            flat_slab_pair_at<ANY_HIT, kOneBase && (MTR_BATCH & 1) != 0>(id, noid, tb, sel0, sel1, sel2, root + 48u * (e_child >> 1), e_child & ~1u,
+                                                                         (e_child & 1u) == 0u, (e_child & 1u) != 0u, qm, key1, key2);
+            if (!risky_e) qm = 0u;
+        } else if (TOP_LEAVES) {
             MTR_FLAT_SLAB_PAIR(0u);
             if (fh.prim_mask > 3u) MTR_FLAT_SLAB_PAIR(1u);
             if (fh.prim_mask > 15u) MTR_FLAT_SLAB_PAIR(2u);
@@ -1073,8 +1124,11 @@
         }
 #undef MTR_FLAT_SLAB_PAIR
         if (!live) qm = 0u;
-        st.prof_flat(2);
+        st.prof_flat(kProfKind + 2);
         for (uint32_t it = 0; __ballot(qm != 0u) != 0ull; ++it) {
+#if defined(MTR_PROFILE_OCC) && MTR_PROFILE_OCC == 4
+            if (HULL && it == 0u) st.occ_hull(2);
+#endif
             if (qm != 0u) {
                 const uint32_t k = (!ANY_HIT && it == 0u) ? (key1 & 7u) : (uint32_t)__builtin_ctz(qm);
                 qm &= ~(1u << k);
@@ -1091,16 +1145,16 @@
             }
         }
     }
-    st.prof_flat(4);
+    st.prof_flat(kProfKind + 4);
     return tr.h;
 }
 #endif
 
-template <bool ANY_HIT, bool ONE_PAIR = false, int FLAT = 0, bool SPH = !ONE_PAIR && FLAT == 0, class Stack>
+template <bool ANY_HIT, bool ONE_PAIR = false, int FLAT = 0, bool SPH = !ONE_PAIR && FLAT == 0, bool HULL = false, class Stack>
 MTR_HD Hit traverse(const SceneView &sc, f3 o, f3 d, float tmax, Stack &st)
 {
 #if defined(__HIP_DEVICE_COMPILE__)
-    if (FLAT) return flat_walk_device<ANY_HIT, ONE_PAIR, FLAT == 2>(sc, o, d, tmax, st);
+    if (FLAT) return flat_walk_device<ANY_HIT, ONE_PAIR, FLAT == 2, HULL && FLAT == 1>(sc, o, d, tmax, st);
 #endif
     Trav tr;
     trav_init(tr, sc, o, d, tmax, st);
@@ -1857,6 +1911,21 @@
     if (sign_neg(dot(sn, dir))) mag = -mag;
     return fma3(sn, mag, sp);
 }
+MTR_HD f3 rect_emitter_point(const Emitter &E, float u1, float u2)
+{
+    const float a = fmaf(u1, 2.0f, -1.0f), b = fmaf(u2, 2.0f, -1.0f);
+    return mk(fmaf(E.du[0], a, fmaf(E.dv[0], b, E.center[0])),
+              fmaf(E.du[1], a, fmaf(E.dv[1], b, E.center[1])),
+              fmaf(E.du[2], a, fmaf(E.dv[2], b, E.center[2])));
+}
+MTR_HD Ray shadow_ray_to(f3 sp, f3 gn, f3 ep)
+{
+    const f3 so = offset_point(sp, gn, ep - sp);
+    const f3 sd = ep - so;
+    const float sdist = sqrtf(dot(sd, sd));
+    Ray r; r.o = so; r.d = sd / sdist; r.tmax = sdist * (1.0f - kShadowEps);
+    return r;
+}
 
 MTR_HD bool sphere_ref_outside(const Emitter &E, float dc2)
 {
@@ -1999,10 +2068,7 @@
         else if (!kOneRect && E.kind == kEmMesh) {
             mesh_sample_position(sc.samp_tris, sc.face_cdf, sc.face_pmf, E.first_tri, E.n_tris, u1, u2, ep, en, ROUGH ? sc.samp_vn : nullptr);
         } else {
-            float a = fmaf(u1, 2.0f, -1.0f), b = fmaf(u2, 2.0f, -1.0f);
-            ep = mk(fmaf(E.du[0], a, fmaf(E.dv[0], b, E.center[0])),
-                    fmaf(E.du[1], a, fmaf(E.dv[1], b, E.center[1])),
-                    fmaf(E.du[2], a, fmaf(E.dv[2], b, E.center[2])));
+            ep = rect_emitter_point(E, u1, u2);
             en = ld3(E.n);
         }
         f3 dd = ep - c.sp;
@@ -2025,10 +2091,7 @@
                 f3 wo = mk(dot(dd, c.ss), dot(dd, c.stt), dot(dd, c.sn));
                 f3 wi_e = c.wi;
                 if (!kDiff && (mat.flags & MTR_MAT_TWOSIDED) && wi_e.z < 0.0f) { wi_e.z = -wi_e.z; wo.z = -wo.z; }
-                f3 so = offset_point(c.sp, c.gn, ep - c.sp);
-                f3 sd = ep - so;
-                float sdist = sqrtf(dot(sd, sd));
-                shadow.o = so; shadow.d = sd / sdist; shadow.tmax = sdist * (1.0f - kShadowEps);
+                shadow = shadow_ray_to(c.sp, c.gn, ep);
                 pd.has_shadow = 1u;
                 if constexpr (LEAN && (MTR_PATH_STATE & 2) != 0) { pd.Lr = mk(0, 0, 0); pd.opl = 0.0f; }
                 if (lobes_on<ROUGH, TR>() && bsdf_is_rough(mat.type)) {
@@ -2140,7 +2203,8 @@
     bool occluded = false;
     if (pd.has_shadow) {
         stats.shadow++;
-        Hit sh = traverse<true, (TR & kTrLeafPair) != 0u, flat_kind(TR), tr_spheres(TR)>(sc, shadow.o, shadow.d, shadow.tmax, st);
+        constexpr bool kHull = stack_shadow_hull<Stack>::value && flat_kind(TR) == 1 && (TR & kTrOneRectEmitter) != 0u;
+        Hit sh = traverse<true, (TR & kTrLeafPair) != 0u, flat_kind(TR), tr_spheres(TR), kHull>(sc, shadow.o, shadow.d, shadow.tmax, st);
         occluded = sh.prim >= 0;
     }
     st.prof_mark(0);
diff --git a/mitransient_amd/csrc/mtr_kernels.h b/mitransient_amd/csrc/mtr_kernels.h
--- a/mitransient_amd/csrc/mtr_kernels.h
+++ b/mitransient_amd/csrc/mtr_kernels.h
@@ -148,6 +148,7 @@
     uint32_t *band_count, *band_done;
     NlosConst nlos;
     unsigned char *start_tab;
+    ShadowHull hull;
 };
 
 struct FusedConfig { int stack; bool scene_lds; bool hist_lds; bool fixed; bool rough; size_t lds_bytes; int grid; int per_cu; uint32_t traits; };
diff --git a/mitransient_amd/csrc/mtr_kernels.hip b/mitransient_amd/csrc/mtr_kernels.hip
--- a/mitransient_amd/csrc/mtr_kernels.hip
+++ b/mitransient_amd/csrc/mtr_kernels.hip
@@ -11,6 +11,7 @@
 template <bool ONE_BASE = false>
 struct LdsStackT {
     static constexpr bool kOneKernargBase = ONE_BASE;
+    static constexpr bool kShadowHull = true;
     int32_t *base;
     int sp;
     __device__ __forceinline__ void reset() { sp = 0; }
@@ -42,9 +43,9 @@
 #if MTR_PROFILE_CYCLES == 3
     __device__ __forceinline__ void prof_mark(int) {}
     __device__ __forceinline__ void prof_flat(int) {}
-#elif MTR_PROFILE_CYCLES == 2
+#elif MTR_PROFILE_CYCLES == 2 || MTR_PROFILE_CYCLES == 4
     __device__ __forceinline__ void prof_mark(int sec) { unsigned long long t = __builtin_readcyclecounter(); cyc[sec == 1 ? 1 : 3] += t - t0; t0 = t; }
-    __device__ __forceinline__ void prof_flat(int sec) { unsigned long long t = __builtin_readcyclecounter(); cyc[sec] += t - t0; t0 = t; }
+    __device__ __forceinline__ void prof_flat(int sec) { unsigned long long t = __builtin_readcyclecounter(); cyc[MTR_PROFILE_CYCLES == 2 ? (sec & 7) : (sec >= 8 ? sec - 8 : 3)] += t - t0; t0 = t; }
 #else
     __device__ __forceinline__ void prof_mark(int sec) { unsigned long long t = __builtin_readcyclecounter(); cyc[sec] += t - t0; t0 = t; }
     __device__ __forceinline__ void prof_flat(int) {}
@@ -52,6 +53,10 @@
 #else
     __device__ __forceinline__ void prof_mark(int) {}
     __device__ __forceinline__ void prof_flat(int) {}
+#endif
+#if defined(MTR_PROFILE_OCC) && MTR_PROFILE_OCC == 4
+    unsigned int hull_n[5];
+    __device__ __forceinline__ void occ_hull(int k) { const unsigned long long m = __ballot(1); if ((int)(threadIdx.x & 63) == __ffsll((long long)m) - 1) hull_n[k] += 1u; }
 #endif
 #ifdef MTR_PROFILE_SIMT
     unsigned int ls[2], ws[2], wmax, wcalls;
@@ -269,6 +274,7 @@
     sv.samp_tris = a.sc.samp_tris; sv.samp_vn = a.sc.samp_vn; sv.face_pmf = a.sc.face_pmf; sv.face_cdf = a.sc.face_cdf; sv.vnormals = a.sc.vnormals;
     sv.texels = a.sc.texels; sv.tex_info = a.sc.tex_info; sv.uvs = a.sc.uvs;
     sv.flat_off = (uint32_t)(offsetof(FusedArgs, sc) + offsetof(SceneDev, flat));
+    sv.hull_off = (uint32_t)offsetof(FusedArgs, hull);
     if (SCENE_LDS) {
         const uint32_t tree_bytes = a.sc.n_wnodes * (uint32_t)sizeof(WNode);
         if constexpr (kPrimTable) {
@@ -333,6 +339,9 @@
 #endif
 #ifdef MTR_PROFILE_SIMT
     st.ls[0] = st.ls[1] = st.ws[0] = st.ws[1] = 0; st.wmax = 0; st.wcalls = 0;
+#endif
+#if defined(MTR_PROFILE_OCC) && MTR_PROFILE_OCC == 4
+    for (int k = 0; k < 5; ++k) st.hull_n[k] = 0u;
 #endif
 #ifdef MTR_PROFILE_CYCLES
     for (int k = 0; k < 6; ++k) st.cyc[k] = 0;
@@ -513,6 +522,7 @@
 #if MTR_PROFILE_OCC == 2
         occ_alive += occ_ran ? 1u : 0u; occ_wait += occ_need ? 1u : 0u; occ_ran = false; occ_need = false;
 #elif MTR_PROFILE_OCC == 3
+#elif MTR_PROFILE_OCC == 4
 #else
         occ_alive += (uint32_t)__popcll(__ballot(alive)); occ_wait += (uint32_t)__popcll(__ballot(waiting));
 #endif
@@ -757,9 +767,16 @@
     if (kLean) __syncthreads();
     if (tid < 5 && a.counters) atomicAdd(&a.counters->paths + tid, s_cnt[tid]);
 #ifdef MTR_PROFILE_OCC
+#if MTR_PROFILE_OCC == 4
+    if (a.counters) {
+        atomicAdd(&a.counters->r0, ((unsigned long long)st.hull_n[0] << 32) | st.hull_n[1]); atomicAdd(&a.counters->r1, ((unsigned long long)st.hull_n[2] << 32) | st.hull_n[3]);
+        atomicAdd(&a.counters->splats_overflow, ((unsigned long long)st.hull_n[4] << 32) | ((tid & 63) == 0 ? (occ_iter & 0xffffffffull) : 0ull));
+    }
+#else
     if ((tid & 63) == 0 && a.counters) {
         atomicAdd(&a.counters->splats_overflow, occ_iter); atomicAdd(&a.counters->r0, occ_alive); atomicAdd(&a.counters->r1, occ_wait);
     }
+#endif
 #endif
 #ifdef MTR_PROFILE_TAIL
     if (tid == 0 && a.counters) {
diff --git a/mitransient_amd/csrc/mtr_scene_host.cpp b/mitransient_amd/csrc/mtr_scene_host.cpp
--- a/mitransient_amd/csrc/mtr_scene_host.cpp
+++ b/mitransient_amd/csrc/mtr_scene_host.cpp
@@ -71,7 +71,7 @@
     return mk((neg ? -x : x) + 1.0f, neg ? -b : b, neg ? -nx : nx);
 }
 static void sh_frame_from(f3 n, f3 dp_du, f3 &s, f3 &t) { sh_frame_of(n, dp_du, s, t); }
-static void rect_to_object(const float c[3], const float du[3], const float dv[3], float rx[4], float ry[4], float rz[4])
+void rect_to_object(const float c[3], const float du[3], const float dv[3], float rx[4], float ry[4], float rz[4])
 {
     const double a[3] = { du[0], du[1], du[2] }, b[3] = { dv[0], dv[1], dv[2] }, o[3] = { c[0], c[1], c[2] };
     double n[3] = { a[1] * b[2] - a[2] * b[1], a[2] * b[0] - a[0] * b[2], a[0] * b[1] - a[1] * b[0] };
@@ -478,6 +478,42 @@
             if (prim_mask >> root.n_quads) hs.traits |= kTrFlatLeaves;
         }
     }
+    classify_shadow_hull(d, hs);
+}
+
+void classify_shadow_hull(const mtr_scene_desc &d, HostScene &hs)
+{
+    static_assert((float)kHullShadowEps == kShadowEps, "mtr_shadow_hull.h derives delta_E from shade_hit's kShadowEps");
+    hs.hull = ShadowHull{};
+    if ((hs.traits & (kTrFlatTop | kTrFlatLeaves | kTrOneRectEmitter)) != (kTrFlatTop | kTrOneRectEmitter) || hs.ems.size() != 1u) return;
+    const WNode &root = hs.wnodes[0];
+    const Emitter &E = hs.ems[0];
+    float rows[kWide][4];
+    HullInput in{};
+    std::vector<float> verts(d.tri_verts, d.tri_verts + 9u * (size_t)d.n_tris);
+    uint32_t n_e = 0u;
+    for (uint32_t k = 0; k < root.n_quads && k < kWide; ++k) {
+        const uint32_t first = ((~(uint32_t)root.ref[k]) & ~kLeafQuadBit) >> 2;
+        if (first >= hs.tshade.size()) return;
+        const q4 Z = hs.tpairs[first >> 1].g[0];
+        rows[k][0] = Z.x; rows[k][1] = Z.y; rows[k][2] = Z.z; rows[k][3] = Z.w;
+        const TriShade &t = hs.tshade[first];
+        const f3 du = mk(t.h[2].y, t.h[2].z, t.h[2].w), dv = mk(t.h[3].x, t.h[3].y, t.h[3].z), c = mk(t.h[3].w, t.h[4].x, t.h[4].y);
+        for (int i = 0; i < 4; ++i) {
+            const float a = (i & 1) ? 1.0f : -1.0f, b = (i & 2) ? 1.0f : -1.0f;
+            verts.push_back(c.x + a * du.x + b * dv.x); verts.push_back(c.y + a * du.y + b * dv.y); verts.push_back(c.z + a * du.z + b * dv.z);
+        }
+        if ((fbits(t.h[4].z) >> 16) == 1u) {
+            if (c.x != E.center[0] || c.y != E.center[1] || c.z != E.center[2] || du.x != E.du[0] || du.y != E.du[1] || du.z != E.du[2] ||
+                dv.x != E.dv[0] || dv.y != E.dv[1] || dv.z != E.dv[2]) return;
+            in.e_child = k; ++n_e;
+        }
+    }
+    if (n_e != 1u) return;
+    in.n_quads = root.n_quads; in.rows = rows;
+    for (int k = 0; k < 3; ++k) { in.ec[k] = E.center[k]; in.edu[k] = E.du[k]; in.edv[k] = E.dv[k]; in.en[k] = E.n[k]; }
+    in.verts = verts.data(); in.n_verts = verts.size() / 3u;
+    if (!shadow_hull_classify(in, hs.hull)) hs.hull.count = 0u;
 }
 
 const char *derive_nlos(const mtr_scene_desc &d, HostNlos &o)
diff --git a/mitransient_amd/csrc/mtr_scene_host.h b/mitransient_amd/csrc/mtr_scene_host.h
--- a/mitransient_amd/csrc/mtr_scene_host.h
+++ b/mitransient_amd/csrc/mtr_scene_host.h
@@ -32,6 +32,7 @@
     bool grey_scene = false;
     bool has_sphere = false;
     FlatTop flat{};
+    ShadowHull hull{};
 };
 
 inline bool bsdf_is_lobe(uint32_t type) { return bsdf_is_rough(type) || type == MTR_BSDF_THINDIELECTRIC; }
@@ -40,7 +41,9 @@
 {
     return !has_sphere && colours_are_grey(mats, n_mats, ems, n_ems, textured);
 }
+void rect_to_object(const float c[3], const float du[3], const float dv[3], float rx[4], float ry[4], float rz[4]);
 void classify_scene(const mtr_scene_desc &d, HostScene &s);
+void classify_shadow_hull(const mtr_scene_desc &d, HostScene &s);
 uint32_t traits_with_laser(uint32_t traits, bool grey_scene, const float laser_irradiance[3]);
 
 uint32_t tint_slot_table(const mtr_material *mats, uint32_t n_mats, int32_t *slots);
diff --git a/mitransient_amd/csrc/mtr_shadow_hull.h b/mitransient_amd/csrc/mtr_shadow_hull.h
--- /dev/null
+++ b/mitransient_amd/csrc/mtr_shadow_hull.h
@@ -0,0 +1,108 @@
+#pragma once
+#include <cmath>
+#include <cstddef>
+#include <cstdint>
+
+#if defined(__HIPCC__)
+#define MTR_SH_HD __host__ __device__ inline
+#else
+#define MTR_SH_HD inline
+#endif
+
+namespace mtr {
+
+constexpr uint32_t kHullRows = 8;
+struct ShadowHull {
+    uint32_t count, e_child;
+    float e_delta, pad;
+    float e_row[4];
+    float delta[kHullRows];
+    float row[kHullRows][4];
+};
+static_assert(sizeof(ShadowHull) == 192, "dword-sized, no padding");
+
+MTR_SH_HD float hull_side(const float r[4], float ox, float oy, float oz) { return fmaf(r[2], oz, fmaf(r[1], oy, fmaf(r[0], ox, r[3]))); }
+
+constexpr double kHullU = 5.9604644775390625e-8;
+constexpr double kHullSafety = 4.0, kHullSafetyE = 2.0, kHullPoke = 64.0;
+constexpr double kHullShadowEps = 1500.0 * 5.9604644775390625e-8 * 10.0;
+constexpr double kHullOffsetGrow = 1.001;
+
+struct HullInput {
+    uint32_t n_quads;
+    const float (*rows)[4];
+    uint32_t e_child;
+    float ec[3], edu[3], edv[3], en[3];
+    const float *verts; size_t n_verts;
+};
+
+inline bool shadow_hull_classify(const HullInput &in, ShadowHull &out)
+{
+    out = ShadowHull{};
+    for (uint32_t k = 0; k < kHullRows; ++k) out.row[k][3] = 1.0f;
+    if (in.n_quads < 2u || in.n_quads > kHullRows || in.e_child >= in.n_quads || !in.n_verts) return false;
+    double lo[3] = { 1e300, 1e300, 1e300 }, hi[3] = { -1e300, -1e300, -1e300 };
+    for (size_t v = 0; v < in.n_verts; ++v)
+        for (int a = 0; a < 3; ++a) {
+            const double x = in.verts[3 * v + a];
+            if (!std::isfinite(x)) return false;
+            lo[a] = fmin(lo[a], x); hi[a] = fmax(hi[a], x);
+        }
+    double corner[4][3], B[3], L[3];
+    for (int c = 0; c < 4; ++c)
+        for (int a = 0; a < 3; ++a) {
+            corner[c][a] = (double)in.ec[a] + ((c & 1) ? 1.0 : -1.0) * (double)in.edu[a] + ((c & 2) ? 1.0 : -1.0) * (double)in.edv[a];
+            lo[a] = fmin(lo[a], corner[c][a]); hi[a] = fmax(hi[a], corner[c][a]);
+        }
+    for (int a = 0; a < 3; ++a) { B[a] = fmax(fabs(lo[a]), fabs(hi[a])) * kHullOffsetGrow + 1e-3; L[a] = (hi[a] - lo[a]) * kHullOffsetGrow + 2e-3; }
+    auto plane = [](const float *Z, const double *p) { return (double)Z[0] * p[0] + (double)Z[1] * p[1] + (double)Z[2] * p[2] + (double)Z[3]; };
+    auto mag = [&](const float *Z) { return fabs((double)Z[0]) * B[0] + fabs((double)Z[1]) * B[1] + fabs((double)Z[2]) * B[2] + fabs((double)Z[3]); };
+    auto ext = [&](const float *Z) { return fabs((double)Z[0]) * L[0] + fabs((double)Z[1]) * L[1] + fabs((double)Z[2]) * L[2]; };
+    uint32_t n = 0;
+    for (uint32_t k = 0; k < in.n_quads; ++k) {
+        const float *Z = in.rows[k];
+        const double M = mag(Z), D = ext(Z);
+        if (!std::isfinite(M) || !(M > 0.0)) return false;
+        if (k == in.e_child) {
+            const double front[3] = { (double)in.ec[0] + (double)in.en[0], (double)in.ec[1] + (double)in.en[1], (double)in.ec[2] + (double)in.en[2] };
+            const double sf = plane(Z, front);
+            if (!(fabs(sf) > 0.5)) return false;
+            const float s = sf > 0.0 ? 1.0f : -1.0f;
+            double hc = 0.0;
+            for (int c = 0; c < 4; ++c) hc = fmax(hc, fabs(plane(Z, corner[c])));
+            const double err = kHullU * (5.02 * M + 6.1 * D) + hc;
+            const double de = kHullSafetyE * err / (kHullShadowEps - 4.0 * kHullU);
+            if (!std::isfinite(de) || !(de < 3.0e38)) return false;
+            for (int a = 0; a < 4; ++a) out.e_row[a] = s * Z[a];
+            out.e_delta = (float)de * 1.000001f;
+            out.e_child = k;
+            continue;
+        }
+        double hmin = 1e300, hmax = -1e300;
+        for (int c = 0; c < 4; ++c) { const double h = plane(Z, corner[c]); hmin = fmin(hmin, h); hmax = fmax(hmax, h); }
+        const float s = hmin > 0.0 ? 1.0f : -1.0f;
+        const double m = s > 0.0f ? hmin : -hmax;
+        if (!(m >= kHullSafety * kHullU * (8.0 * M + 7.0 * D))) return false;
+        const double eta = 16.0 * kHullU * M, poke = fmax(eta, D / kHullPoke);
+        for (size_t v = 0; v < in.n_verts; ++v) {
+            const double p[3] = { in.verts[3 * v], in.verts[3 * v + 1], in.verts[3 * v + 2] };
+            if (!((double)s * plane(Z, p) >= -poke)) return false;
+        }
+        for (int a = 0; a < 4; ++a) out.row[n][a] = s * Z[a];
+        out.delta[n] = (float)eta * 1.000001f;
+        ++n;
+    }
+    out.count = n;
+    return n != 0u;
+}
+
+inline ShadowHull shadow_hull_with_margin(const ShadowHull &h, float margin)
+{
+    ShadowHull o = h;
+    if (!(margin >= 1.0f) || !h.count) { o.count = 0u; return o; }
+    for (uint32_t k = 0; k < kHullRows; ++k) o.delta[k] = h.delta[k] * margin;
+    o.e_delta = h.e_delta * margin;
+    return o;
+}
+
+}
diff --git a/mitransient_amd/integrators/common.py b/mitransient_amd/integrators/common.py
--- a/mitransient_amd/integrators/common.py
+++ b/mitransient_amd/integrators/common.py
@@ -1,6 +1,7 @@
 from __future__ import annotations
 
 import ctypes as C
+import math
 from typing import Tuple
 
 from .. import _cabi, variant
@@ -57,6 +58,10 @@
         self.deterministic = bool(props.get("amd_deterministic", False))
         self.direct_develop = bool(props.get("amd_direct_develop", True))
         self.reserve_cus = int(props.get("amd_reserve_cus", 0))
+        m = props.get("amd_shadow_hull_margin", 1)
+        if not (m == 0 or 1 <= m <= 65535):
+            raise Exception("\"amd_shadow_hull_margin\" must be 0 (off) or a value in [1, 65535]")
+        self.shadow_hull_margin = 0 if m == 0 else int(math.ceil(m))
         self.mode = _cabi.MTR_MODE_AUTO
         m = props.get("amd_mode", None)
         if m is not None:
@@ -158,6 +163,8 @@
             f |= _cabi.MTR_FLAG_DETERMINISTIC
         if variant.is_polarized():
             f |= _cabi.MTR_FLAG_POLARIZED
+        m = int(self.shadow_hull_margin)
+        f |= (_cabi.MTR_SHADOW_HULL_OFF if m == 0 else m - 1) << _cabi.MTR_SHADOW_HULL_SHIFT
         return f
 
     def render_params(self, film, seed_value, spp_total, spp_begin=0, spp_end=None,
diff --git a/mitransient_amd/mi.py b/mitransient_amd/mi.py
--- a/mitransient_amd/mi.py
+++ b/mitransient_amd/mi.py
@@ -453,6 +453,13 @@
         ctx.check(ctx.lib.mtr_scene_traits(self.gpu_handle(ctx, sensor), C.byref(t)), "mtr_scene_traits")
         return int(t.value)
 
+    def gpu_shadow_hull(self, sensor=0):
+        from .runtime import get_context
+        ctx = get_context()
+        n = C.c_uint32(0)
+        ctx.check(ctx.lib.mtr_scene_shadow_hull(self.gpu_handle(ctx, sensor), C.byref(n)), "mtr_scene_shadow_hull")
+        return int(n.value)
+
     def __del__(self):
         try:
             lib = _cabi.load_library()
```
